# huzaifakhan04/truely-real-time-ai-generated-video-detection-framework-for-social-platforms

Measured on AMD Instinct MI355X. Metric: frames/sec (detect+embed+drift) 720p, higher is better.
Workload: dtype f32; 1 GPU; BASELINE configs[1]: synthetic 720p 1-face frames, batch=256 per GPU, fp32, MTCNN detect + 80x80 crop + InceptionResnetV1 embed + cosine drift score; frames_per_gpu=256, height=720, width=1280, weights=seeded synthetic (no checkpoints offline), prelu_slopes=unit, min_face_size=20, pyramid_levels=11, valid_faces=256, score=6, emb_crc32=3015932725, mode=sharded, ingest=resident, parallelism=single GPU, batches_in_flight=1, driver=single, embed_group=8

## Files before the change

include/truely_hip.h:

```cpp
#ifndef TRUELY_HIP_H
#define TRUELY_HIP_H
#include <stddef.h>
#include <stdint.h>

#ifdef __cplusplus
extern "C" {
#endif

#define TRL_ABI_VERSION 7

typedef enum {
    TRL_OK = 0,
    TRL_ERR_INVALID = -1,
    TRL_ERR_HIP = -2,
    TRL_ERR_WEIGHTS = -3,
    TRL_ERR_CAPACITY = -4,
    TRL_ERR_STATE = -5
} trl_status;

typedef struct trl_ctx trl_ctx;

typedef struct {
    int    device;
    int    min_face_size;
    float  thr0, thr1, thr2;
    double factor;
    int    cap_level;
    int    cap_frame;
    int    max_faces;
    int    pnet_mode;
    int    embed_mode;
    int    embed_precision;
} trl_config;

int  trl_abi_version(void);
const char* trl_last_error(void);
int  trl_default_config(trl_config* cfg);

int  trl_create(const trl_config* cfg, trl_ctx** out);
int  trl_destroy(trl_ctx* ctx);
int  trl_load_weights(trl_ctx* ctx, const void* host_blob, size_t nbytes);

int  trl_mtcnn_detect(trl_ctx* ctx, const uint8_t* d_frames, int n, int H, int W,
                      float* d_boxes, float* d_probs, int32_t* d_counts, void* stream);

int  trl_mtcnn_detect_landmarks(trl_ctx* ctx, const uint8_t* d_frames, int n, int H, int W,
                                float* d_boxes, float* d_probs, float* d_points, int32_t* d_counts, void* stream);

int  trl_mtcnn_detect_ordered(trl_ctx* ctx, const uint8_t* d_frames, int n, int H, int W, int order,
                              float* d_boxes, float* d_probs, float* d_points, int32_t* d_counts, void* stream);

int  trl_select_faces(trl_ctx* ctx, int n, const float* d_boxes, const float* d_probs, const int32_t* d_counts, int H, int W,
                      int method, float threshold, double center_weight, int32_t* d_pick, void* stream);

int  trl_extract_faces(trl_ctx* ctx, const uint8_t* d_frames, int n, int H, int W, const int32_t* d_frame_of, const float* d_boxes,
                       int m, int S, int margin, int resample, int post_process, float* d_out, int32_t* d_status, void* stream);

int  trl_facenet_embed(trl_ctx* ctx, const float* d_faces, int n, int h, int w, float* d_emb, void* stream);

int  trl_facenet_num_classes(trl_ctx* ctx, int* C);
int  trl_facenet_features(trl_ctx* ctx, const float* d_faces, const uint8_t* d_valid, int n, int h, int w, float* d_feat, void* stream);
int  trl_facenet_logits(trl_ctx* ctx, const float* d_feat, int n, float* d_logits, long long ld, void* stream);

int  trl_detect_embed(trl_ctx* ctx, const uint8_t* d_frames, int n, int H, int W,
                      float* d_box, float* d_prob, int32_t* d_rect, uint8_t* d_valid, float* d_emb,
                      void* stream);

int  trl_detect_crop(trl_ctx* ctx, const uint8_t* d_frames, int n, int H, int W,
                     float* d_box, float* d_prob, int32_t* d_rect, uint8_t* d_valid, float* d_faces, void* stream);
int  trl_facenet_embed_masked(trl_ctx* ctx, const float* d_faces, const uint8_t* d_valid, int n, int h, int w, float* d_emb, void* stream);

int  trl_detect_embed_begin(trl_ctx* ctx, const uint8_t* d_frames, int n, int H, int W,
                            float* d_box, float* d_prob, int32_t* d_rect, uint8_t* d_valid, float* d_emb, void* stream);
int  trl_detect_crop_begin(trl_ctx* ctx, const uint8_t* d_frames, int n, int H, int W,
                           float* d_box, float* d_prob, int32_t* d_rect, uint8_t* d_valid, float* d_faces, void* stream);
int  trl_detect_embed_end(trl_ctx* ctx);

int  trl_drift_score(trl_ctx* ctx, const float* d_emb, const uint8_t* d_valid, int n,
                     long long frame_count, int fps, float* d_sims, uint8_t* d_flags,
                     int32_t* d_result, void* stream);

#define TRL_DRIFT_STATE_BYTES 2064
int  trl_drift_update(trl_ctx* ctx, void* d_state, const float* d_emb, const uint8_t* d_valid, int n,
                      long long frame_count, int fps, float* d_sims, uint8_t* d_flags, int32_t* d_result, void* stream);

int  trl_ingest_nv12(trl_ctx* ctx, const uint8_t* d_nv12, int n_in, int H, int W, int step,
                     uint8_t* d_bgr, int* n_out, void* stream);
int  trl_ingest_i420(trl_ctx* ctx, const uint8_t* d_i420, int n_in, int H, int W, int step,
                     uint8_t* d_bgr, int* n_out, void* stream);

int  trl_debug_stage_boxes(trl_ctx* ctx, int stage, int frame, float* h_boxes, int max_rows, int* n_out);
int  trl_debug_level_counts(trl_ctx* ctx, int frame, int32_t* h_cand, int32_t* h_keep, int* n_levels);
int  trl_debug_level_cands(trl_ctx* ctx, int frame, int level, void* h_rows, int max_rows, int* n_out);
int  trl_debug_level_keep(trl_ctx* ctx, int frame, int level, int32_t* h_idx, int max_rows, int* n_out);
int  trl_debug_nms_tiers(trl_ctx* ctx, int small_tier, int full_tier);
int  trl_debug_list_stats(trl_ctx* ctx, long long* h_out8);
int  trl_debug_option(trl_ctx* ctx, const char* key, int value);
int  trl_debug_pnet_screen_bound(trl_ctx* ctx, float* A, float* B, int* on);
int  trl_debug_pnet_screen_weights(trl_ctx* ctx, float* h_g16);
int  trl_debug_batch_capacity(trl_ctx* ctx, float t2_per_frame, float t3_per_frame, int* last_attempts);
int  trl_debug_pyramid_level(trl_ctx* ctx, const uint8_t* d_frame, int H, int W, int level, float* d_out, int* h, int* w, void* stream);
int  trl_debug_pyramid_batch(trl_ctx* ctx, const uint8_t* d_frames, int n, int H, int W, float* d_out, long long* pyr_stride,
                             int32_t* h_levels, int max_levels, int* n_levels, void* stream);
#define TRL_PYR_PLAN_COLS 6
enum { TRL_PYR_FINE = 1, TRL_PYR_S4 = 2, TRL_PYR_S8 = 3, TRL_PYR_SW4 = 4, TRL_PYR_SW8 = 5,
       TRL_PYR_L0_3 = 6, TRL_PYR_L0_4 = 7, TRL_PYR_L0_5 = 8, TRL_PYR_L1 = 9, TRL_PYR_L2 = 10 };
int  trl_debug_pyramid_plan(trl_ctx* ctx, int32_t* h_rows, int max_levels, int* n_levels);
enum { TRL_FNK_FN_CONV = 1, TRL_FNK_FN_SPLIT4 = 2, TRL_FNK_CONV_TAP = 3, TRL_FNK_IGEMM_VEC = 4, TRL_FNK_IGEMM_SCALAR = 5,
       TRL_FNK_SPLITK4 = 6, TRL_FNK_SPLITK4_TAP = 7, TRL_FNK_TAP48 = 8, TRL_FNK_BF16 = 9 };
typedef struct {
    int32_t conv, family, bm, bn, bk, pad, nz, m, cout, k, precision, has_res;
    char layer[48];
} trl_fn_plan_row;
int  trl_debug_facenet_plan(trl_ctx* ctx, trl_fn_plan_row* h_rows, int max_rows, int* n_rows);
int  trl_debug_facenet_capture(trl_ctx* ctx, int conv_index);
int  trl_debug_facenet_capture_read(trl_ctx* ctx, int view, void* h_dst, size_t max_bytes, int32_t* dims5);
int  trl_debug_poison(trl_ctx* ctx, int byte);
int  trl_debug_pnet_level(trl_ctx* ctx, const uint8_t* d_frame, int H, int W, int level,
                          float* d_prob, float* d_reg, int* oh, int* ow, void* stream);
int  trl_debug_rnet(trl_ctx* ctx, const float* d_crops, int n, float* d_out, void* stream);
int  trl_debug_onet(trl_ctx* ctx, const float* d_crops, int n, float* d_out, void* stream);
int  trl_debug_front_net(trl_ctx* ctx, const uint8_t* d_frame, int H, int W, const float* h_boxes, int nb, int net,
                         float* d_out, void* stream);
int  trl_debug_stage_net(trl_ctx* ctx, const uint8_t* d_frames, int nf, int H, int W, const float* h_recs, int nb, int net,
                         int capacity, float* d_out, void* stream);
int  trl_debug_front(trl_ctx* ctx, const uint8_t* d_frames, int nf, int H, int W, const int32_t* h_win, int nb, int net,
                     int capacity, float* d_pool, void* stream);
int  trl_debug_lists(trl_ctx* ctx, int kind, int n, int H, int W, const int32_t* h_caps, int n_levels, const int32_t* h_counts,
                     const void* h_rows, const float* h_logits, float* h_pts, float* d_boxes, float* d_probs, float* d_points,
                     int32_t* d_counts, float* d_box0, float* d_prob0, int32_t* d_rect, uint8_t* d_valid, void* stream);
int  trl_debug_mtcnn_plan(trl_ctx* ctx, trl_fn_plan_row* h_rows, int max_rows, int* n_rows);
int  trl_debug_crop_resize(trl_ctx* ctx, const uint8_t* d_frames, int n, int H, int W,
                           const int32_t* d_rect, const uint8_t* d_valid, float* d_faces, void* stream);
int  trl_debug_crop_aligned(trl_ctx* ctx, const uint8_t* d_frames, int n, int H, int W, const float* d_pts,
                            const uint8_t* d_valid, int S, int rgb, float* d_faces, void* stream);
int  trl_debug_crop_area(trl_ctx* ctx, const uint8_t* d_frames, int n, int H, int W, const int32_t* d_rect,
                         const uint8_t* d_valid, int S, int rgb, float* d_faces, void* stream);
int  trl_debug_timings(trl_ctx* ctx, float* out4);
int  trl_debug_workspace(trl_ctx* ctx, int what, int n, int h, int w, long long* h_out6);
enum { TRL_RZ_MAX_GUARD = 1 << 20, TRL_RZ_MAX_HITS = 256, TRL_RZ_CLEAR = 1, TRL_RZ_SWEEP = 2 };
typedef struct {
    int32_t arena, block;
    char site[24];
    long long block_bytes, gap_off, gap_bytes, first, last, count;
} trl_rz_hit;
int  trl_debug_redzone(trl_ctx* ctx, long long guard, int byte);
int  trl_debug_redzone_report(trl_ctx* ctx, int flags, long long* h_out4, trl_rz_hit* h_hits, int max_hits);
int  trl_debug_redzone_poke(trl_ctx* ctx, int arena, int block, long long offset, int value);
int  trl_debug_stage_totals(trl_ctx* ctx, int32_t* h_out2);
int  trl_debug_pnet_run(trl_ctx* ctx, int run);
int  trl_debug_pnet_kernel_ms(trl_ctx* ctx, float* ms);
int  trl_debug_pnet_span(trl_ctx* ctx, int reset, double* ms_sum, int32_t* launches);

typedef struct trl_jpeg trl_jpeg;
int  trl_jpeg_create(int device, int H, int W, int quality, int max_frames, trl_jpeg** out);
int  trl_jpeg_destroy(trl_jpeg* enc);
int  trl_jpeg_encode(trl_jpeg* enc, const uint8_t* d_bgr, int n, long long frame_stride, uint8_t* d_out, long long capacity,
                     long long* h_sizes, void* stream);
int  trl_jpeg_header(int H, int W, int quality, uint8_t* buf, size_t cap, int* len);
typedef struct trl_jpeg_options {
    int quality, subsampling, restart_rows, restart_blocks, optimize;
} trl_jpeg_options;
int  trl_jpeg_create_ex(int device, int H, int W, const trl_jpeg_options* opt, int max_frames, trl_jpeg** out);
int  trl_jpeg_header_ex(int H, int W, const trl_jpeg_options* opt, uint8_t* buf, size_t cap, int* len);
int  trl_jpeg_optimal_table(const uint32_t* hist, uint8_t* bits, uint8_t* vals, int* nvals, int* maxlen);

typedef struct trl_jpegd trl_jpegd;
typedef struct {
    int32_t width, height;
    int32_t h_samp, v_samp;
    int32_t restart_interval;
    int32_t scan_offset;
    int32_t supported;
    int32_t reason;
} trl_jpegd_info;
int  trl_jpegd_parse(const uint8_t* file, size_t len, trl_jpegd_info* info);
int  trl_jpegd_create(int device, int H, int W, int max_frames, long long max_bytes, trl_jpegd** out);
int  trl_jpegd_destroy(trl_jpegd* dec);
int  trl_jpegd_debug_poison(trl_jpegd* dec, int byte);
int  trl_jpegd_decode(trl_jpegd* dec, const uint8_t* h_files, const uint8_t* d_files, const long long* offsets, const long long* sizes,
                      int n, uint8_t* d_bgr, long long frame_stride, int32_t* h_status, void* stream);

typedef struct {
    int32_t frame;
    int32_t x0, y0, x1, y1;
    int32_t thickness;
    int32_t seg_begin, seg_end;
    uint8_t rect_bgr[3];
    uint8_t text_bgr[3];
    uint8_t reserved[2];
} trl_draw_frame;
typedef struct { float x0, y0, dx, dy, L2, reach; } trl_draw_seg;
size_t trl_draw_workspace(int n_frames, int n_segs);
int  trl_draw(uint8_t* d_bgr, int n, long long frame_stride, int H, int W, const trl_draw_frame* frames, int n_frames,
              const trl_draw_seg* segs, int n_segs, void* d_work, size_t work_bytes, void* stream);

int    trl_gallery_pack(const float* d_rows, long long m, float* d_mat, long long ld, float* d_n2, long long c0, void* stream);
int    trl_gallery_scores(const float* d_q, int n, const float* d_mat, long long ld, const float* d_n2, long long m, int metric,
                          float* d_out, long long ldo, void* stream);
size_t trl_gallery_search_workspace(int n, long long m, int k, int max_strip_cols);
int    trl_gallery_search(const float* d_q, const uint8_t* d_valid, int n, const float* d_mat, long long ld, const float* d_n2,
                          long long m, int metric, int k, float* d_score, int32_t* d_index, void* d_ws, size_t ws_bytes,
                          int max_strip_cols, void* stream);

int    trl_cluster_links(const float* d_q, const uint8_t* d_valid, int n, const float* d_mat, long long ld, const float* d_n2,
                         int metric, float threshold, uint32_t* d_adj, long long pitch_words, int32_t* d_degree,
                         int max_strip_cols, void* stream);
size_t trl_cluster_workspace(int n);
int    trl_cluster_labels(const uint32_t* d_adj, long long pitch_words, const int32_t* d_degree, int n, int min_samples,
                          int32_t* d_labels, uint8_t* d_core, int32_t* d_count, void* d_ws, size_t ws_bytes, int* rounds_out,
                          void* stream);
size_t trl_cluster_lists_workspace(int n);
int    trl_cluster_labels_lists(const long long* d_offsets, const int32_t* d_index, const uint8_t* d_valid, int n, int min_samples,
                                int lanes_per_row, int32_t* d_degree, int32_t* d_labels, uint8_t* d_core, int32_t* d_count,
                                void* d_ws, size_t ws_bytes, int* rounds_out, void* stream);

size_t trl_gallery_hist_workspace(int n, long long m, int nedges, int max_strip_cols);
int    trl_gallery_hist(const float* d_q, const uint8_t* d_qvalid, const int32_t* d_qid, int n, const float* d_mat, long long ld,
                        const float* d_n2, const uint8_t* d_gvalid, const int32_t* d_gid, long long m, int metric, int pairs,
                        const float* d_edges, int nedges, long long* d_counts, void* d_ws, size_t ws_bytes, int max_strip_cols,
                        void* stream);

size_t trl_gallery_range_workspace(int n, long long m, int max_strip_cols);
int    trl_gallery_range_count(const float* d_q, const uint8_t* d_qvalid, int n, const float* d_mat, long long ld, const float* d_n2,
                               const uint8_t* d_gvalid, long long m, int metric, float threshold, int self, long long* d_offsets,
                               void* d_ws, size_t ws_bytes, int max_strip_cols, void* stream);
int    trl_gallery_range_fill(const float* d_q, const uint8_t* d_qvalid, int n, const float* d_mat, long long ld, const float* d_n2,
                              const uint8_t* d_gvalid, long long m, int metric, float threshold, int self, const long long* d_offsets,
                              const void* d_ws, size_t ws_bytes, long long capacity, int32_t* d_index, float* d_score,
                              int max_strip_cols, void* stream);

size_t trl_gallery_search_groups_workspace(int n, long long m, int k, int max_strip_cols);
int    trl_gallery_search_groups(const float* d_q, const uint8_t* d_valid, int n, const float* d_mat, long long ld, const float* d_n2,
                                 const int32_t* d_gid, long long m, int metric, int k, float* d_score, int32_t* d_index,
                                 int32_t* d_group, void* d_ws, size_t ws_bytes, int max_strip_cols, void* stream);

#define TRL_TRACK_SLOTS 64
#define TRL_TRACK_STATE_BYTES 135200
int    trl_track_update(void* d_state, const float* d_boxes, const int32_t* d_counts, int n, int m, const float* d_emb, float iou_min,
                        float sim_min, int max_age, int32_t* d_track, float* d_sim, uint8_t* d_flag, int32_t* d_table, int table_cap,
                        void* stream);
int    trl_track_scores(const void* d_state, const int32_t* d_table, int table_cap, long long frame_count, int fps, int32_t* d_score,
                        int32_t* d_summary, void* stream);

#ifdef __cplusplus
}
#endif
#endif
```

truely-real-time-ai-generated-video-detection-framework-for-social-platforms_amd/_lib.py:

```python
from __future__ import annotations

import ctypes as C
import os

_HERE = os.path.dirname(os.path.abspath(__file__))
LIB_PATH = os.path.join(_HERE, "libtruely_hip.so")


class TrlConfig(C.Structure):
    _fields_ = [("device", C.c_int), ("min_face_size", C.c_int), ("thr0", C.c_float), ("thr1", C.c_float),
                ("thr2", C.c_float), ("factor", C.c_double), ("cap_level", C.c_int), ("cap_frame", C.c_int),
                ("max_faces", C.c_int), ("pnet_mode", C.c_int), ("embed_mode", C.c_int), ("embed_precision", C.c_int)]


class TrlJpegdInfo(C.Structure):
    _fields_ = [(n, C.c_int32) for n in ("width", "height", "h_samp", "v_samp", "restart_interval", "scan_offset", "supported", "reason")]


class TrlJpegOptions(C.Structure):
    _fields_ = [(n, C.c_int) for n in ("quality", "subsampling", "restart_rows", "restart_blocks", "optimize")]


class TrlRzHit(C.Structure):
    _fields_ = [("arena", C.c_int32), ("block", C.c_int32), ("site", C.c_char * 24)] + \
               [(n, C.c_longlong) for n in ("block_bytes", "gap_off", "gap_bytes", "first", "last", "count")]


class TrlError(RuntimeError):
    def __init__(self, status: int, msg: str):
        super().__init__(f"libtruely_hip status {status}: {msg}")
        self.status = status


_lib = None
_vp, _i, _f = C.c_void_p, C.c_int, C.c_float

_SIGNATURES = {
    "trl_abi_version": (C.c_int, []),
    "trl_last_error": (C.c_char_p, []),
    "trl_default_config": (C.c_int, [C.POINTER(TrlConfig)]),
    "trl_create": (C.c_int, [C.POINTER(TrlConfig), C.POINTER(_vp)]),
    "trl_destroy": (C.c_int, [_vp]),
    "trl_load_weights": (C.c_int, [_vp, C.c_char_p, C.c_size_t]),
    "trl_mtcnn_detect": (C.c_int, [_vp, _vp, _i, _i, _i, _vp, _vp, _vp, _vp]),
    "trl_mtcnn_detect_landmarks": (C.c_int, [_vp, _vp, _i, _i, _i, _vp, _vp, _vp, _vp, _vp]),
    "trl_mtcnn_detect_ordered": (C.c_int, [_vp, _vp, _i, _i, _i, _i, _vp, _vp, _vp, _vp, _vp]),
    "trl_select_faces": (C.c_int, [_vp, _i, _vp, _vp, _vp, _i, _i, _i, _f, C.c_double, _vp, _vp]),
    "trl_extract_faces": (C.c_int, [_vp, _vp, _i, _i, _i, _vp, _vp, _i, _i, _i, _i, _i, _vp, _vp, _vp]),
    "trl_facenet_embed": (C.c_int, [_vp, _vp, _i, _i, _i, _vp, _vp]),
    "trl_facenet_num_classes": (C.c_int, [_vp, C.POINTER(_i)]),
    "trl_facenet_features": (C.c_int, [_vp, _vp, _vp, _i, _i, _i, _vp, _vp]),
    "trl_facenet_logits": (C.c_int, [_vp, _vp, _i, _vp, C.c_longlong, _vp]),
    "trl_detect_embed": (C.c_int, [_vp, _vp, _i, _i, _i, _vp, _vp, _vp, _vp, _vp, _vp]),
    "trl_detect_crop": (C.c_int, [_vp, _vp, _i, _i, _i, _vp, _vp, _vp, _vp, _vp, _vp]),
    "trl_detect_embed_begin": (C.c_int, [_vp, _vp, _i, _i, _i, _vp, _vp, _vp, _vp, _vp, _vp]),
    "trl_detect_crop_begin": (C.c_int, [_vp, _vp, _i, _i, _i, _vp, _vp, _vp, _vp, _vp, _vp]),
    "trl_detect_embed_end": (C.c_int, [_vp]),
    "trl_facenet_embed_masked": (C.c_int, [_vp, _vp, _vp, _i, _i, _i, _vp, _vp]),
    "trl_drift_score": (C.c_int, [_vp, _vp, _vp, _i, C.c_longlong, _i, _vp, _vp, _vp, _vp]),
    "trl_ingest_nv12": (C.c_int, [_vp, _vp, _i, _i, _i, _i, _vp, C.POINTER(_i), _vp]),
    "trl_ingest_i420": (C.c_int, [_vp, _vp, _i, _i, _i, _i, _vp, C.POINTER(_i), _vp]),
    "trl_drift_update": (C.c_int, [_vp, _vp, _vp, _vp, _i, C.c_longlong, _i, _vp, _vp, _vp, _vp]),
    "trl_debug_stage_boxes": (C.c_int, [_vp, _i, _i, _vp, _i, C.POINTER(_i)]),
    "trl_debug_level_counts": (C.c_int, [_vp, _i, _vp, _vp, C.POINTER(_i)]),
    "trl_debug_level_cands": (C.c_int, [_vp, _i, _i, _vp, _i, C.POINTER(_i)]),
    "trl_debug_level_keep": (C.c_int, [_vp, _i, _i, _vp, _i, C.POINTER(_i)]),
    "trl_debug_batch_capacity": (C.c_int, [_vp, _f, _f, C.POINTER(_i)]),
    "trl_debug_nms_tiers": (C.c_int, [_vp, _i, _i]),
    "trl_debug_option": (C.c_int, [_vp, C.c_char_p, _i]),
    "trl_debug_list_stats": (C.c_int, [_vp, C.POINTER(C.c_longlong)]),
    "trl_debug_poison": (C.c_int, [_vp, _i]),
    "trl_debug_pyramid_level": (C.c_int, [_vp, _vp, _i, _i, _i, _vp, C.POINTER(_i), C.POINTER(_i), _vp]),
    "trl_debug_pyramid_batch": (C.c_int, [_vp, _vp, _i, _i, _i, _vp, C.POINTER(C.c_longlong), _vp, _i, C.POINTER(_i), _vp]),
    "trl_debug_pyramid_plan": (C.c_int, [_vp, _vp, _i, C.POINTER(_i)]),
    "trl_debug_facenet_plan": (C.c_int, [_vp, _vp, _i, C.POINTER(_i)]),
    "trl_debug_facenet_capture": (C.c_int, [_vp, _i]),
    "trl_debug_facenet_capture_read": (C.c_int, [_vp, _i, _vp, C.c_size_t, _vp]),
    "trl_debug_pnet_level": (C.c_int, [_vp, _vp, _i, _i, _i, _vp, _vp, C.POINTER(_i), C.POINTER(_i), _vp]),
    "trl_debug_rnet": (C.c_int, [_vp, _vp, _i, _vp, _vp]),
    "trl_debug_onet": (C.c_int, [_vp, _vp, _i, _vp, _vp]),
    "trl_debug_front_net": (C.c_int, [_vp, _vp, _i, _i, _vp, _i, _i, _vp, _vp]),
    "trl_debug_stage_net": (C.c_int, [_vp, _vp, _i, _i, _i, _vp, _i, _i, _i, _vp, _vp]),
    "trl_debug_front": (C.c_int, [_vp, _vp, _i, _i, _i, _vp, _i, _i, _i, _vp, _vp]),
    "trl_debug_mtcnn_plan": (C.c_int, [_vp, _vp, _i, C.POINTER(_i)]),
    "trl_debug_lists": (C.c_int, [_vp, _i, _i, _i, _i, _vp, _i, _vp, _vp, _vp, _vp, _vp, _vp, _vp, _vp, _vp, _vp, _vp, _vp, _vp]),
    "trl_debug_crop_resize": (C.c_int, [_vp, _vp, _i, _i, _i, _vp, _vp, _vp, _vp]),
    "trl_debug_crop_aligned": (C.c_int, [_vp, _vp, _i, _i, _i, _vp, _vp, _i, _i, _vp, _vp]),
    "trl_debug_crop_area": (C.c_int, [_vp, _vp, _i, _i, _i, _vp, _vp, _i, _i, _vp, _vp]),
    "trl_debug_timings": (C.c_int, [_vp, C.POINTER(_f)]),
    "trl_debug_workspace": (C.c_int, [_vp, _i, _i, _i, _i, C.POINTER(C.c_longlong)]),
    "trl_debug_redzone": (C.c_int, [_vp, C.c_longlong, _i]),
    "trl_debug_redzone_report": (C.c_int, [_vp, _i, C.POINTER(C.c_longlong), C.POINTER(TrlRzHit), _i]),
    "trl_debug_redzone_poke": (C.c_int, [_vp, _i, _i, C.c_longlong, _i]),
    "trl_debug_stage_totals": (C.c_int, [_vp, C.POINTER(C.c_int32)]),
    "trl_debug_pnet_run": (C.c_int, [_vp, _i]),
    "trl_debug_pnet_kernel_ms": (C.c_int, [_vp, C.POINTER(C.c_float)]),
    "trl_debug_pnet_span": (C.c_int, [_vp, C.c_int, C.POINTER(C.c_double), C.POINTER(C.c_int32)]),
    "trl_debug_pnet_screen_bound": (C.c_int, [_vp, C.POINTER(_f), C.POINTER(_f), C.POINTER(_i)]),
    "trl_debug_pnet_screen_weights": (C.c_int, [_vp, C.POINTER(_f)]),
    "trl_jpeg_create": (C.c_int, [_i, _i, _i, _i, _i, C.POINTER(_vp)]),
    "trl_jpeg_destroy": (C.c_int, [_vp]),
    "trl_jpeg_encode": (C.c_int, [_vp, _vp, _i, C.c_longlong, _vp, C.c_longlong, _vp, _vp]),
    "trl_jpeg_header": (C.c_int, [_i, _i, _i, _vp, C.c_size_t, C.POINTER(_i)]),
    "trl_jpeg_create_ex": (C.c_int, [_i, _i, _i, C.POINTER(TrlJpegOptions), _i, C.POINTER(_vp)]),
    "trl_jpeg_header_ex": (C.c_int, [_i, _i, C.POINTER(TrlJpegOptions), _vp, C.c_size_t, C.POINTER(_i)]),
    "trl_jpeg_optimal_table": (C.c_int, [_vp, _vp, _vp, C.POINTER(_i), C.POINTER(_i)]),
    "trl_jpegd_parse": (C.c_int, [_vp, C.c_size_t, _vp]),
    "trl_jpegd_create": (C.c_int, [_i, _i, _i, _i, C.c_longlong, C.POINTER(_vp)]),
    "trl_jpegd_destroy": (C.c_int, [_vp]),
    "trl_jpegd_debug_poison": (C.c_int, [_vp, _i]),
    "trl_jpegd_decode": (C.c_int, [_vp, _vp, _vp, _vp, _vp, _i, _vp, C.c_longlong, _vp, _vp]),
    "trl_draw_workspace": (C.c_size_t, [_i, _i]),
    "trl_draw": (C.c_int, [_vp, _i, C.c_longlong, _i, _i, _vp, _i, _vp, _i, _vp, C.c_size_t, _vp]),
    "trl_gallery_pack": (C.c_int, [_vp, C.c_longlong, _vp, C.c_longlong, _vp, C.c_longlong, _vp]),
    "trl_gallery_scores": (C.c_int, [_vp, _i, _vp, C.c_longlong, _vp, C.c_longlong, _i, _vp, C.c_longlong, _vp]),
    "trl_gallery_search_workspace": (C.c_size_t, [_i, C.c_longlong, _i, _i]),
    "trl_gallery_search": (C.c_int, [_vp, _vp, _i, _vp, C.c_longlong, _vp, C.c_longlong, _i, _i, _vp, _vp, _vp, C.c_size_t, _i, _vp]),
    "trl_cluster_links": (C.c_int, [_vp, _vp, _i, _vp, C.c_longlong, _vp, _i, _f, _vp, C.c_longlong, _vp, _i, _vp]),
    "trl_cluster_workspace": (C.c_size_t, [_i]),
    "trl_cluster_labels": (C.c_int, [_vp, C.c_longlong, _vp, _i, _i, _vp, _vp, _vp, _vp, C.c_size_t, C.POINTER(_i), _vp]),
    "trl_cluster_lists_workspace": (C.c_size_t, [_i]),
    "trl_cluster_labels_lists": (C.c_int, [_vp, _vp, _vp, _i, _i, _i, _vp, _vp, _vp, _vp, _vp, C.c_size_t, C.POINTER(_i), _vp]),
    "trl_gallery_hist_workspace": (C.c_size_t, [_i, C.c_longlong, _i, _i]),
    "trl_gallery_hist": (C.c_int, [_vp, _vp, _vp, _i, _vp, C.c_longlong, _vp, _vp, _vp, C.c_longlong, _i, _i, _vp, _i, _vp, _vp, C.c_size_t, _i, _vp]),
    "trl_gallery_range_workspace": (C.c_size_t, [_i, C.c_longlong, _i]),
    "trl_gallery_range_count": (C.c_int, [_vp, _vp, _i, _vp, C.c_longlong, _vp, _vp, C.c_longlong, _i, _f, _i, _vp, _vp, C.c_size_t, _i, _vp]),
    "trl_gallery_range_fill": (C.c_int, [_vp, _vp, _i, _vp, C.c_longlong, _vp, _vp, C.c_longlong, _i, _f, _i, _vp, _vp, C.c_size_t, C.c_longlong,
                                         _vp, _vp, _i, _vp]),
    "trl_gallery_search_groups_workspace": (C.c_size_t, [_i, C.c_longlong, _i, _i]),
    "trl_gallery_search_groups": (C.c_int, [_vp, _vp, _i, _vp, C.c_longlong, _vp, _vp, C.c_longlong, _i, _i, _vp, _vp, _vp, _vp, C.c_size_t,
                                            _i, _vp]),
    "trl_track_update": (C.c_int, [_vp, _vp, _vp, _i, _i, _vp, _f, _f, _i, _vp, _vp, _vp, _vp, _i, _vp]),
    "trl_track_scores": (C.c_int, [_vp, _vp, _i, C.c_longlong, _i, _vp, _vp, _vp]),
}
EXPORTS = tuple(_SIGNATURES)


def load(path: str | None = None):
    global _lib
    if _lib is not None:
        return _lib
    path = path or os.environ.get("TRUELY_HIP_LIB") or LIB_PATH
    if not os.path.exists(path):
        raise ImportError(f"{path} not found: build it with `make -C {_HERE}/csrc` "
                          "(or __graft_entry__.build()); there is no CPU fallback")
    try:
        import torch
    except Exception:
        pass
    lib = C.CDLL(path, mode=C.RTLD_GLOBAL)
    for name, (res, args) in _SIGNATURES.items():
        fn = getattr(lib, name, None)
        if fn is None and path != LIB_PATH and name.startswith("trl_debug_"):
            continue
        if fn is None:
            raise ImportError(f"{path} lacks {name}")
        fn.restype = res
        fn.argtypes = args
    if lib.trl_abi_version() != 7:
        raise ImportError("libtruely_hip ABI mismatch")
    _lib = lib
    return lib


def check(status: int):
    if status != 0:
        raise TrlError(status, load().trl_last_error().decode(errors="replace"))
```

truely-real-time-ai-generated-video-detection-framework-for-social-platforms_amd/csrc/trl_api.hip:

```cpp
#include <limits.h>
#include <stdarg.h>
#include <stdio.h>
#include <string.h>
#include <stdlib.h>
#include <algorithm>

#include "trl_ctx.h"

static thread_local char g_err[512] = "";
int g_trl_no_fnconv = 0;
int g_trl_pnet_gate = 0;

#include <mutex>
namespace {
std::mutex g_gate_mu;
hipEvent_t g_gate_ev[64] = {};
bool g_gate_set[64] = {};
}
int trl_gate_wait(trl_ctx* c, hipStream_t s) {
    const int d = c->cfg.device;
    if (!g_trl_pnet_gate || d < 0 || d >= 64) return TRL_OK;
    std::lock_guard<std::mutex> lk(g_gate_mu);
    if (g_gate_set[d]) TRL_HIP(hipStreamWaitEvent(s, g_gate_ev[d], 0));
    return TRL_OK;
}
int trl_gate_record(trl_ctx* c, hipStream_t s) {
    const int d = c->cfg.device;
    if (!g_trl_pnet_gate || d < 0 || d >= 64) return TRL_OK;
    std::lock_guard<std::mutex> lk(g_gate_mu);
    if (!g_gate_ev[d]) TRL_HIP(hipEventCreateWithFlags(&g_gate_ev[d], hipEventDisableTiming));
    TRL_HIP(hipEventRecord(g_gate_ev[d], s));
    g_gate_set[d] = true;
    return TRL_OK;
}
void trl_set_error(const char* fmt, ...) {
    va_list ap;
    va_start(ap, fmt);
    vsnprintf(g_err, sizeof g_err, fmt, ap);
    va_end(ap);
}

extern "C" {

int trl_abi_version(void) { return TRL_ABI_VERSION; }
const char* trl_last_error(void) { return g_err; }

int trl_default_config(trl_config* cfg) {
    if (!cfg) return TRL_ERR_INVALID;
    cfg->device = 0;
    cfg->min_face_size = 20;
    cfg->thr0 = 0.6f; cfg->thr1 = 0.7f; cfg->thr2 = 0.7f;
    cfg->factor = 0.709;
    cfg->cap_level = 2048;
    cfg->cap_frame = 2048;
    cfg->max_faces = 64;
    cfg->pnet_mode = 0;
    cfg->embed_mode = 0;
    cfg->embed_precision = 0;
    return TRL_OK;
}

int trl_create(const trl_config* cfg, trl_ctx** out) {
    if (!cfg || !out) { trl_set_error("null argument"); return TRL_ERR_INVALID; }
    if (cfg->cap_level < 64 || cfg->cap_level > (1 << 24) || cfg->cap_frame < 64 || cfg->cap_frame > (1 << 24) || (cfg->cap_level & 3) ||
        (cfg->cap_frame & 3) || cfg->min_face_size < 12 || cfg->max_faces < 1 || !(cfg->factor > 0.1 && cfg->factor < 0.99) || cfg->embed_mode < 0 || cfg->embed_mode > 3 ||
        cfg->embed_precision < 0 || cfg->embed_precision > 2) {
        trl_set_error("bad trl_config (list start capacities must be multiples of 4 in [64, 2^24], min_face_size >= 12)");
        return TRL_ERR_INVALID;
    }
    TRL_HIP(hipSetDevice(cfg->device));
    trl_ctx* c = new trl_ctx();
    c->cfg = *cfg;
    c->pnet_prof = trl_tune_set("TRL_PNET_CLOCK");
    if (hipMalloc((void**)&c->pnet_clk, 8 * 41) != hipSuccess || hipMemset(c->pnet_clk, 0, 8 * 41) != hipSuccess || hipMemset(c->pnet_clk, 0xFF, 8) != hipSuccess ||
        hipMalloc((void**)&c->pnet_cursor, 64) != hipSuccess || hipHostMalloc((void**)&c->h_pinned, 1024) != hipSuccess ||
        hipEventCreate(&c->ev_call0) != hipSuccess || hipEventCreate(&c->ev_call1) != hipSuccess) {
        trl_set_error("context allocation failed: %s", hipGetErrorString(hipGetLastError()));
        trl_destroy(c);
        return TRL_ERR_HIP;
    }
    memset(c->h_pinned, 0, 1024);
    *out = c;
    return TRL_OK;
}

int trl_destroy(trl_ctx* c) {
    if (!c) return TRL_OK;
    (void)hipSetDevice(c->cfg.device);
    (void)hipDeviceSynchronize();
    c->pend.active = false;
    trl_free_weights(c);
    if (c->arena.base) (void)hipFree(c->arena.base);
    if (c->scratch.base) (void)hipFree(c->scratch.base);
    if (c->sims_tmp.base) (void)hipFree(c->sims_tmp.base);
    if (c->pyr_tab) (void)hipFree(c->pyr_tab);
    if (c->rz.dev) (void)hipFree(c->rz.dev);
    for (auto& b : c->fn_cap) if (b.p) (void)hipFree(b.p);
    if (c->pnet_clk) {
        unsigned long long t[41];
        if (c->pnet_prof && hipMemcpy(t, c->pnet_clk, sizeof t, hipMemcpyDeviceToHost) == hipSuccess && t[2 + 32] > 0) {
            static const char* nm[8] = {"phase0", "barrier0", "phase1", "barrier1", "phase2", "barrier2", "phase3", "barrier3"};
            const double tiles = (double)t[2 + 32];
            fprintf(stderr, "[TRL_PNET_CLOCK] shader clocks per tile (wave 0..3), %.0f workgroup-tiles\n", tiles);
            for (int k = 0; k < 8; k++)
                fprintf(stderr, "[TRL_PNET_CLOCK] %-9s %8.0f %8.0f %8.0f %8.0f\n", nm[k], t[2 + k] / tiles, t[2 + 8 + k] / tiles, t[2 + 16 + k] / tiles, t[2 + 24 + k] / tiles);
            fprintf(stderr, "[TRL_PNET_CLOCK] fp16 screen: %llu M-tiles screened, %llu confirmed (%.2f %%)\n", t[39], t[40],
                    t[39] ? 100.0 * (double)t[40] / (double)t[39] : 0.0);
        }
        (void)hipFree(c->pnet_clk);
    }
    if (c->pnet_cursor) (void)hipFree(c->pnet_cursor);
    if (c->h_pinned) (void)hipHostFree(c->h_pinned);
    if (c->ev_call0) (void)hipEventDestroy(c->ev_call0);
    if (c->ev_call1) (void)hipEventDestroy(c->ev_call1);
    for (auto& e : c->pnet_ev) { (void)hipEventDestroy(e.first); (void)hipEventDestroy(e.second); }
    delete c;
    return TRL_OK;
}

}

__global__ void k_rz_scan(const unsigned char* __restrict__ base, const unsigned long long* __restrict__ gaps, unsigned long long* __restrict__ res,
                          int g0, unsigned byte) {
    const int g = g0 + blockIdx.y;
    const unsigned long long len = gaps[2 * g + 1];
    const unsigned char* p = base + gaps[2 * g];
    unsigned long long head = (16 - ((uintptr_t)p & 15)) & 15;
    if (head > len) head = len;
    const unsigned long long nw = (len - head) / 16, tail0 = head + nw * 16;
    const unsigned long long w = 0x0101010101010101ull * (byte & 0xFF);
    const unsigned long long tid = (unsigned long long)blockIdx.x * blockDim.x + threadIdx.x, nt = (unsigned long long)gridDim.x * blockDim.x;
    unsigned long long cnt = 0, first = ~0ull, last = 0;
    auto look = [&](unsigned long long i) {
        if (p[i] == (unsigned char)byte) return;
        cnt++;
        if (i < first) first = i;
        if (i > last) last = i;
    };
    if (tid == 0) {
        for (unsigned long long i = 0; i < head; i++) look(i);
        for (unsigned long long i = tail0; i < len; i++) look(i);
    }
    const ulonglong2* q = reinterpret_cast<const ulonglong2*>(p + head);
    for (unsigned long long k = tid; k < nw; k += nt) {
        const ulonglong2 v = q[k];
        if (v.x == w && v.y == w) continue;
        for (int b = 0; b < 16; b++) look(head + k * 16 + b);
    }
    if (cnt) {
        atomicAdd(&res[3 * g], cnt);
        atomicMin(&res[3 * g + 1], first);
        atomicMax(&res[3 * g + 2], last);
    }
}

namespace {
struct RzGap { size_t off, len; int block; size_t block_bytes; };
void rz_gaps(const Arena& a, std::vector<RzGap>& out) {
    const size_t nb = a.blocks.size();
    for (size_t i = 0; i < nb; i++) {
        const size_t end = a.blocks[i].off + a.blocks[i].bytes, next = i + 1 < nb ? a.blocks[i + 1].off : a.off;
        if (next > end) out.push_back({end, next - end, (int)i, a.blocks[i].bytes});
    }
    if (a.cap > a.off) out.push_back({a.off, a.cap - a.off, (int)nb, 0});
}
int rz_sweep(trl_ctx* c, Arena& a, const char* site, long long refill_from) {
    trl_ctx::RedZone& z = c->rz;
    TRL_HIP(hipDeviceSynchronize());
    if (!a.base) return TRL_OK;
    std::vector<RzGap> gaps;
    rz_gaps(a, gaps);
    const size_t ng = gaps.size();
    if (ng) {
        if (z.dev_gaps < ng) {
            if (z.dev) TRL_HIP(hipFree(z.dev));
            z.dev = nullptr; z.dev_gaps = 0;
            TRL_HIP(hipMalloc((void**)&z.dev, (ng + 256) * 5 * 8));
            z.dev_gaps = ng + 256;
        }
        std::vector<unsigned long long> tab(5 * ng, 0);
        for (size_t g = 0; g < ng; g++) { tab[2 * g] = gaps[g].off; tab[2 * g + 1] = gaps[g].len; tab[2 * ng + 3 * g + 1] = ~0ull; }
        TRL_HIP(hipMemcpy(z.dev, tab.data(), tab.size() * 8, hipMemcpyHostToDevice));
        const bool has_tail = gaps.back().block == (int)a.blocks.size();
        const size_t nshort = has_tail ? ng - 1 : ng;
        for (size_t g0 = 0; g0 < nshort; g0 += 32768) {
            const unsigned ny = (unsigned)std::min<size_t>(32768, nshort - g0);
            k_rz_scan<<<dim3(4, ny), 256>>>((const unsigned char*)a.base, z.dev, z.dev + 2 * ng, (int)g0, (unsigned)z.byte);
            TRL_LAUNCH_CHECK();
        }
        if (has_tail) {
            k_rz_scan<<<dim3(4096, 1), 256>>>((const unsigned char*)a.base, z.dev, z.dev + 2 * ng, (int)(ng - 1), (unsigned)z.byte);
            TRL_LAUNCH_CHECK();
        }
        TRL_HIP(hipMemcpy(tab.data() + 2 * ng, z.dev + 2 * ng, 3 * ng * 8, hipMemcpyDeviceToHost));
        for (size_t g = 0; g < ng; g++) {
            z.bytes += (long long)gaps[g].len;
            const unsigned long long* r = &tab[2 * ng + 3 * g];
            if (!r[0]) continue;
            z.nhits++;
            if (z.hits.size() < TRL_RZ_MAX_HITS) {
                trl_rz_hit h;
                memset(&h, 0, sizeof h);
                h.arena = &a == &c->arena ? 0 : 1; h.block = gaps[g].block;
                strncpy(h.site, site, sizeof(h.site) - 1);
                h.block_bytes = (long long)gaps[g].block_bytes; h.gap_off = (long long)gaps[g].off; h.gap_bytes = (long long)gaps[g].len;
                h.first = (long long)r[1]; h.last = (long long)r[2]; h.count = (long long)r[0];
                z.hits.push_back(h);
            }
            TRL_HIP(hipMemset(a.base + gaps[g].off, z.byte, gaps[g].len));
        }
    }
    z.sweeps++;
    if (refill_from >= 0 && (size_t)refill_from < a.cap) TRL_HIP(hipMemset(a.base + refill_from, z.byte, a.cap - (size_t)refill_from));
    TRL_HIP(hipDeviceSynchronize());
    return TRL_OK;
}
void rz_on_rewind(Arena& a, size_t mark, const char* site, void* owner) { (void)rz_sweep((trl_ctx*)owner, a, site, (long long)mark); }
}

int trl_rz_sweep_all(trl_ctx* c, const char* site) {
    TRL_CHECK(rz_sweep(c, c->arena, site, -1));
    return rz_sweep(c, c->scratch, site, -1);
}

int trl_ensure(trl_ctx* c, Arena& a, size_t bytes) {
    if (bytes <= a.cap) return TRL_OK;
    const size_t ncap = bytes + (bytes >> 3) + (32u << 20);
    TRL_HIP(hipDeviceSynchronize());
    if (a.guard && a.base) TRL_CHECK(rz_sweep(c, a, "ensure", -1));
    if (a.base) { TRL_HIP(hipFree(a.base)); a.base = nullptr; a.cap = 0; }
    TRL_HIP(hipMalloc((void**)&a.base, ncap));
    a.cap = ncap;
    a.off = 0;
    a.blocks.clear();
    if (c->dbg_poison >= 0) TRL_HIP(hipMemset(a.base, c->dbg_poison, ncap));
    return TRL_OK;
}

int trl_check_idle(trl_ctx* c) {
    if (!c) { trl_set_error("null context"); return TRL_ERR_INVALID; }
    if (c->pend.active) { trl_set_error("the context has a call in flight: trl_detect_embed_end() first"); return TRL_ERR_STATE; }
    return TRL_OK;
}

static int check_call(trl_ctx* c, const void* frames, int n, int H, int W) {
    TRL_CHECK(trl_check_idle(c));
    if (!c->have_weights) { trl_set_error("trl_load_weights has not been called"); return TRL_ERR_STATE; }
    if (!frames || n <= 0 || n > 65535 || H < 12 || W < 12 || H > 16383 || W > 16383) {
        trl_set_error("bad frame batch n=%d H=%d W=%d (1..65535 frames of 12..16383 px per side)", n, H, W);
        return TRL_ERR_INVALID;
    }
    if (((uintptr_t)frames & 3) != 0) { trl_set_error("frame buffer must be 4-byte aligned"); return TRL_ERR_INVALID; }
    return TRL_OK;
}

static void collect_timings(trl_ctx* c) {
    float call_ms = 0.f, pnet_ms = 0.f, pyr_ms = 0.f;
    (void)hipEventElapsedTime(&call_ms, c->ev_call0, c->ev_call1);
    int launches = 0;
    if (c->cfg.pnet_mode == 0 && c->pnet_ev_used >= 2) {
// ... 522 lines not shown
        const int cap = kind == 1 ? h_caps[i % n_levels] : h_caps[n_levels];
        if (h_counts[i] < 0 || h_counts[i] > cap) { trl_set_error("list %d: count %d, capacity %d", i, h_counts[i], cap); return TRL_ERR_INVALID; }
        total += h_counts[i];
    }
    if (total > 0 && (!h_rows || (kind > 1 && !h_logits))) { trl_set_error("null rows"); return TRL_ERR_INVALID; }
    TRL_HIP(hipSetDevice(c->cfg.device));
    const int st = trl_cascade_lists(c, kind, n, H, W, h_caps, n_levels, h_counts, h_rows, h_logits, h_pts, d_boxes, d_probs, d_points, d_counts,
                                     d_box0, d_prob0, d_rect, d_valid, (hipStream_t)stream);
    TRL_CHECK(trl_rz_end(c, "lists_hook"));
    return st;
}

int trl_debug_workspace(trl_ctx* c, int what, int n, int h, int w, long long* h_out6) {
    TRL_CHECK(trl_check_idle(c));
    if (!h_out6 || (what != 0 && what != 1 && what != 24 && what != 48) || (what && n <= 0) || (what == 1 && (h < 75 || w < 75))) { trl_set_error("bad argument"); return TRL_ERR_INVALID; }
    if (what && !c->have_weights) { trl_set_error("context without weights"); return TRL_ERR_STATE; }
    Arena X = Arena::counter(c->scratch.guard);
    if (what == 1) TRL_CHECK(embed_need(c, false, n, h, w));
    else if (what) { const NetDesc& d = trl_net_of(what); TRL_CHECK(trl_run_net(c, X, d, 0, Act::dense(nullptr, n, d.side, d.side, 3), nullptr, nullptr)); }
    const size_t v[6] = {c->scratch.cap, c->scratch.high, c->arena.cap, c->arena.off, c->arena_need, what == 1 ? c->fn_need_bytes : X.high};
    for (int k = 0; k < 6; k++) h_out6[k] = (long long)v[k];
    return TRL_OK;
}

int trl_debug_redzone(trl_ctx* c, long long guard, int byte) {
    TRL_CHECK(trl_check_idle(c));
    if (guard < 0 || guard > TRL_RZ_MAX_GUARD || (guard & 255) || byte < 0 || byte > 255) {
        trl_set_error("bad red zone: guard %lld (0, or a multiple of 256 up to %d), fill byte %d", guard, (int)TRL_RZ_MAX_GUARD, byte);
        return TRL_ERR_INVALID;
    }
    trl_ctx::RedZone& z = c->rz;
    if (!guard && !z.guard) return TRL_OK;
    TRL_HIP(hipSetDevice(c->cfg.device));
    TRL_HIP(hipDeviceSynchronize());
    if (!z.guard) z.saved_poison = c->dbg_poison;
    for (Arena* a : {&c->arena, &c->scratch}) {
        if (a->base) TRL_HIP(hipFree(a->base));
        a->base = nullptr; a->cap = a->off = a->high = 0;
        a->blocks.clear();
        a->guard = (size_t)guard; a->on_rewind = guard ? rz_on_rewind : nullptr; a->owner = c;
    }
    c->cb = CascadeBufs();
    c->arena_need = 0;
    c->fn_need_key[0] = 0;
    z.guard = (size_t)guard; z.byte = byte;
    z.sweeps = z.bytes = z.nhits = 0;
    z.hits.clear();
    c->dbg_poison = guard ? byte : z.saved_poison;
    return TRL_OK;
}

int trl_debug_redzone_report(trl_ctx* c, int flags, long long* h_out4, trl_rz_hit* h_hits, int max_hits) {
    TRL_CHECK(trl_check_idle(c));
    if (!h_out4 || (max_hits > 0 && !h_hits)) { trl_set_error("null argument"); return TRL_ERR_INVALID; }
    trl_ctx::RedZone& z = c->rz;
    if ((flags & TRL_RZ_SWEEP) && z.guard) {
        TRL_HIP(hipSetDevice(c->cfg.device));
        TRL_CHECK(trl_rz_sweep_all(c, "report"));
    }
    int m = 0;
    for (; m < (int)z.hits.size() && m < max_hits; m++) h_hits[m] = z.hits[m];
    h_out4[0] = z.sweeps; h_out4[1] = z.bytes; h_out4[2] = z.nhits; h_out4[3] = m;
    if (flags & TRL_RZ_CLEAR) { z.sweeps = z.bytes = z.nhits = 0; z.hits.clear(); }
    return TRL_OK;
}

int trl_debug_redzone_poke(trl_ctx* c, int arena, int block, long long offset, int value) {
    TRL_CHECK(trl_check_idle(c));
    trl_ctx::RedZone& z = c->rz;
    if (!z.guard) { trl_set_error("red zones are off"); return TRL_ERR_STATE; }
    if ((arena != 0 && arena != 1) || value < 0 || value > 255 || value == z.byte) { trl_set_error("bad argument"); return TRL_ERR_INVALID; }
    Arena& a = arena ? c->scratch : c->arena;
    if (!a.base) { trl_set_error("the workspace has not been allocated"); return TRL_ERR_STATE; }
    std::vector<RzGap> gaps;
    rz_gaps(a, gaps);
    if (block < 0) block = (int)a.blocks.size();
    for (const RzGap& g : gaps) {
        if (g.block != block) continue;
        if (offset < 0 || (size_t)offset >= g.len) break;
        TRL_HIP(hipSetDevice(c->cfg.device));
        TRL_HIP(hipDeviceSynchronize());
        TRL_HIP(hipMemset(a.base + g.off + (size_t)offset, value, 1));
        TRL_HIP(hipDeviceSynchronize());
        return TRL_OK;
    }
    trl_set_error("no byte %lld in the gap behind block %d (%zu live blocks)", offset, block, a.blocks.size());
    return TRL_ERR_INVALID;
}

int trl_debug_mtcnn_plan(trl_ctx* c, trl_fn_plan_row* h_rows, int max_rows, int* n_rows) {
    TRL_CHECK(trl_check_idle(c));
    if (!n_rows || (max_rows > 0 && !h_rows)) { trl_set_error("null argument"); return TRL_ERR_INVALID; }
    *n_rows = (int)c->mt_plan.size();
    for (int i = 0; i < *n_rows && i < max_rows; i++) h_rows[i] = c->mt_plan[i];
    return TRL_OK;
}

static int check_crop_hook(trl_ctx* c, const void* d_frames, int n, int n_max, int H, int W, const void* d_rows, const void* d_valid,
                           int S, const void* d_faces) {
    if (!c || !d_frames || !d_rows || !d_valid || !d_faces || n <= 0 || n > n_max || H < 1 || W < 1 || S < 1 || S > 4096) {
        trl_set_error("bad argument (n=%d H=%d W=%d S=%d)", n, H, W, S);
        return TRL_ERR_INVALID;
    }
    return TRL_OK;
}
int trl_debug_crop_resize(trl_ctx* c, const uint8_t* d_frames, int n, int H, int W, const int32_t* d_rect, const uint8_t* d_valid,
                          float* d_faces, void* stream) {
    TRL_CHECK(check_crop_hook(c, d_frames, n, INT_MAX, H, W, d_rect, d_valid, 80, d_faces));
    TRL_CHECK(trl_launch_crop_resize80(d_frames, n, H, W, d_rect, d_valid, d_faces, (hipStream_t)stream));
    return trl_rz_end(c, "crop_resize");
}
int trl_debug_crop_aligned(trl_ctx* c, const uint8_t* d_frames, int n, int H, int W, const float* d_pts, const uint8_t* d_valid, int S,
                           int rgb, float* d_faces, void* stream) {
    TRL_CHECK(check_crop_hook(c, d_frames, n, 65535, H, W, d_pts, d_valid, S, d_faces));
    TRL_CHECK(trl_launch_crop_aligned(d_frames, n, H, W, d_pts, d_valid, S, rgb != 0, d_faces, (hipStream_t)stream));
    return trl_rz_end(c, "crop_aligned");
}
int trl_debug_crop_area(trl_ctx* c, const uint8_t* d_frames, int n, int H, int W, const int32_t* d_rect, const uint8_t* d_valid, int S,
                        int rgb, float* d_faces, void* stream) {
    TRL_CHECK(check_crop_hook(c, d_frames, n, 65535, H, W, d_rect, d_valid, S, d_faces));
    TRL_CHECK(trl_launch_crop_area_std(d_frames, n, H, W, d_rect, d_valid, S, rgb != 0, d_faces, (hipStream_t)stream));
    return trl_rz_end(c, "crop_area");
}
int trl_debug_nms_tiers(trl_ctx* c, int small_tier, int full_tier) {
    TRL_CHECK(trl_check_idle(c));
    if ((small_tier && (small_tier < 16 || small_tier > 3072 || (small_tier & 3))) || (full_tier && (full_tier < 16 || full_tier > 3072 || (full_tier & 3)))) {
        trl_set_error("tiers must be multiples of 4 in [16, 3072]");
        return TRL_ERR_INVALID;
    }
    if (small_tier) c->nms_small = small_tier;
    if (full_tier) c->nms_full = full_tier;
    return TRL_OK;
}
int trl_debug_list_stats(trl_ctx* c, long long* h_out8) {
    if (!c || !h_out8) { trl_set_error("null argument"); return TRL_ERR_INVALID; }
    const int32_t* f = c->h_pinned + 4;
    unsigned long long used = 0;
    memcpy(&used, f + FLG_SPILL_CUR, 8);
    int mx = 0;
    for (int l = 0; l < 32; l++) if (f[FLG_LEVEL_MAX + l] > mx) mx = f[FLG_LEVEL_MAX + l];
    h_out8[0] = c->caps.last_attempts; h_out8[1] = f[FLG_SPILL_LISTS]; h_out8[2] = (long long)used; h_out8[3] = (long long)c->cb.spill_cap;
    h_out8[4] = c->cb.capF; h_out8[5] = c->cb.lay.S; h_out8[6] = mx; h_out8[7] = f[FLG_FRAME_MAX];
    return TRL_OK;
}

int trl_debug_option(trl_ctx* c, const char* key, int value) {
    if (!key) { trl_set_error("null key"); return TRL_ERR_INVALID; }
    if (!strcmp(key, "no_fnconv")) { g_trl_no_fnconv = value ? 1 : 0; return TRL_OK; }
    if (!strcmp(key, "pnet_gate")) { g_trl_pnet_gate = value ? 1 : 0; return TRL_OK; }
    TRL_CHECK(trl_check_idle(c));
    if (!strcmp(key, "rnet_chunk") && value >= 16) { c->rnet_chunk = value; return TRL_OK; }
    if (!strcmp(key, "onet_chunk") && value >= 16) { c->onet_chunk = value; return TRL_OK; }
    if (!strcmp(key, "pnet_screen") && (value == 0 || value == 1)) { c->pnet_screen = value; return TRL_OK; }
    if (!strcmp(key, "pyr_row_bands") && value >= 0) { c->pyr_row_bands = value; return TRL_OK; }
    if (!strcmp(key, "tail_pool") && (value == 0 || value == 1)) { c->tail_pool = value; return TRL_OK; }
    trl_set_error("unknown option '%s' (or value %d out of range)", key, value);
    return TRL_ERR_INVALID;
}

int trl_debug_pnet_screen_bound(trl_ctx* c, float* A, float* B, int* on) {
    if (!c || !A || !B || !on) { trl_set_error("null argument"); return TRL_ERR_INVALID; }
    *A = c->pnet_scrA; *B = c->pnet_scrB; *on = c->pnet_screen_ok && c->pnet_screen;
    return TRL_OK;
}

int trl_debug_pnet_screen_weights(trl_ctx* c, float* h_g16) {
    if (!c || !h_g16) { trl_set_error("null argument"); return TRL_ERR_INVALID; }
    for (int i = 0; i < 16; i++) h_g16[i] = c->pnet_scrG[i];
    return TRL_OK;
}

int trl_debug_batch_capacity(trl_ctx* c, float t2_per_frame, float t3_per_frame, int* last_attempts) {
    if (!c) { trl_set_error("null context"); return TRL_ERR_INVALID; }
    if (t2_per_frame > 0.f) c->caps.t_per_frame[0] = t2_per_frame;
    if (t3_per_frame > 0.f) c->caps.t_per_frame[1] = t3_per_frame;
    if (last_attempts) *last_attempts = c->caps.last_attempts;
    return TRL_OK;
}

int trl_debug_stage_totals(trl_ctx* c, int32_t* h_out2) {
    if (!c || !h_out2) { trl_set_error("null argument"); return TRL_ERR_INVALID; }
    h_out2[0] = c->h_pinned[4 + FLG_T2N]; h_out2[1] = c->h_pinned[4 + FLG_T3N];
    return TRL_OK;
}

int trl_debug_pnet_run(trl_ctx* c, int run) {
    if (!c || run < 0 || run > 64) { trl_set_error("bad argument"); return TRL_ERR_INVALID; }
    c->pnet_run = run;
    return TRL_OK;
}

int trl_debug_pnet_span(trl_ctx* c, int reset, double* ms_sum, int32_t* launches) {
    if (!c || !ms_sum || !launches) { trl_set_error("null argument"); return TRL_ERR_INVALID; }
    *ms_sum = 0.0; *launches = 0;
    if (!c->pnet_clk) return TRL_OK;
    TRL_CHECK(trl_check_idle(c));
    TRL_HIP(hipSetDevice(c->cfg.device));
    TRL_HIP(hipDeviceSynchronize());
    unsigned long long t[2] = {0, 0};
    int khz = 0;
    TRL_HIP(hipMemcpy(t, c->pnet_clk + 36, sizeof t, hipMemcpyDeviceToHost));
    TRL_HIP(hipDeviceGetAttribute(&khz, hipDeviceAttributeWallClockRate, c->cfg.device));
    if (khz > 0) *ms_sum = (double)t[0] / (double)khz;
    *launches = (int32_t)t[1];
    if (reset) TRL_HIP(hipMemset(c->pnet_clk + 36, 0, 16));
    return TRL_OK;
}

int trl_debug_pnet_kernel_ms(trl_ctx* c, float* ms) {
    if (!c || !ms) { trl_set_error("null argument"); return TRL_ERR_INVALID; }
    *ms = c->pnet_kernel_ms;
    return TRL_OK;
}

int trl_debug_timings(trl_ctx* c, float* out4) {
    if (!c || !out4) return TRL_ERR_INVALID;
    out4[0] = c->last_ms[0]; out4[1] = c->last_ms[1]; out4[2] = c->last_ms[2]; out4[3] = c->last_ms[3];
    return TRL_OK;
}

}
```

truely-real-time-ai-generated-video-detection-framework-for-social-platforms_amd/csrc/trl_capacity.h:

```cpp
#pragma once
#include <cstddef>
#include <cstdint>
#include <cstring>

enum { TRL_NFLAGS = 64 };
enum { FLG_LEVEL = 0, FLG_FRAME = 1, FLG_T2 = 2, FLG_T3 = 3, FLG_T2N = 4, FLG_T3N = 5, FLG_FRAME_MAX = 6, FLG_SPILL = 7,
       FLG_SPILL_CUR = 8 , FLG_SPILL_LISTS = 10, FLG_LEVEL_MAX = 16  };

struct LvLayout {
    int L = 0, S = 0;
    int capl[32] = {0}, rec0[32] = {0};
};

struct CapRule { float mul, add, decay, floor; };
inline float trl_cap_follow(const CapRule& r, float cur, float measured, float per, bool overflow) {
    const float want = r.mul * measured / per + r.add;
    if (overflow) return want;
    const float d = r.decay * cur;
    return want > d ? want : (d > r.floor ? d : (cur < r.floor ? cur : r.floor));
}

struct CascadeCaps {
    static constexpr float T_START[2] = {160.f, 48.f};
    static constexpr CapRule T_RULE[2] = {{1.25f, 1.f, 0.97f, T_START[0]}, {1.25f, 1.f, 0.97f, T_START[1]}};
    static constexpr CapRule LIST_RULE = {1.25f, 4.f, 0.97f, 0.f};

    float t_per_frame[2] = {T_START[0], T_START[1]};
    float lvl_hint[32] = {0}, frame_hint = 0.f;
    size_t spill_hint = 0;
    int cap_t[2] = {0, 0};
    int resume_stage = 0;
    int last_attempts = 0;
};

struct CascadePlan { LvLayout lay; int capF = 0; int cap_t[2] = {0, 0}; };
inline int trl_cap_list(long long start, float hint, long long cells) {
    long long want = start;
    if ((long long)hint > want) want = (long long)hint;
    if (want > cells) want = cells;
    if (want < 4) want = 4;
    return (int)((want + 3) & ~3ll);
}
inline CascadePlan trl_caps_plan(const CascadeCaps& k, int cap_level, int cap_frame, const long long* cells, int L, int n) {
    CascadePlan p;
    LvLayout& G = p.lay;
    G.L = L;
    long long cells_total = 0;
    for (int l = 0; l < L; l++) {
        G.capl[l] = trl_cap_list(cap_level, k.lvl_hint[l], cells[l]);
        G.rec0[l] = G.S;
        G.S += G.capl[l];
        cells_total += cells[l];
    }
    p.capF = trl_cap_list(cap_frame, k.frame_hint, cells_total);
    const long long lim = (long long)n * p.capF;
    for (int s = 0; s < 2; s++) {
        const long long want = (long long)(k.t_per_frame[s] * n) + 64;
        p.cap_t[s] = (int)(want < lim ? want : lim);
    }
    return p;
}

struct CapsVerdict { int retry, resume_stage; };
inline CapsVerdict trl_caps_check(CascadeCaps& k, const int32_t* f, int n, const LvLayout& lay) {
    const int L = lay.L;
    k.resume_stage = 0;
    unsigned long long spill_used = 0;
    memcpy(&spill_used, f + FLG_SPILL_CUR, 8);
    if (f[FLG_LEVEL]) {
        long long sum = 0;
        for (int l = 0; l < L; l++) {
            const float want = trl_cap_follow(CascadeCaps::LIST_RULE, k.lvl_hint[l], (float)f[FLG_LEVEL_MAX + l], 1.f, true);
            if (f[FLG_LEVEL_MAX + l] > lay.capl[l] && want > k.lvl_hint[l]) k.lvl_hint[l] = want;
            sum += f[FLG_LEVEL_MAX + l];
        }
        if ((float)sum > k.frame_hint && (double)sum * 132.0 * (double)n < 8e9) k.frame_hint = (float)sum;
        return {1, 0};
    }
    const float frame_max = (float)f[FLG_FRAME_MAX];
    if (f[FLG_SPILL]) {
        k.spill_hint = (size_t)spill_used * 2 + (16u << 20);
        if (f[FLG_FRAME]) k.frame_hint = trl_cap_follow(CascadeCaps::LIST_RULE, k.frame_hint, frame_max, 1.f, true);
        return {1, 0};
    }
    if (f[FLG_FRAME]) { k.frame_hint = trl_cap_follow(CascadeCaps::LIST_RULE, k.frame_hint, frame_max, 1.f, true); return {1, 0}; }
    for (int s = 0; s < 2; s++)
        if (f[FLG_T2 + s]) {
            k.t_per_frame[s] = trl_cap_follow(CascadeCaps::T_RULE[s], k.t_per_frame[s], (float)f[FLG_T2N + s], (float)n, true);
            return {1, k.resume_stage = 2 + s};
        }
    for (int s = 0; s < 2; s++)
        k.t_per_frame[s] = trl_cap_follow(CascadeCaps::T_RULE[s], k.t_per_frame[s], (float)f[FLG_T2N + s], (float)n, false);
    for (int l = 0; l < L; l++)
        k.lvl_hint[l] = trl_cap_follow(CascadeCaps::LIST_RULE, k.lvl_hint[l], (float)f[FLG_LEVEL_MAX + l], 1.f, false);
    k.frame_hint = trl_cap_follow(CascadeCaps::LIST_RULE, k.frame_hint, frame_max, 1.f, false);
    {
        const size_t want = (size_t)spill_used + (spill_used >> 2), d = k.spill_hint - (k.spill_hint >> 5);
        k.spill_hint = spill_used ? (want > d ? want : d) : (d > (1u << 20) ? d : 0);
    }
    return {0, 0};
}
```

truely-real-time-ai-generated-video-detection-framework-for-social-platforms_amd/csrc/trl_cascade.hip:

```cpp
#include "trl_ctx.h"
#include <algorithm>
#include <stdlib.h>
#include <string.h>


namespace {

__device__ __forceinline__ uint32_t f2ord(float f) {
    uint32_t u = __float_as_uint(f);
    return (u & 0x80000000u) ? ~u : (u | 0x80000000u);
}

__device__ __forceinline__ uint64_t sort_key(float score, uint32_t tie) { return ((uint64_t)~f2ord(score) << 32) | tie; }
constexpr uint64_t NO_KEY = ~0ull;

__device__ void lds_bitonic_steps(uint64_t* key, uint32_t* id, int C, int base, int k, int j0) {
    for (int j = j0; j > 0; j >>= 1) {
        for (int t = threadIdx.x; t < C; t += blockDim.x) {
            const int u = t ^ j;
            if (u > t) {
                const bool up = (((base + t) & k) == 0);
                const uint64_t a = key[t], b = key[u];
                if ((a > b) == up) {
                    key[t] = b; key[u] = a;
// ... 543 lines not shown
                                                     const float* __restrict__ s1_box, const int32_t* __restrict__ off2,
                                                     const float* __restrict__ out6, int32_t* __restrict__ n2,
                                                     float* __restrict__ s2_box, Spill sp) {
    extern __shared__ __attribute__((aligned(16))) unsigned char smem_raw[];
    Smem S(smem_raw, lds_cap, blockDim.x);
    const int f = blockIdx.x;
    const int cnt = n1[f];
    if (cnt == 0 || off2[gridDim.x] > cap_total) { if (threadIdx.x == 0) n2[f] = 0; return; }
    const float* logits = out6 + (size_t)off2[f] * 6;
    const float* fb = s1_box + (size_t)f * capF * 5;
    auto prob = [&](int i) { return trl_softmax2_p1(logits[6 * i], logits[6 * i + 1]); };
    auto s1 = [&](uint32_t i) { const float* b = fb + 5 * i; return make_float4(b[0], b[1], b[2], b[3]); };
    const Kept K = sort_and_suppress<false, true>(S, lds_cap, cnt, 0.7f, sp, nullptr, W, H,
        [&](int i, uint32_t&) { const float p = prob(i); return p > thr ? sort_key(p, (uint32_t)i) : NO_KEY; },
        s1);
    const int out = write_rows(S, lds_cap, K.n, s2_box + (size_t)f * capF * 5, [&](int r, float4& b, float& score) {
        const int i = (int)K.id(r);
        score = prob(i);
        return stage2_row(s1(i), logits + 6 * i + 2, W, H, b);
    });
    if (threadIdx.x == 0) n2[f] = out;
}

__device__ __forceinline__ float4 stage3_box(const float* b, const float* g) {
    const float w = b[2] - b[0] + 1.f, h = b[3] - b[1] + 1.f;
    return make_float4(b[0] + g[0] * w, b[1] + g[1] * h, b[2] + g[2] * w, b[3] + g[3] * h);
}
__device__ __forceinline__ void stage3_points(const float* b, const float* pt, float* po) {
    const float w_i = b[2] - b[0] + 1.f, h_i = b[3] - b[1] + 1.f;
    for (int j = 0; j < 5; j++) {
        po[j] = w_i * pt[j] + b[0] - 1.f;
        po[5 + j] = h_i * pt[5 + j] + b[1] - 1.f;
    }
}
__global__ __launch_bounds__(1024) void k_stage3_post(int lds_cap, int capF, int cap_total, float thr, const int32_t* __restrict__ n2, const float* __restrict__ s2_box,
                                                     const int32_t* __restrict__ off3, const float* __restrict__ out16,
                                                     int32_t* __restrict__ n3, float* __restrict__ s3_box, float* __restrict__ s3_pts, Spill sp) {
    extern __shared__ __attribute__((aligned(16))) unsigned char smem_raw[];
    Smem S(smem_raw, lds_cap, blockDim.x);
    const int f = blockIdx.x;
    const int cnt = n2[f];
    if (cnt == 0 || off3[gridDim.x] > cap_total) { if (threadIdx.x == 0) n3[f] = 0; return; }
    const float* logits = out16 + (size_t)off3[f] * 16;
    const float* fb = s2_box + (size_t)f * capF * 5;
    auto prob = [&](int i) { return trl_softmax2_p1(logits[16 * i], logits[16 * i + 1]); };
    const Kept K = sort_and_suppress<true, true>(S, lds_cap, cnt, 0.7f, sp, nullptr, 0, 0,
        [&](int i, uint32_t&) { const float p = prob(i); return p > thr ? sort_key(p, ~(uint32_t)i) : NO_KEY; },
        [&](uint32_t i) { return stage3_box(fb + 5 * i, logits + 16 * i + 2); });
    for (int r = threadIdx.x; r < K.n; r += blockDim.x) {
        const int i = (int)K.id(r);
        const float4 bb = K.box(r);
        float* o = s3_box + ((size_t)f * capF + r) * 5;
        o[0] = bb.x; o[1] = bb.y; o[2] = bb.z; o[3] = bb.w; o[4] = prob(i);
        stage3_points(fb + 5 * i, logits + 16 * i + 6, s3_pts + ((size_t)f * capF + r) * 10);
    }
    if (threadIdx.x == 0) n3[f] = K.n;
}

__global__ __launch_bounds__(64) void k_select(int capF, int max_faces, int W, int H, int order, const int32_t* __restrict__ n3,
                                               const float* __restrict__ s3_box, const float* __restrict__ s3_pts,
                                               float* __restrict__ boxes, float* __restrict__ probs, float* __restrict__ points,
                                               int32_t* __restrict__ counts, float* __restrict__ box0, float* __restrict__ prob0,
                                               int32_t* __restrict__ rect, uint8_t* __restrict__ valid, float* __restrict__ pts0) {
    const int f = blockIdx.x;
    const int n = n3[f];
    const float* b = s3_box + (size_t)f * capF * 5;
    for (int r = threadIdx.x; r < n; r += blockDim.x) {
        int rank = r;
        if (order == 0) {
            const float ar = (b[5 * r + 2] - b[5 * r]) * (b[5 * r + 3] - b[5 * r + 1]);
            rank = 0;
            for (int q = 0; q < n; q++) {
                const float aq = (b[5 * q + 2] - b[5 * q]) * (b[5 * q + 3] - b[5 * q + 1]);
                rank += (aq > ar) || (aq == ar && q > r);
            }
        }
        if (boxes && rank < max_faces) {
            float* o = boxes + ((size_t)f * max_faces + rank) * 4;
            o[0] = b[5 * r]; o[1] = b[5 * r + 1]; o[2] = b[5 * r + 2]; o[3] = b[5 * r + 3];
            probs[(size_t)f * max_faces + rank] = b[5 * r + 4];
            if (points) {
                const float* ps = s3_pts + ((size_t)f * capF + r) * 10;
                float* po = points + ((size_t)f * max_faces + rank) * 10;
                for (int q = 0; q < 10; q++) po[q] = ps[q];
            }
        }
        if (rank == 0 && box0) {
            box0[4 * f] = b[5 * r]; box0[4 * f + 1] = b[5 * r + 1]; box0[4 * f + 2] = b[5 * r + 2]; box0[4 * f + 3] = b[5 * r + 3];
            prob0[f] = b[5 * r + 4];
            long long x0 = (long long)b[5 * r], y0 = (long long)b[5 * r + 1], x1 = (long long)b[5 * r + 2], y1 = (long long)b[5 * r + 3];
            if (x0 < 0) x0 = 0;
            if (y0 < 0) y0 = 0;
            if (x1 > W) x1 = W;
            if (y1 > H) y1 = H;
            rect[4 * f] = (int)x0; rect[4 * f + 1] = (int)y0; rect[4 * f + 2] = (int)x1; rect[4 * f + 3] = (int)y1;
            valid[f] = (x1 > x0 && y1 > y0) ? 1 : 0;
            if (pts0) {
                const float* ps = s3_pts + ((size_t)f * capF + r) * 10;
                for (int q = 0; q < 10; q++) pts0[10 * f + q] = ps[q];
            }
        }
    }
    if (threadIdx.x == 0) {
        if (counts) counts[f] = n < max_faces ? n : max_faces;
        if (n == 0 && box0) {
            for (int q = 0; q < 4; q++) { box0[4 * f + q] = 0.f; rect[4 * f + q] = 0; }
            prob0[f] = 0.f; valid[f] = 0;
            if (pts0) for (int q = 0; q < 10; q++) pts0[10 * f + q] = 0.f;
        }
    }
}

template <typename K>
int set_dyn_smem(K kernel, size_t bytes) {
    TRL_HIP(hipFuncSetAttribute((const void*)kernel, hipFuncAttributeMaxDynamicSharedMemorySize, (int)bytes));
    return TRL_OK;
}

}

int trl_compute_levels(trl_ctx* c, int H, int W) {
    const double m = 12.0 / c->cfg.min_face_size;
    double minl = (H < W ? H : W) * m;
    double scale_i = m;
    int L = 0;
    while (minl >= 12 && L < 32) {
        LevelGeom& g = c->lv[L];
        g.scale = scale_i;
        g.h = (int)(H * scale_i + 1);
        g.w = (int)(W * scale_i + 1);
        const int ph = (g.h - 2 + 1) / 2, pw = (g.w - 2 + 1) / 2;
        g.oh = ph - 4; g.ow = pw - 4;
        L++;
        scale_i = scale_i * c->cfg.factor;
        minl = minl * c->cfg.factor;
    }
    return L;
}

int trl_launch_area_level(const uint8_t* d_frames, int nf, int H, int W, int h, int w, float* d_level, hipStream_t s) {
    const size_t total = (size_t)nf * h * w;
    size_t blocks = (total + 255) / 256;
    if (blocks > 32768) blocks = 32768;
    k_area_level<<<(unsigned)blocks, 256, 0, s>>>(d_frames, nf, H, W, h, w, d_level);
    TRL_LAUNCH_CHECK();
    return TRL_OK;
}
int trl_launch_heads_to_maps(const float* d_heads, int cells, float* d_prob, float* d_reg, hipStream_t s) {
    k_heads_to_maps<<<(cells + 255) / 256, 256, 0, s>>>(d_heads, cells, d_prob, d_reg);
    TRL_LAUNCH_CHECK();
    return TRL_OK;
}

static void plan_caps(trl_ctx* c, int L, int n) {
    long long cells[32];
    for (int l = 0; l < L; l++) cells[l] = (long long)c->lv[l].oh * c->lv[l].ow;
    const CascadePlan p = trl_caps_plan(c->caps, c->cfg.cap_level, c->cfg.cap_frame, cells, L, n);
    c->cb.lay = p.lay;
    c->cb.capF = p.capF;
    c->caps.cap_t[0] = p.cap_t[0]; c->caps.cap_t[1] = p.cap_t[1];
}
static size_t spill_need(long long cnt, int W, int H) {
    long long P = 2;
    while (P < cnt) P <<= 1;
    return SpillWs::bytes((size_t)P, (size_t)cnt, true, true, W, H) + 256;
}

static size_t spill_pool(const trl_ctx* c, int n, int H, int W) {
    const LvLayout& G = c->cb.lay;
    const int lds_full = c->nms_full;
    size_t spill = c->caps.spill_hint;
    size_t per_frame = 0;
    for (int l = 0; l < G.L; l++) if (G.capl[l] > lds_full) per_frame += spill_need(G.capl[l], W, H);
    if (c->cb.capF > lds_full) per_frame += 3 * spill_need(c->cb.capF, W, H);
    size_t up_front = per_frame * (size_t)n;
    if (up_front > (8ull << 30)) up_front = 8ull << 30;
    if (up_front > spill) spill = up_front;
    return spill;
}

struct ListLaunch {
    int small_cap, full_l, full_f, max_capl, th_l, th_f;
    size_t sm_s, sm_l, sm_f;
};
static int list_launch(trl_ctx* c, ListLaunch& ll) {
    const LvLayout& G = c->cb.lay;
    const int capF = c->cb.capF;
    const int lds_full = c->nms_full, lds_small = c->nms_small < c->nms_full ? c->nms_small : c->nms_full;
    int max_capl = 4;
    for (int l = 0; l < G.L; l++) if (G.capl[l] > max_capl) max_capl = G.capl[l];
    ll.max_capl = max_capl;
    ll.full_l = max_capl < lds_full ? max_capl : lds_full;
    ll.full_f = capF < lds_full ? capF : lds_full;
    ll.th_l = max_capl > lds_full ? 1024 : 256;
    ll.th_f = capF > lds_full ? 1024 : 256;
    ll.sm_l = Smem::bytes(ll.full_l, ll.th_l);
    ll.sm_f = Smem::bytes(ll.full_f, ll.th_f);
    ll.small_cap = ll.full_l < lds_small ? ll.full_l : lds_small;
    ll.sm_s = Smem::bytes(ll.small_cap);
    TRL_CHECK(set_dyn_smem(k_nms_level, ll.sm_l));
    TRL_CHECK(set_dyn_smem(k_nms_frame, ll.sm_f));
    TRL_CHECK(set_dyn_smem(k_stage2_post, ll.sm_f));
    TRL_CHECK(set_dyn_smem(k_stage3_post, ll.sm_f));
    return TRL_OK;
}
static int launch_stage1_lists(trl_ctx* c, const ListLaunch& ll, int n, int H, int W, const Spill& sp, hipStream_t s) {
    CascadeBufs& B = c->cb;
    const LvLayout& G = B.lay;
    const int L = G.L;
    k_nms_level<<<n * L, 256, ll.sm_s, s>>>(G, ll.small_cap, 0, ll.small_cap == ll.max_capl ? 1 : 0, W, H, B.lvl_cnt, B.lvl_rec, B.lvl_keep_cnt, B.lvl_keep_idx, B.flags, sp);
    TRL_LAUNCH_CHECK();
    if (ll.small_cap < ll.max_capl) {
        k_nms_level<<<n * L, ll.th_l, ll.sm_l, s>>>(G, ll.full_l, ll.small_cap + 1, 1, W, H, B.lvl_cnt, B.lvl_rec, B.lvl_keep_cnt, B.lvl_keep_idx, B.flags, sp);
        TRL_LAUNCH_CHECK();
    }
    k_nms_frame<<<n, ll.th_f, ll.sm_f, s>>>(G, ll.full_f, B.capF, W, H, B.lvl_rec, B.lvl_keep_cnt, B.lvl_keep_idx, B.cnt[0], B.box[0], B.flags, sp);
    TRL_LAUNCH_CHECK();
    return TRL_OK;
}
struct StageDesc {
    int net;
    float trl_config::*thr;
    void (*post)(const CascadeBufs& B, const ListLaunch& ll, int cap, float thr, const float* out, const Spill& sp, hipStream_t s);
};
static const StageDesc trl_stages[2] = {
    {24, &trl_config::thr1, [](const CascadeBufs& B, const ListLaunch& ll, int cap, float thr, const float* out, const Spill& sp, hipStream_t s) {
         k_stage2_post<<<B.n, ll.th_f, ll.sm_f, s>>>(ll.full_f, B.capF, cap, B.W, B.H, thr, B.cnt[0], B.box[0], B.off[0], out, B.cnt[1], B.box[1], sp);
     }},
    {48, &trl_config::thr2, [](const CascadeBufs& B, const ListLaunch& ll, int cap, float thr, const float* out, const Spill& sp, hipStream_t s) {
         k_stage3_post<<<B.n, ll.th_f, ll.sm_f, s>>>(ll.full_f, B.capF, cap, thr, B.cnt[1], B.box[1], B.off[1], out, B.cnt[2], B.box[2], B.pts3, sp);
     }},
};
static int launch_stage_scan(const CascadeBufs& B, int st, int cap, hipStream_t s) {
    k_scan_counts<<<1, 256, 0, s>>>(B.cnt[st], B.n, B.off[st], cap, B.flags, st);
    TRL_LAUNCH_CHECK();
    return TRL_OK;
}
static int launch_stage_post(trl_ctx* c, const ListLaunch& ll, int st, int cap, const float* out, const Spill& sp, hipStream_t s) {
    trl_stages[st].post(c->cb, ll, cap, c->cfg.*trl_stages[st].thr, out, sp, s);
    TRL_LAUNCH_CHECK();
    return TRL_OK;
}

static void layout_lists(CascadeBufs& B, Arena& A, size_t spill) {
    const LvLayout& G = B.lay;
    const int n = B.n, L = B.L, capF = B.capF;
    A.reset("lists");
    B.lvl_cnt = (int32_t*)A.alloc((size_t)n * L * 4);
    B.lvl_keep_cnt = (int32_t*)A.alloc((size_t)n * L * 4);
    B.lvl_rec = (Cand*)A.alloc((size_t)n * G.S * sizeof(Cand));
    B.lvl_keep_idx = (int32_t*)A.alloc((size_t)n * G.S * 4);
    for (int k = 0; k < 3; k++) B.cnt[k] = (int32_t*)A.alloc((size_t)n * 4);
    for (int k = 0; k < 3; k++) B.box[k] = (float*)A.alloc((size_t)n * capF * 20);
    B.pts3 = (float*)A.alloc((size_t)n * capF * 40);
    for (int k = 0; k < 2; k++) B.off[k] = (int32_t*)A.alloc((size_t)(n + 1) * 4);
    B.cbox = (int32_t*)A.alloc((size_t)n * capF * 32);
    B.flags = (int32_t*)A.alloc(TRL_NFLAGS * 4);
    B.spill = spill ? (char*)A.alloc(spill) : nullptr;
    B.spill_cap = B.spill ? spill : 0;
    B.box0 = (float*)A.alloc((size_t)n * 16); B.prob0 = (float*)A.alloc((size_t)n * 4);
    B.rect = (int32_t*)A.alloc((size_t)n * 16); B.valid = (uint8_t*)A.alloc((size_t)n);
    B.pts0 = (float*)A.alloc((size_t)n * 40);
}
static int carve_lists(trl_ctx* c, size_t spill, hipStream_t s) {
    CascadeBufs& B = c->cb;
    Arena count = Arena::counter(c->arena.guard);
    layout_lists(B, count, spill);
    TRL_CHECK(trl_ensure(c, c->arena, c->arena_need = count.off));
    layout_lists(B, c->arena, spill);
    if (c->arena.off != c->arena_need) { trl_set_error("cascade workspace allocation failed"); return TRL_ERR_STATE; }
    TRL_HIP(hipMemsetAsync(B.flags, 0, TRL_NFLAGS * 4, s));
    return TRL_OK;
}

int trl_pnet_generic_level(trl_ctx* c, Arena& X, const uint8_t* d_frames, int nf, int H, int W, const LevelGeom& g, float** d_heads, hipStream_t s) {
    X.reset("pnet_level");
    float* lvl = (float*)X.alloc((size_t)nf * g.h * g.w * 12);
    float* heads = (float*)X.alloc((size_t)nf * g.oh * g.ow * 24);
    if (!lvl || !heads) { trl_set_error("pnet generic workspace"); return TRL_ERR_STATE; }
    if (!X.counting) TRL_CHECK(trl_launch_area_level(d_frames, nf, H, W, g.h, g.w, lvl, s));
    TRL_CHECK(trl_run_net(c, X, trl_nets[TRL_PNET], 0, Act::dense(lvl, nf, g.h, g.w, 3), heads, s));
    *d_heads = heads;
    return TRL_OK;
}

static int next_pnet_events(trl_ctx* c, std::pair<hipEvent_t, hipEvent_t>*& out) {
    if ((int)c->pnet_ev.size() <= c->pnet_ev_used) {
        hipEvent_t e0, e1;
        TRL_HIP(hipEventCreate(&e0)); TRL_HIP(hipEventCreate(&e1));
        c->pnet_ev.push_back({e0, e1});
    }
    out = &c->pnet_ev[c->pnet_ev_used++];
    return TRL_OK;
}

static int stage_carve(trl_ctx* c, Arena& X, int net, const uint8_t* d_frames, int H, int W, const int32_t* d_total, int cap, float** d_out, hipStream_t s) {
    const NetDesc& d = trl_net_of(net);
    X.reset("stage_carve");
    *d_out = (float*)X.alloc((size_t)cap * d.nout * 4);
    if (!*d_out) { trl_set_error("%s workspace", d.name); return TRL_ERR_STATE; }
    return trl_stage_net(c, X, net, d_frames, H, W, d_total, cap, *d_out, s);
}

static int size_scratch(trl_ctx* c, int n, int H, int W, bool fused) {
    Arena X = Arena::counter(c->scratch.guard);
    X.high = std::max(c->scratch_after_cascade, fused ? trl_pnet_fused_bytes(c, n, H, W) + (1u << 20) : 0);
    float* o;
    for (int l = 0; l < c->cb.L && !fused; l++) {
        LevelGeom& g = c->lv[l];
        if (g.oh < 1 || g.ow < 1) continue;
        TRL_CHECK(trl_pnet_generic_level(c, X, nullptr, 1, 0, 0, g, &o, nullptr));
        g.chunk = (int)std::min<size_t>(n, std::max<size_t>(1, (size_t)(2048ull << 20) / X.off));
        TRL_CHECK(trl_pnet_generic_level(c, X, nullptr, g.chunk, 0, 0, g, &o, nullptr));
    }
    for (int st = 0; st < 2; st++) TRL_CHECK(stage_carve(c, X, trl_stages[st].net, nullptr, 0, 0, nullptr, c->caps.cap_t[st], &o, nullptr));
    return trl_scratch_begin(c, X.high);
}

static int stage1_fused(trl_ctx* c, const uint8_t* d_frames, hipStream_t s) {
    const CascadeBufs& B = c->cb;
    std::pair<hipEvent_t, hipEvent_t>*pa, *pb;
    c->pnet_ev.reserve(64);
    TRL_CHECK(next_pnet_events(c, pa)); TRL_CHECK(next_pnet_events(c, pb));
    hipEvent_t ev[4] = {pa->first, pa->second, pb->first, pb->second};
    return trl_pnet_fused_all(c, d_frames, B.n, B.H, B.W, ev, s);
}

static int stage1_generic(trl_ctx* c, const uint8_t* d_frames, hipStream_t s) {
    const CascadeBufs& B = c->cb;
    const LvLayout& G = B.lay;
    const int n = B.n, H = B.H, W = B.W, L = B.L;
    for (int l = 0; l < L; l++) {
        const LevelGeom& g = c->lv[l];
        if (g.oh < 1 || g.ow < 1) continue;
        std::pair<hipEvent_t, hipEvent_t>* pe;
        TRL_CHECK(next_pnet_events(c, pe));
        TRL_HIP(hipEventRecord(pe->first, s));
        const int chunk = g.chunk;
        for (int f0 = 0; f0 < n; f0 += chunk) {
            const int nf = (n - f0 < chunk) ? n - f0 : chunk;
            float* heads;
            TRL_CHECK(trl_pnet_generic_level(c, c->scratch, d_frames + (size_t)f0 * H * W * 3, nf, H, W, g, &heads, s));
            const size_t total = (size_t)nf * g.oh * g.ow;
            size_t blocks = (total + 255) / 256;
            if (blocks > 16384) blocks = 16384;
            k_pnet_collect<<<(unsigned)blocks, 256, 0, s>>>(heads, nf, f0, g.oh, g.ow, (float)g.scale, c->cfg.thr0, L, l, G.capl[l],
                                                             G.rec0[l], G.S, B.lvl_cnt, B.lvl_rec, B.flags);
            TRL_LAUNCH_CHECK();
        }
        TRL_HIP(hipEventRecord(pe->second, s));
    }
    return TRL_OK;
}

static int stage_net_and_post(trl_ctx* c, int st, const ListLaunch& ll, const uint8_t* d_frames, const Spill& sp, hipStream_t s) {
    const CascadeBufs& B = c->cb;
    const int n = B.n, H = B.H, W = B.W, cap = c->caps.cap_t[st];
    TRL_CHECK(launch_stage_scan(B, st, cap, s));
    k_build_map<<<n, 64, 0, s>>>(B.cnt[st], B.off[st], B.box[st], B.capF, W, H, B.cbox);
    TRL_LAUNCH_CHECK();
    float* out;
    TRL_CHECK(stage_carve(c, c->scratch, trl_stages[st].net, d_frames, H, W, B.off[st] + n, cap, &out, s));
    return launch_stage_post(c, ll, st, cap, out, sp, s);
}

int trl_cascade_detect(trl_ctx* c, const uint8_t* d_frames, int n, int H, int W, hipStream_t s, int resume) {
    const int L = trl_compute_levels(c, H, W);
    CascadeBufs& B = c->cb;
    if (resume >= 2 && !(B.flags && B.n == n && B.L == L && B.H == H && B.W == W && L > 0)) resume = 0;
    B.n = n; B.L = L; B.H = H; B.W = W;
    plan_caps(c, L, n);
    const size_t spill = spill_pool(c, n, H, W);
    if (resume) {
        for (int st = resume - 2; st < 2; st++) {
            TRL_HIP(hipMemsetAsync(B.flags + FLG_T2 + st, 0, 4, s));
            TRL_HIP(hipMemsetAsync(B.flags + FLG_T2N + st, 0, 4, s));
        }
    } else {
        TRL_CHECK(carve_lists(c, spill, s));
    }
    const Spill sp{B.spill, (unsigned long long)B.spill_cap, B.flags};
    if (L == 0) {
        for (int k = 0; k < 3; k++) TRL_HIP(hipMemsetAsync(B.cnt[k], 0, (size_t)n * 4, s));
        for (int k = 0; k < 2; k++) TRL_HIP(hipMemsetAsync(B.off[k], 0, (size_t)(n + 1) * 4, s));
        TRL_CHECK(trl_scratch_begin(c, c->scratch_after_cascade));
        return TRL_OK;
    }
    if (!resume) {
        TRL_HIP(hipMemsetAsync(B.lvl_cnt, 0, (size_t)n * L * 4, s));
        c->pnet_ev_used = 0;
    }
    const bool fused = c->cfg.pnet_mode == 0 && L <= 16;
    TRL_CHECK(size_scratch(c, n, H, W, fused));
    if (!resume) TRL_CHECK(fused ? stage1_fused(c, d_frames, s) : stage1_generic(c, d_frames, s));
    ListLaunch ll;
    TRL_CHECK(list_launch(c, ll));
    if (!resume) TRL_CHECK(launch_stage1_lists(c, ll, n, H, W, sp, s));
    for (int st = resume ? resume - 2 : 0; st < 2; st++) TRL_CHECK(stage_net_and_post(c, st, ll, d_frames, sp, s));
    return TRL_OK;
}

int trl_stage_net(trl_ctx* c, Arena& X, int net, const uint8_t* d_frames, int H, int W, const int32_t* d_total, int cap, float* d_out, hipStream_t s) {
    const NetDesc& d = trl_net_of(net);
    const int CH = c->*d.chunk;
    const size_t mk = X.off;
    for (int t0 = 0; t0 < cap; t0 += CH) {
        const int nc = (cap - t0 < CH) ? cap - t0 : CH;
        X.rewind(mk, "chunk");
        float* pool1 = (float*)X.alloc((size_t)nc * d.P * d.P * d.C1 * 4);
        if (!pool1) { trl_set_error("%s workspace", d.name); return TRL_ERR_STATE; }
        if (!X.counting) TRL_CHECK(trl_launch_front(c, d, d_frames, H, W, d_total, t0, nc, pool1, s));
        TRL_CHECK(trl_run_net(c, X, d, d.tail, Act::dense(pool1, nc, d.P, d.P, d.C1), d_out + (size_t)t0 * d.nout, s, d_total, t0));
        if (X.counting) break;
    }
    return TRL_OK;
}

int trl_cascade_finish(trl_ctx* c, const uint8_t* d_frames, int n, int H, int W, float* d_boxes, float* d_probs, float* d_points,
                       int32_t* d_counts, float* d_box0, float* d_prob0, int32_t* d_rect, uint8_t* d_valid, float* d_pts0, hipStream_t s,
                       int order) {
    (void)d_frames;
    CascadeBufs& B = c->cb;
    k_select<<<n, 64, 0, s>>>(B.capF, c->cfg.max_faces, W, H, order, B.cnt[2], B.box[2], B.pts3, d_boxes, d_probs, d_points, d_counts, d_box0, d_prob0,
                              d_rect, d_valid, d_pts0);
    TRL_LAUNCH_CHECK();
    TRL_HIP(hipMemcpyAsync(c->h_pinned + 4, B.flags, TRL_NFLAGS * 4, hipMemcpyDeviceToHost, s));
    return TRL_OK;
}

int trl_cascade_check(trl_ctx* c, int n, int* retry) {
    *retry = trl_caps_check(c->caps, c->h_pinned + 4, n, c->cb.lay).retry;
    return TRL_OK;
}

int trl_cascade_lists(trl_ctx* c, int kind, int n, int H, int W, const int32_t* h_caps, int L, const int32_t* h_counts, const void* h_rows,
                      const float* h_logits, float* h_pts, float* d_boxes, float* d_probs, float* d_points, int32_t* d_counts, float* d_box0,
                      float* d_prob0, int32_t* d_rect, uint8_t* d_valid, hipStream_t s) {
    CascadeBufs& B = c->cb;
    B = CascadeBufs();
    LvLayout& G = B.lay;
    G.L = L;
    for (int l = 0; l < L; l++) { G.capl[l] = h_caps[l]; G.rec0[l] = G.S; G.S += h_caps[l]; }
    B.capF = h_caps[L];
    B.n = n; B.L = L; B.H = H; B.W = W;
    const int capF = B.capF, nc = kind == 1 ? n * L : n;
    long long total = 0;
    for (int i = 0; i < nc; i++) total += h_counts[i];
    const int carved = carve_lists(c, spill_pool(c, n, H, W), s);
    if (carved != TRL_OK) { B = CascadeBufs(); return carved; }
    const int poison = c->dbg_poison >= 0 ? c->dbg_poison : 0xA5;
    TRL_HIP(hipMemsetAsync(c->arena.base, poison, (size_t)((char*)B.flags - c->arena.base), s));
    std::vector<int32_t> cnt(h_counts, h_counts + nc);
    std::vector<float> logits;
    const int st = kind - 2;
    const int NO = kind == 1 ? 0 : trl_net_of(trl_stages[st].net).nout;
    if (kind == 1) {
        const Cand* src = (const Cand*)h_rows;
        TRL_HIP(hipMemcpyAsync(B.lvl_cnt, cnt.data(), (size_t)nc * 4, hipMemcpyHostToDevice, s));
        for (int f = 0; f < n; f++)
            for (int l = 0; l < L; l++) {
                const int k = cnt[f * L + l];
                if (k) TRL_HIP(hipMemcpyAsync(B.lvl_rec + (size_t)f * G.S + G.rec0[l], src, (size_t)k * sizeof(Cand), hipMemcpyHostToDevice, s));
                src += k;
            }
    } else {
        const float* src = (const float*)h_rows;
        float* rows = B.box[st];
        TRL_HIP(hipMemcpyAsync(B.cnt[st], cnt.data(), (size_t)n * 4, hipMemcpyHostToDevice, s));
        for (int f = 0; f < n; f++) {
            if (cnt[f]) TRL_HIP(hipMemcpyAsync(rows + (size_t)f * capF * 5, src, (size_t)cnt[f] * 20, hipMemcpyHostToDevice, s));
            src += 5 * (size_t)cnt[f];
        }
        logits.assign(h_logits, h_logits + (size_t)total * NO);
    }
    TRL_HIP(hipStreamSynchronize(s));
    const Spill sp{B.spill, (unsigned long long)B.spill_cap, B.flags};
    ListLaunch ll;
    TRL_CHECK(list_launch(c, ll));
    if (kind == 1) {
        TRL_CHECK(launch_stage1_lists(c, ll, n, H, W, sp, s));
    } else {
        const int cap = (int)total + 64;
        Arena& X = c->scratch;
        TRL_CHECK(trl_scratch_begin(c, (size_t)cap * NO * 4 + (1u << 20)));
        float* out = (float*)X.alloc((size_t)cap * NO * 4);
        if (!out) { trl_set_error("list hook net outputs"); return TRL_ERR_STATE; }
        TRL_HIP(hipMemsetAsync(out, poison, (size_t)cap * NO * 4, s));
        if (total) TRL_HIP(hipMemcpyAsync(out, logits.data(), logits.size() * 4, hipMemcpyHostToDevice, s));
        TRL_CHECK(launch_stage_scan(B, st, cap, s));
        TRL_CHECK(launch_stage_post(c, ll, st, cap, out, sp, s));
        if (kind == 3) {
            TRL_CHECK(trl_cascade_finish(c, nullptr, n, H, W, d_boxes, d_probs, d_points, d_counts, d_box0, d_prob0, d_rect, d_valid, nullptr, s));
        }
        TRL_HIP(hipStreamSynchronize(s));
    }
    if (kind != 3) TRL_HIP(hipMemcpyAsync(c->h_pinned + 4, B.flags, TRL_NFLAGS * 4, hipMemcpyDeviceToHost, s));
    if (kind == 3 && h_pts) TRL_HIP(hipMemcpyAsync(h_pts, B.pts3, (size_t)n * capF * 40, hipMemcpyDeviceToHost, s));
    TRL_HIP(hipStreamSynchronize(s));
    c->caps.last_attempts = 1;
    const int32_t* fl = c->h_pinned + 4;
    if (fl[FLG_LEVEL] || fl[FLG_FRAME] || fl[FLG_SPILL]) {
        trl_set_error("list hook: a capacity was too small (level %d, frame %d, spill %d)", fl[FLG_LEVEL], fl[FLG_FRAME], fl[FLG_SPILL]);
        return TRL_ERR_CAPACITY;
    }
    return TRL_OK;
}
```

truely-real-time-ai-generated-video-detection-framework-for-social-platforms_amd/csrc/trl_ctx.h:

```cpp
#pragma once
#include "trl_common.h"
#include "trl_capacity.h"
#include "trl_facenet.h"

struct Cand {
    float x1, y1, x2, y2, score;
    float r0, r1, r2, r3;
    int cell;
};

struct LevelGeom {
    double scale;
    int h, w;
    int oh, ow;
    int chunk;
};

struct CascadeBufs {
    int n = 0, L = 0, H = 0, W = 0;
    LvLayout lay;
    int capF = 0;
    int32_t* lvl_cnt = nullptr;
    Cand* lvl_rec = nullptr;
    int32_t* lvl_keep_cnt = nullptr;
    int32_t* lvl_keep_idx = nullptr;
    int32_t* cnt[3] = {nullptr, nullptr, nullptr};
    float* box[3] = {nullptr, nullptr, nullptr};
    float* pts3 = nullptr;
    int32_t* off[2] = {nullptr, nullptr};
    int32_t* cbox = nullptr;
    int32_t* flags = nullptr;
    char* spill = nullptr;
    size_t spill_cap = 0;
    float* box0 = nullptr; float* prob0 = nullptr; int32_t* rect = nullptr; uint8_t* valid = nullptr; float* pts0 = nullptr;
};
struct NetLayer { const char* name; const char* prelu; int k, st, cout; };
struct trl_ctx;
struct NetDesc {
    const char* name;
    int side;
    int nl; NetLayer layer[9];
    int tail;
    int P, C1;
    int nout;
    int trl_ctx::*chunk;
};
enum { TRL_PNET = 0, TRL_RNET = 1, TRL_ONET = 2 };
extern const NetDesc trl_nets[3];
inline const NetDesc& trl_net_of(int net) { return trl_nets[net == 24 ? TRL_RNET : TRL_ONET]; }
struct NetLayerW { const DevW* w = nullptr; const float* b = nullptr; const float* slope = nullptr; };
struct FnW { const DevW* w = nullptr; const float* scale = nullptr; const float* shift = nullptr; const float* bias = nullptr; };

struct trl_ctx {
    trl_config cfg;
    bool have_weights = false;
    char* wdev = nullptr;
    size_t wbytes = 0;
    std::vector<DevW> wmat;
    NetLayerW mt[3][9];
    FnW fn[FN_ROWS];
    int front_mode[3] = {0, 0, 0};
    const DevW* logits_w = nullptr;
    const float* logits_b = nullptr;
    int num_classes = 0;
    Arena arena;
    Arena scratch;
    size_t arena_need = 0;
    int fn_need_key[6] = {0}; size_t fn_need_bytes = 0;
    Arena sims_tmp;
    int32_t* h_pinned = nullptr;
    CascadeBufs cb;
    LevelGeom lv[32];
    hipEvent_t ev_call0 = nullptr, ev_call1 = nullptr;
    std::vector<std::pair<hipEvent_t, hipEvent_t>> pnet_ev;
    int pnet_ev_used = 0;
    float last_ms[4] = {0, 0, 0, 0};
    int pnet_mono1 = 0;
    int pnet_unit = 0;
    float pnet_scrA = 0.f, pnet_scrB = 0.f;
    float pnet_scrG[16] = {};
    int pnet_screen_ok = 0;
    int pnet_screen = 1;
    int pnet_run = 0;
    int32_t* pnet_cursor = nullptr;
    unsigned long long* pnet_clk = nullptr;
    bool pnet_prof = false;
    float pnet_kernel_ms = 0.f;
    int dbg_poison = -1;
    struct RedZone {
        size_t guard = 0; int byte = 0, saved_poison = -1;
        long long sweeps = 0, bytes = 0, nhits = 0;
        std::vector<trl_rz_hit> hits;
        unsigned long long* dev = nullptr; size_t dev_gaps = 0;
    } rz;
    CascadeCaps caps;
    int rnet_chunk = 49152, onet_chunk = 16384;
    int tail_pool = 1;
    int nms_small = 512, nms_full = 2048;
    size_t scratch_after_cascade = 0;
    struct Pending {
        enum Kind { EMBED, CROP, DETECT };
        bool active = false; int attempt = 0; Kind kind = EMBED;
        const uint8_t* frames = nullptr; int n = 0, H = 0, W = 0;
        void* stream = nullptr;
        float* box = nullptr; float* prob = nullptr; int32_t* rect = nullptr; uint8_t* valid = nullptr; float* emb = nullptr;
        float* faces_out = nullptr;
        float* boxes = nullptr; float* probs = nullptr; float* points = nullptr; int32_t* counts = nullptr; int order = 0;
    } pend;
    uint32_t* pyr_tab = nullptr;
    int pyr_tab_H = 0, pyr_tab_W = 0;
    int pyr_row_bands = 0;
    struct { int nlev = 0, own0 = 0, band_cols = 0, strip_rows = 0, n_bands = 0, n_strips = 0; } pyr_fine;
    struct { int L = 0; int32_t row[16][TRL_PYR_PLAN_COLS] = {}; } pyr_plan;
    std::vector<trl_fn_plan_row> fn_plan;
    std::vector<trl_fn_plan_row> mt_plan;
    bool mt_plan_arm = false;
    int fn_cap_arm = -1;
    struct { void* p = nullptr; size_t cap = 0; int32_t dims[5] = {0, 0, 0, 0, 0}; } fn_cap[3];
};

struct TrlConvChoice { int family = 0, bm = 0, bn = 0, bk = 0, pad = 0, nz = 1; };
extern thread_local TrlConvChoice g_trl_conv_choice;

int trl_gate_wait(trl_ctx* c, hipStream_t s);
int trl_gate_record(trl_ctx* c, hipStream_t s);
extern int g_trl_pnet_gate;
int trl_ensure(trl_ctx* c, Arena& a, size_t bytes);
inline int trl_scratch_begin(trl_ctx* c, size_t bytes) { c->scratch.reset("scratch_begin"); c->scratch.high = 0; return trl_ensure(c, c->scratch, bytes); }
int trl_rz_sweep_all(trl_ctx* c, const char* site);
inline int trl_rz_end(trl_ctx* c, const char* site) { return c->rz.guard ? trl_rz_sweep_all(c, site) : TRL_OK; }
template <class F> int trl_carve_scratch(trl_ctx* c, F&& carve) {
    Arena X = Arena::counter(c->scratch.guard);
    TRL_CHECK(carve(X)); TRL_CHECK(trl_scratch_begin(c, X.high));
    return carve(c->scratch);
}
int trl_check_idle(trl_ctx* c);
void trl_free_weights(trl_ctx* c);

int trl_run_facenet(trl_ctx* c, Arena& X, const float* d_faces, int n, int h, int w, const uint8_t* d_valid, float* d_emb, hipStream_t s,
                    bool features = false);
int trl_run_net(trl_ctx* c, Arena& X, const NetDesc& d, int first, const Act& x, float* d_out, hipStream_t s, const int32_t* m_dev = nullptr,
                int m_base = 0);
inline const float* trl_host_of(const trl_ctx* c, const char* himg, const float* dev) { return (const float*)(himg + ((const char*)dev - c->wdev)); }
int trl_front_slope_class(const float* h_slope, int n);
int trl_launch_front(trl_ctx* c, const NetDesc& d, const uint8_t* d_frames, int H, int W, const int32_t* d_total, int t0, int nc, float* d_pool, hipStream_t s);
int trl_stage_net(trl_ctx* c, Arena& X, int net, const uint8_t* d_frames, int H, int W, const int32_t* d_total, int cap, float* d_out, hipStream_t s);

int trl_cascade_detect(trl_ctx* c, const uint8_t* d_frames, int n, int H, int W, hipStream_t s, int resume = 0);
int trl_cascade_finish(trl_ctx* c, const uint8_t* d_frames, int n, int H, int W, float* d_boxes, float* d_probs, float* d_points,
                       int32_t* d_counts, float* d_box0, float* d_prob0, int32_t* d_rect, uint8_t* d_valid, float* d_pts0, hipStream_t s,
                       int order = 0);
int trl_cascade_check(trl_ctx* c, int n, int* retry);
int trl_cascade_lists(trl_ctx* c, int kind, int n, int H, int W, const int32_t* h_caps, int L, const int32_t* h_counts, const void* h_rows,
                      const float* h_logits, float* h_pts, float* d_boxes, float* d_probs, float* d_points, int32_t* d_counts, float* d_box0,
                      float* d_prob0, int32_t* d_rect, uint8_t* d_valid, hipStream_t s);
int trl_launch_area_level(const uint8_t* d_frames, int nf, int H, int W, int h, int w, float* d_level, hipStream_t s);
int trl_launch_heads_to_maps(const float* d_heads, int cells, float* d_prob, float* d_reg, hipStream_t s);
int trl_compute_levels(trl_ctx* c, int H, int W);
int trl_launch_crop_resize80(const uint8_t* d_frames, int n, int H, int W, const int32_t* d_rect, const uint8_t* d_valid,
                             float* d_faces, hipStream_t s);
int trl_launch_crop_aligned(const uint8_t* d_frames, int n, int H, int W, const float* d_pts0, const uint8_t* d_valid, int S, bool rgb,
                            float* d_faces, hipStream_t s);
int trl_launch_crop_area_std(const uint8_t* d_frames, int n, int H, int W, const int32_t* d_rect, const uint8_t* d_valid, int S,
                             bool rgb, float* d_faces, hipStream_t s);
int trl_pnet_generic_level(trl_ctx* c, Arena& X, const uint8_t* d_frames, int nf, int H, int W, const LevelGeom& g, float** d_heads, hipStream_t s);
int trl_pnet_prepare(trl_ctx* c, const char* himg);
size_t trl_pnet_fused_bytes(trl_ctx* c, int n, int H, int W);
int trl_pnet_fused_all(trl_ctx* c, const uint8_t* d_frames, int n, int H, int W, hipEvent_t* ev, hipStream_t s);
int trl_pyramid_export(trl_ctx* c, const uint8_t* d_frame, int H, int W, int level, float* d_out, int* h, int* w, hipStream_t s);
int trl_pyramid_export_batch(trl_ctx* c, const uint8_t* d_frames, int n, int H, int W, float* d_out, long long* pyr_stride,
                             int32_t* h_levels, int max_levels, int* n_levels, hipStream_t s);
```

truely-real-time-ai-generated-video-detection-framework-for-social-platforms_amd/csrc/trl_pnet.hip:

```cpp
#include "trl_pyramid.h"
#include <stdlib.h>
#include <type_traits>

typedef float f32x4 __attribute__((ext_vector_type(4)));
typedef float f32x16 __attribute__((ext_vector_type(16)));
typedef _Float16 f16x8 __attribute__((ext_vector_type(8)));

namespace {

constexpr int TS = 16;
constexpr int IN_T = 2 * TS + 10;
constexpr int P1_T = TS + 4;
constexpr int C2_T = TS + 2;
constexpr int C2_LD = 17;
constexpr int REGION_A = C2_T * C2_T * C2_LD;
constexpr int REGION_B = P1_T * P1_T * 10 + 224;
static_assert(3 * 7 * 256 <= REGION_A, "input tile (+ the 28 overhang pixels of the 7x256 copy) fits region A");
static_assert(P1_T * P1_T * 10 <= REGION_B, "pooled tile fits region B");
constexpr int SCR_XM = 2 * C2_T * C2_T * 4;
constexpr int CARRY_P = P1_T * 4 * 10;
constexpr int CARRY_C = C2_T * 2 * C2_LD;
constexpr int BAND = 3;
constexpr int VCARRY_P = 4 * P1_T * 10;
constexpr int VCARRY_C = 2 * C2_T * C2_LD;
constexpr int DYN_LDS = (144 * 32 + BAND * (CARRY_P + CARRY_C) + VCARRY_P + VCARRY_C) * 4;
static_assert((144 * 32) % 4 == 0 && CARRY_P % 4 == 0 && CARRY_C % 4 == 0 && VCARRY_P % 4 == 0, "strips stay 16-byte aligned");

struct PLevel {
    int h, w, oh, ow;
    int tiles_x, tile0;
    int tiles_y;
    unsigned bmagic;
    int pix0;
    int kept0[9];
    unsigned txmagic;
    int kept1[19];
    float scale;
    int cap, rec0;
};
static_assert(sizeof(PLevel) == 164 && offsetof(PLevel, txmagic) == 72 && offsetof(PLevel, scale) == 152, "k_pnet_fused's argument layout");
struct PnetArgs {
    const PyrPx* pyr; long long pyr_stride;
    int n_frames, L, tiles_per_frame, H, W;
    unsigned tpf_magic;
    long long kept;
    PLevel lv[16];
    const float *w1, *w2, *w3, *wh;
    const float *b1, *b2, *b3, *bh, *s1, *s2, *s3;
    float thr; int rec_stride;
    float dthr;
    float scrB; int screen;
    float scrG[16];
    int dbg_skip;
    int32_t* lvl_cnt; Cand* lvl_rec; int32_t* flags;
    int32_t* xcd_next;
    int run;
    unsigned long long* clk;
    int prof;
};


template <int D, int E>
__device__ __forceinline__ int koff(int s, int kq, int e1, int e2, int e3) {
    const int q0 = (4 * s) / D, r0 = (4 * s) % D, thr = D - r0;
    const int add = thr == 1 ? e1 : (thr == 2 ? e2 : (thr == 3 ? e3 : 0));
    return 4 * s + E * q0 + kq + add;
}

template <bool UNIT>
__device__ __forceinline__ float prelu_t(float v, float sl, float sel) { return UNIT ? vmax_nc(v, sl * v) : trl_prelu_med3(v, sl, sel); }
template <bool UNIT>
__device__ __forceinline__ float prelu_pooled_t(float m, float n, float sl, float sel) {
    return UNIT ? vmax_nc(m, sl * (sl < 0.f ? n : m)) : trl_prelu_pooled(m, n, sl, sel);
}

template <int CB, int AB>
__device__ __forceinline__ f32x4 mfma4(float a, float b, f32x4 c) { return __builtin_amdgcn_mfma_f32_4x4x1f32(a, b, c, CB, AB, 0); }
__device__ __forceinline__ void quad_max4(const f32x4& v, float (&o)[4]) {
    float t0, t1, t2, t3;
    asm("v_max_f32_dpp %4, %8, %8 quad_perm:[1,0,3,2] row_mask:0xf bank_mask:0xf\n\t"
        "v_max_f32_dpp %5, %9, %9 quad_perm:[1,0,3,2] row_mask:0xf bank_mask:0xf\n\t"
        "v_max_f32_dpp %6, %10, %10 quad_perm:[1,0,3,2] row_mask:0xf bank_mask:0xf\n\t"
        "v_max_f32_dpp %7, %11, %11 quad_perm:[1,0,3,2] row_mask:0xf bank_mask:0xf\n\t"
        "v_max_f32_dpp %0, %4, %4 quad_perm:[2,3,0,1] row_mask:0xf bank_mask:0xf\n\t"
        "v_max_f32_dpp %1, %5, %5 quad_perm:[2,3,0,1] row_mask:0xf bank_mask:0xf\n\t"
        "v_max_f32_dpp %2, %6, %6 quad_perm:[2,3,0,1] row_mask:0xf bank_mask:0xf\n\t"
        "v_max_f32_dpp %3, %7, %7 quad_perm:[2,3,0,1] row_mask:0xf bank_mask:0xf"
        : "=&v"(o[0]), "=&v"(o[1]), "=&v"(o[2]), "=&v"(o[3]), "=&v"(t0), "=&v"(t1), "=&v"(t2), "=&v"(t3)
        : "v"(v[0]), "v"(v[1]), "v"(v[2]), "v"(v[3]));
}
__device__ __forceinline__ void quad_min4(const f32x4& v, float (&o)[4]) {
    float t0, t1, t2, t3;
    asm("v_min_f32_dpp %4, %8, %8 quad_perm:[1,0,3,2] row_mask:0xf bank_mask:0xf\n\t"
        "v_min_f32_dpp %5, %9, %9 quad_perm:[1,0,3,2] row_mask:0xf bank_mask:0xf\n\t"
        "v_min_f32_dpp %6, %10, %10 quad_perm:[1,0,3,2] row_mask:0xf bank_mask:0xf\n\t"
        "v_min_f32_dpp %7, %11, %11 quad_perm:[1,0,3,2] row_mask:0xf bank_mask:0xf\n\t"
        "v_min_f32_dpp %0, %4, %4 quad_perm:[2,3,0,1] row_mask:0xf bank_mask:0xf\n\t"
        "v_min_f32_dpp %1, %5, %5 quad_perm:[2,3,0,1] row_mask:0xf bank_mask:0xf\n\t"
        "v_min_f32_dpp %2, %6, %6 quad_perm:[2,3,0,1] row_mask:0xf bank_mask:0xf\n\t"
        "v_min_f32_dpp %3, %7, %7 quad_perm:[2,3,0,1] row_mask:0xf bank_mask:0xf"
        : "=&v"(o[0]), "=&v"(o[1]), "=&v"(o[2]), "=&v"(o[3]), "=&v"(t0), "=&v"(t1), "=&v"(t2), "=&v"(t3)
        : "v"(v[0]), "v"(v[1]), "v"(v[2]), "v"(v[3]));
}
__device__ __forceinline__ float lane_sel(float if0, float if1, unsigned long long mask) {
    float r;
    asm("v_cndmask_b32_e64 %0, %1, %2, %3" : "=v"(r) : "v"(if0), "v"(if1), "s"(mask));
    return r;
}
template <int... I, typename F>
__device__ __forceinline__ void pn_static_for(std::integer_sequence<int, I...>, F&& f) { (f(std::integral_constant<int, I>{}), ...); }

template <bool UNIT, bool NEG1, bool DBG>
__global__ __launch_bounds__(256, 2) void k_pnet_fused(PnetArgs a) {
    __shared__ __attribute__((aligned(16))) float RA[REGION_A];
    __shared__ __attribute__((aligned(16))) float RB[REGION_B];
    __shared__ __attribute__((aligned(16))) float T3all[108];
    extern __shared__ __attribute__((aligned(16))) float DYN[];
    float* const B3S = DYN;
    float* const CP0 = DYN + 144 * 32;
    float* const VP = CP0 + BAND * (CARRY_P + CARRY_C);
    float* const VC = VP + VCARRY_P;

    const int tid = threadIdx.x, lane = tid & 63;
    const int wave = __builtin_amdgcn_readfirstlane(tid >> 6);
    const int dbg_skip = DBG ? a.dbg_skip : 0;
    if (DBG && tid == 0) atomicMin(&a.clk[0], (unsigned long long)wall_clock64());
    const int l15 = lane & 15, kq = lane >> 4;
    const int l31 = lane & 31, hh = lane >> 5;

    for (int i = tid; i < 144 * 32; i += 256) B3S[i] = a.w3[i];
    float B2[23], WH[4];
#pragma unroll
    for (int s = 0; s < 23; s++) B2[s] = a.w2[(4 * s + kq) * 32 + l15];
#pragma unroll
    for (int r = 0; r < 4; r++) WH[r] = a.wh[(((lane >> 2) & 7) + 8 * r) * 32 + 4 * (lane >> 5) + (lane & 3)];
    const float bias2 = a.b2[l15], slope2 = a.s2[l15];
    if (tid < 32) { T3all[tid] = a.b3[tid]; T3all[32 + tid] = a.s3[tid]; if (tid < 8) T3all[64 + tid] = a.bh[tid]; }
    if (tid < 32) { T3all[72 + tid] = a.wh[tid * 32 + 1] - a.wh[tid * 32]; if (tid == 0) T3all[104] = a.bh[1] - a.bh[0]; }
    const float sel2 = trl_prelu_sel(slope2);
    const f32x4 bias2v = {bias2, bias2, bias2, bias2};

    for (int i = tid; i < REGION_A; i += 256) RA[i] = 0.f;
    for (int i = tid; i < REGION_B; i += 256) RB[i] = 0.f;
    __syncthreads();

    const int e2_2 = kq >= 2 ? 170 : 0;
    const int xb = lane >> 2, xj = lane & 3, xdy = xj >> 1, xdx = xj & 1;
    float WC[3][2];
#pragma unroll
    for (int cg = 0; cg < 3; cg++)
#pragma unroll
        for (int h = 0; h < 2; h++) {
            const int k = xb + 16 * h;
            WC[cg][h] = k < 27 ? a.w1[k * 32 + 4 * cg + xj] : (k == 27 ? a.b1[4 * cg + xj] : 0.f);
        }
    float xone = 1.0f;
    asm volatile("" : "+v"(xone));
    const int xcg = xj < 3 ? xj : 2;
    const float sl4[4] = {a.s1[4 * xcg], a.s1[4 * xcg + 1], a.s1[4 * xcg + 2], a.s1[4 * xcg + 3]};
    const int c1x_w = ((2 * wave + xdy) * IN_T + 8 + 2 * xb + xdx) * 3;
    const int c1x_sw = (wave * P1_T + 4 + xb) * 10 + 4 * xj;
    const int c1s_l = ((2 * wave + 8 * xj) * IN_T + 8 + 2 * xb) * 3;
    const int c1s_s = ((wave + 4 * xj) * P1_T + 4 + xb) * 10;

    const int total_tiles = a.tiles_per_frame * a.n_frames;
    const int xcd = blockIdx.x & 7;
    const int chunk = (total_tiles + 7) / 8;
    const int t_begin = xcd * chunk, t_end = (t_begin + chunk < total_tiles) ? t_begin + chunk : total_tiles;

    const int lvl_t0v = lane < a.L ? a.lv[lane < 16 ? lane : 15].tile0 : 0x7fffffff;
    auto sdiv = [](int n, unsigned magic, int d) {
        int q = (int)__umulhi((unsigned)n, magic);
        if (q * d > n) q--;
        if (n - q * d >= d) q++;
        return q;
    };
    struct TileId { int f, l, ty, tx, h, w, oh, ow, tiles_x, pix0, rib, rows; float scale; };
    auto decode = [&](int tile) {
        TileId t;
        const int tpf = __builtin_amdgcn_readfirstlane(a.tiles_per_frame);
        t.f = __builtin_amdgcn_readfirstlane(sdiv(tile, __builtin_amdgcn_readfirstlane(a.tpf_magic), tpf));
        const int tt = tile - t.f * tpf;
        t.l = __popcll(__ballot(tt >= lvl_t0v)) - 1;
        const PLevel& g = a.lv[t.l];
        t.h = g.h; t.w = g.w; t.oh = g.oh; t.ow = g.ow; t.tiles_x = g.tiles_x; t.pix0 = g.pix0; t.scale = g.scale;
        const int tq = tt - g.tile0;
        const int band = sdiv(tq, g.bmagic, BAND * t.tiles_x);
        const int rb = tq - band * (BAND * t.tiles_x);
        t.rows = g.tiles_y - BAND * band < BAND ? g.tiles_y - BAND * band : BAND;
        static_assert(BAND == 2 || BAND == 3, "column of a band position: rb / rows for rows in 1..3");
        t.tx = __builtin_amdgcn_readfirstlane(t.rows == 3 ? (rb * 43691) >> 17 : (t.rows == 2 ? rb >> 1 : rb));
        t.rib = rb - t.tx * t.rows;
        t.ty = BAND * band + t.rib;
        return t;
    };
    const int pin_iy0 = tid / IN_T, pin_ix0 = tid - pin_iy0 * IN_T;
    int ctid = tid;
    float4 pre[7];
    auto issue_input = [&](const TileId& t) {
        const TileId& g = t;
        const int gy0 = t.ty * 2 * TS, gx0 = t.tx * 2 * TS;
        const char* srcb = reinterpret_cast<const char*>(a.pyr + (long long)t.f * a.pyr_stride + g.pix0 + (long long)gy0 * g.w + gx0);
        const int w16 = g.w * 12;
        const int hrem = g.h - gy0, wrem = g.w - gx0;
        int iy0 = pin_iy0, ix0 = pin_ix0;
        asm volatile("" : "+v"(iy0), "+v"(ix0));
        if (hrem >= IN_T && wrem >= IN_T) {
            const unsigned v0 = (unsigned)(iy0 * w16 + ix0 * 12);
#pragma unroll
            for (int i = 0; i < 7; i++) {
                unsigned vo = v0 + (unsigned)(i * (6 * w16 + 48)) + ((ix0 >= IN_T - 4 * i) ? (unsigned)(w16 - IN_T * 12) : 0u);
                if (i == 6) vo = (ctid < IN_T * IN_T - 6 * 256) ? vo : 0u;
                { const f32x3_nt v3 = *reinterpret_cast<const f32x3_nt*>(srcb + vo); pre[i] = make_float4(v3[0], v3[1], v3[2], 0.f); }
            }
        } else {
#pragma unroll
            for (int i = 0; i < 7; i++) {
                const bool wrap = ix0 >= IN_T - 4 * i;
                const int iy = iy0 + 6 * i + (wrap ? 1 : 0), ix = ix0 + 4 * i - (wrap ? IN_T : 0);
                const bool ok = iy < hrem && ix < wrem && (i < 6 || ctid < IN_T * IN_T - 6 * 256);
                pre[i] = make_float4(0.f, 0.f, 0.f, 0.f);
                if (ok) { const f32x3_nt v3 = *reinterpret_cast<const f32x3_nt*>(srcb + (unsigned)(iy * w16 + ix * 12)); pre[i] = make_float4(v3[0], v3[1], v3[2], 0.f); }
            }
        }
    };
    typedef float f32x2c __attribute__((ext_vector_type(2)));
    auto copy_pooled = [&](auto SAVE_T, float* CP) {
        constexpr bool SAVE = decltype(SAVE_T)::value;
        const int q = ctid & 15;
#pragma unroll
        for (int pass = 0; pass < 2; pass++) {
            const int r = (ctid >> 4) + 16 * pass;
            if (q < 10 && (pass == 0 || ctid < 64)) {
                f32x4* t = reinterpret_cast<f32x4*>(RB + r * (P1_T * 10) + (SAVE ? 16 * 10 : 0) + 4 * q);
                f32x4* c = reinterpret_cast<f32x4*>(CP + r * 40 + 4 * q);
                if (SAVE) *c = *t; else *t = *c;
            }
        }
    };
    auto copy_conv2 = [&](auto SAVE_T, float* CC) {
        constexpr bool SAVE = decltype(SAVE_T)::value;
        const int q = ctid & 31;
#pragma unroll
        for (int pass = 0; pass < 3; pass++) {
            const int r = (ctid >> 5) + 8 * pass;
            if (q < 17 && (pass < 2 || ctid < 64)) {
                f32x2c* t = reinterpret_cast<f32x2c*>(RA + r * (C2_T * C2_LD) + (SAVE ? 16 * C2_LD : 0) + 2 * q);
                f32x2c* c = reinterpret_cast<f32x2c*>(CC + r * 34 + 2 * q);
                if (SAVE) *c = *t; else *t = *c;
            }
        }
    };
    auto copy_rows = [&](auto SAVE_T) {
        constexpr bool SAVE = decltype(SAVE_T)::value;
        if (ctid < VCARRY_P / 4) {
            f32x4* t = reinterpret_cast<f32x4*>(RB + (SAVE ? 16 * P1_T * 10 : 0)) + ctid;
            f32x4* c = reinterpret_cast<f32x4*>(VP) + ctid;
            if (SAVE) *c = *t; else *t = *c;
        }
    };
    auto copy_rows2 = [&](auto SAVE_T) {
        constexpr bool SAVE = decltype(SAVE_T)::value;
        static_assert((16 * C2_T * C2_LD) % 4 == 0 && VCARRY_C % 4 == 0, "float4 copies");
        if (ctid < VCARRY_C / 4) {
            f32x4* t = reinterpret_cast<f32x4*>(RA + (SAVE ? 16 * C2_T * C2_LD : 0)) + ctid;
            f32x4* c = reinterpret_cast<f32x4*>(VC) + ctid;
            if (SAVE) *c = *t; else *t = *c;
        }
    };
    __shared__ int next_tile_s;
    int run_len = a.run;
    if (tid == 0) next_tile_s = t_begin + atomicAdd(&a.xcd_next[xcd], run_len);
    __syncthreads();
    int tile = __builtin_amdgcn_readfirstlane(next_tile_s);
    __syncthreads();
    TileId cur = decode(tile < t_end ? tile : 0), nxt = cur;
    if (tile < t_end) issue_input(cur);
    int rot = 0, tile_nxt = tile, run_pos = 0;
    int hs_tile[BAND], vs_tile = -1;
#pragma unroll
    for (int i = 0; i < BAND; i++) hs_tile[i] = -1;
    unsigned long long pt[8] = {0, 0, 0, 0, 0, 0, 0, 0}, pt_last = 0;
    const bool prof = DBG && a.prof != 0;
    auto stamp = [&](int k) {
        if (DBG && prof) { const unsigned long long t = clock64(); pt[k] += t - pt_last; pt_last = t; }
    };
    if (DBG && prof) pt_last = clock64();
    unsigned nscr = 0, ncnf = 0;
// ... 179 lines not shown
                const bool two = pr == 2 && !carry && !vcarry;
                if (fast) { if (two) x_units(std::false_type{}, std::true_type{}, A, B); else x_units(std::false_type{}, std::false_type{}, A, B); }
                else { if (two) x_units(std::true_type{}, std::true_type{}, A, B); else x_units(std::true_type{}, std::false_type{}, A, B); }
            }
        }
        stamp(2);
        __syncthreads();
        stamp(3);

        if (!(dbg_skip & 4)) {
            const int w2 = (wave + rot) & 3;
            const int lim2 = C2_T * (vrows + 3 < C2_T ? vrows + 3 : C2_T);
            if (feeds_next) copy_pooled(std::true_type{}, CP);
            if (feeds_down) copy_rows(std::true_type{});
            if (vcarry) copy_rows2(std::false_type{});
            if (carry) copy_conv2(std::false_type{}, CC);
            const int r0 = vcarry ? 2 : 0;
            float xa[23], xb[23];
            if (carry) {
                const int rows2 = vrows + 3 < C2_T ? vrows + 3 : C2_T;
                const int cbase = (2 + l15) * 10;
                auto read_rows = [&](int j) {
                    int yA = r0 + w2 + 8 * j;
                    yA = yA < C2_T ? yA : C2_T - 1;
                    const int yB = (yA + 4 < C2_T) ? yA + 4 : yA;
#pragma unroll
                    for (int s = 0; s < 23; s++) xa[s] = RB[yA * (P1_T * 10) + cbase + koff<30, 170>(s, kq, 0, e2_2, 0)];
                    if (yA + 4 < C2_T) {
#pragma unroll
                        for (int s = 0; s < 23; s++) xb[s] = RB[yB * (P1_T * 10) + cbase + koff<30, 170>(s, kq, 0, e2_2, 0)];
                    }
                };
                read_rows(0);
#pragma unroll
                for (int j = 0; j < 3; j++) {
                    const int yA = r0 + w2 + 8 * j, yB = yA + 4;
                    const bool hasA = yA < rows2, hasB = yB < rows2;
                    f32x4 accA = bias2v, accB = bias2v;
                    __builtin_amdgcn_sched_barrier(0);
                    if (!hasA) {
                    } else if (hasB) {
                        accA = __builtin_amdgcn_mfma_f32_16x16x4f32(xa[0], B2[0], bias2v, 0, 0, 0);
                        accB = __builtin_amdgcn_mfma_f32_16x16x4f32(xb[0], B2[0], bias2v, 0, 0, 0);
#pragma unroll
                        for (int s = 1; s < 23; s++) {
                            accA = __builtin_amdgcn_mfma_f32_16x16x4f32(xa[s], B2[s], accA, 0, 0, 0);
                            accB = __builtin_amdgcn_mfma_f32_16x16x4f32(xb[s], B2[s], accB, 0, 0, 0);
                        }
                    } else {
                        accA = __builtin_amdgcn_mfma_f32_16x16x4f32(xa[0], B2[0], bias2v, 0, 0, 0);
#pragma unroll
                        for (int s = 1; s < 23; s++) accA = __builtin_amdgcn_mfma_f32_16x16x4f32(xa[s], B2[s], accA, 0, 0, 0);
                    }
                    __builtin_amdgcn_sched_barrier(0);
                    if (j < 2) read_rows(j + 1);
                    __builtin_amdgcn_sched_barrier(0);
#pragma unroll
                    for (int q = 0; q < 4; q++) {
                        if (hasA) RA[(yA * C2_T + 2 + kq * 4 + q) * C2_LD + l15] = prelu_t<UNIT>(accA[q], slope2, sel2);
                        if (hasB) RA[(yB * C2_T + 2 + kq * 4 + q) * C2_LD + l15] = prelu_t<UNIT>(accB[q], slope2, sel2);
                    }
                }
            } else {
            const int c0 = r0 * C2_T, nmt2 = vcarry ? 18 : 21;
            auto read_pair2 = [&](int j) {
                const int mtA = w2 + 8 * j, mtB = (mtA + 4 < 21) ? mtA + 4 : mtA;
                int mA = c0 + mtA * 16 + l15; mA = mA < 324 ? mA : 323;
                int mB = c0 + mtB * 16 + l15; mB = mB < 324 ? mB : 323;
                const int yA = mA / C2_T, xA = mA - yA * C2_T, yB = mB / C2_T, xB = mB - yB * C2_T;
                const int baseA = (yA * P1_T + xA) * 10, baseB = (yB * P1_T + xB) * 10;
#pragma unroll
                for (int s = 0; s < 23; s++) xa[s] = RB[baseA + koff<30, 170>(s, kq, 0, e2_2, 0)];
                if (j < 2 || w2 == 0) {
#pragma unroll
                    for (int s = 0; s < 23; s++) xb[s] = RB[baseB + koff<30, 170>(s, kq, 0, e2_2, 0)];
                }
            };
            read_pair2(0);
#pragma unroll
            for (int j = 0; j < 3; j++) {
                const int mtA = w2 + 8 * j, mtB = mtA + 4;
                const bool hasB = mtB < nmt2 && c0 + 16 * mtB < lim2;
                const bool hasA = mtA < nmt2 && c0 + 16 * mtA < lim2;
                f32x4 accA = bias2v, accB = bias2v;
                __builtin_amdgcn_sched_barrier(0);
                if (!hasA) {
                } else if (hasB) {
                    accA = __builtin_amdgcn_mfma_f32_16x16x4f32(xa[0], B2[0], bias2v, 0, 0, 0);
                    accB = __builtin_amdgcn_mfma_f32_16x16x4f32(xb[0], B2[0], bias2v, 0, 0, 0);
#pragma unroll
                    for (int s = 1; s < 23; s++) {
                        accA = __builtin_amdgcn_mfma_f32_16x16x4f32(xa[s], B2[s], accA, 0, 0, 0);
                        accB = __builtin_amdgcn_mfma_f32_16x16x4f32(xb[s], B2[s], accB, 0, 0, 0);
                    }
                } else {
                    accA = __builtin_amdgcn_mfma_f32_16x16x4f32(xa[0], B2[0], bias2v, 0, 0, 0);
#pragma unroll
                    for (int s = 1; s < 23; s++) accA = __builtin_amdgcn_mfma_f32_16x16x4f32(xa[s], B2[s], accA, 0, 0, 0);
                }
                __builtin_amdgcn_sched_barrier(0);
                if (j < 2) read_pair2(j + 1);
                __builtin_amdgcn_sched_barrier(0);
#pragma unroll
                for (int q = 0; q < 4; q++) {
                    const int ra = c0 + mtA * 16 + kq * 4 + q;
                    if (hasA && ra < 324) RA[ra * C2_LD + l15] = prelu_t<UNIT>(accA[q], slope2, sel2);
                    const int rb = c0 + mtB * 16 + kq * 4 + q;
                    if (hasB && rb < 324) RA[rb * C2_LD + l15] = prelu_t<UNIT>(accB[q], slope2, sel2);
                }
            }
            }
        }
        if (tid == 0) next_tile_s = t_begin + cursor;
        stamp(4);
        __syncthreads();
        stamp(5);

        if (a.screen) {
            static_assert(SCR_XM + 2 * 324 <= P1_T * P1_T * 10, "fp16 conv2 tile + error weights stay inside the pooled tile");
#pragma unroll
            for (int p = 0; p < 3; p++) {
                const int half = p < 2 ? p : wave >> 1;
                int cell = ctid;
                if (p == 2) { cell = ctid & 127; cell = 256 + (cell < 324 - 256 ? cell : 324 - 256 - 1); }
                const int i = 324 * half + cell;
                const float* src = RA + cell * C2_LD + 8 * half;
                const float* gs = a.scrG + 8 * half;
                f16x8 hv;
                float m = 0.f, mx = 0.f;
#pragma unroll
                for (int j = 0; j < 8; j++) {
                    const float v = src[j], av = fabsf(v);
                    mx = fmaxf(mx, av);
                    m = __builtin_fmaf(gs[j], av, m);
                    hv[j] = (_Float16)v;
                }
                *reinterpret_cast<f16x8*>(RB + 4 * i) = hv;
                RB[SCR_XM + i] = mx > 65504.f ? 3.402823466e38f : fminf(m, 3.402823466e38f);
                __builtin_amdgcn_sched_barrier(0);
            }
            __syncthreads();
        }

        tile_nxt = __builtin_amdgcn_readfirstlane(next_tile_s);
        if (tile_nxt < t_end) { nxt = decode(tile_nxt); if (!(dbg_skip & 1)) issue_input(nxt); }
        auto strips_get = [&]() __attribute__((always_inline)) {
            if (feeds_next) copy_conv2(std::true_type{}, CC);
            if (feeds_down) copy_rows2(std::true_type{});
        };

        if (!(dbg_skip & 8)) {
            const float fscale = g.scale;
            const f32x4* T3 = reinterpret_cast<const f32x4*>(T3all);
            auto conv3 = [&](int mt, f32x16& P, auto&& between) __attribute__((always_inline)) {
                const int y = mt * 2 + (l31 >> 4), x = l31 & 15;
                const int base = (y * C2_T + x) * C2_LD + hh;
                f32x16 acc;
#pragma unroll
                for (int qa = 0; qa < 4; qa++) {
                    const f32x4 b4 = T3[2 * qa + hh];
                    acc[4 * qa] = b4[0]; acc[4 * qa + 1] = b4[1]; acc[4 * qa + 2] = b4[2]; acc[4 * qa + 3] = b4[3];
                }
                float xa[2][12], wb[2][12];
                auto read_sixth = [&](int sx, float* xo, float* wo) {
#pragma unroll
                    for (int u = 0; u < 12; u++) {
                        const int s = sx * 12 + u, tap = s >> 3, ky = tap / 3, kx = tap - ky * 3;
                        xo[u] = RA[base + (ky * C2_T + kx) * C2_LD + 2 * (s & 7)];
                        wo[u] = B3S[(2 * s + hh) * 32 + l31];
                    }
                };
                read_sixth(0, xa[0], wb[0]);
                pn_static_for(std::make_integer_sequence<int, 6>{}, [&](auto SX) __attribute__((always_inline)) {
                    constexpr int sx = decltype(SX)::value;
                    if (sx < 5) read_sixth(sx + 1, xa[(sx + 1) & 1], wb[(sx + 1) & 1]);
                    __builtin_amdgcn_sched_barrier(0);
                    pn_static_for(std::make_integer_sequence<int, 12>{}, [&](auto UU) __attribute__((always_inline)) {
                        constexpr int u = decltype(UU)::value;
                        acc = __builtin_amdgcn_mfma_f32_32x32x2f32(wb[sx & 1][u], xa[sx & 1][u], acc, 0, 0, 0);
                        between(SX, UU);
                    });
                    __builtin_amdgcn_sched_barrier(0);
                });
#pragma unroll
                for (int qa = 0; qa < 4; qa++) {
                    const f32x4 s4 = T3[8 + 2 * qa + hh];
#pragma unroll
                    for (int qb = 0; qb < 4; qb++) P[4 * qa + qb] = prelu_t<UNIT>(acc[4 * qa + qb], s4[qb], UNIT ? 0.f : trl_prelu_sel(s4[qb]));
                }
            };
            unsigned hlo[4], hhi[4];
            auto head_step = [&](auto H_T, const f32x16& P, f32x4& hq) __attribute__((always_inline)) {
                constexpr int k = decltype(H_T)::value, ga = k >> 3, gb = k & 7;
                if constexpr (gb == 0) {
#pragma unroll
                    for (int qb = 0; qb < 4; qb++) {
                        const unsigned v = __float_as_uint(P[4 * ga + qb]);
                        const auto r = __builtin_amdgcn_permlane32_swap(v, v, false, false);
                        hlo[qb] = r[0]; hhi[qb] = r[1];
                    }
                }
                const float bk = __uint_as_float(gb < 4 ? hlo[gb & 3] : hhi[gb & 3]);
                hq = __builtin_amdgcn_mfma_f32_4x4x1f32(WH[ga], bk, hq, 3, gb, 0);
            };
            auto heads_all = [&](const f32x16& P, f32x4& hq) __attribute__((always_inline)) {
                pn_static_for(std::make_integer_sequence<int, 32>{}, [&](auto H_T) __attribute__((always_inline)) { head_step(H_T, P, hq); });
            };
            auto emit = [&](int mt, const f32x4& hq) __attribute__((always_inline)) {
                if (__builtin_amdgcn_ballot_w64(lane < 32 && hq[1] - hq[0] >= a.dthr) == 0) return;
                const float p = trl_softmax2_p1(hq[0], hq[1]);
                const auto u2 = __builtin_amdgcn_permlane32_swap(__float_as_uint(hq[0]), __float_as_uint(hq[0]), false, false);
                const auto u3 = __builtin_amdgcn_permlane32_swap(__float_as_uint(hq[1]), __float_as_uint(hq[1]), false, false);
                if (lane < 32) {
                    const int oy = ty * TS + mt * 2 + (lane >> 4), ox = tx * TS + (lane & 15);
                    if (oy < g.oh && ox < g.ow) {
                        if (p >= a.thr && !(dbg_skip & 32)) {
                            const int seg = f * a.L + l;
                            const int sl = atomicAdd(&a.lvl_cnt[seg], 1);
                            if (sl < a.lv[l].cap) {
                                Cand c;
                                c.x1 = floorf((2.f * (float)ox + 1.f) / fscale);
                                c.y1 = floorf((2.f * (float)oy + 1.f) / fscale);
                                c.x2 = floorf((2.f * (float)ox + 12.f) / fscale);
                                c.y2 = floorf((2.f * (float)oy + 12.f) / fscale);
                                c.score = p;
                                c.r0 = hq[2]; c.r1 = hq[3]; c.r2 = __uint_as_float(u2[1]); c.r3 = __uint_as_float(u3[1]);
                                c.cell = oy * g.ow + ox;
                                a.lvl_rec[(size_t)f * a.rec_stride + a.lv[l].rec0 + sl] = c;
                            } else {
                                a.flags[FLG_LEVEL] = 1;
                            }
                        }
                    }
                }
            };
            const int mt0 = wave, mt1 = wave + 4;
            const bool has0 = 2 * mt0 < vrows, has1 = 2 * mt1 < vrows;
            bool cf0 = has0, cf1 = has1;
            if (has0 && a.screen) {
                const int sb0 = 324 * hh + (mt0 * 2 + (l31 >> 4)) * C2_T + (l31 & 15);
                auto screen = [&](int mt, int sb) __attribute__((always_inline)) {
                    f32x16 S;
#pragma unroll
                    for (int qa = 0; qa < 4; qa++) {
                        const f32x4 b4 = T3[2 * qa + hh];
#pragma unroll
                        for (int qb = 0; qb < 4; qb++) S[4 * qa + qb] = b4[qb];
                    }
                    float em = 0.f;
#pragma unroll
                    for (int tap = 0; tap < 9; tap++) {
                        const int to = (tap / 3) * C2_T + tap % 3;
                        f16x8 wv;
#pragma unroll
                        for (int j = 0; j < 8; j++) wv[j] = (_Float16)B3S[(tap * 16 + 8 * hh + j) * 32 + l31];
                        const f16x8 xv = *reinterpret_cast<const f16x8*>(RB + 4 * (sb + to));
                        em += RB[SCR_XM + sb + to];
                        S = __builtin_amdgcn_mfma_f32_32x32x16_f16(wv, xv, S, 0, 0, 0);
                    }
                    float part = 0.f;
#pragma unroll
                    for (int qa = 0; qa < 4; qa++) {
                        const f32x4 s4 = T3[8 + 2 * qa + hh], w4 = T3[18 + 2 * qa + hh];
#pragma unroll
                        for (int qb = 0; qb < 4; qb++)
                            part = __builtin_fmaf(w4[qb], prelu_t<UNIT>(S[4 * qa + qb], s4[qb], UNIT ? 0.f : trl_prelu_sel(s4[qb])), part);
                    }
                    const auto pp = __builtin_amdgcn_permlane32_swap(__float_as_uint(part), __float_as_uint(part), false, false);
                    const auto px = __builtin_amdgcn_permlane32_swap(__float_as_uint(em), __float_as_uint(em), false, false);
                    const float d = (part + __uint_as_float(pp[1])) + T3all[104];
                    const float E = (em + __uint_as_float(px[1])) + a.scrB;
                    const int oy = ty * TS + mt * 2 + (lane >> 4), ox = tx * TS + (lane & 15);
                    const bool hit = !(d + E < a.dthr) || !(fabsf(d) <= 3.402823466e38f) || !(E < 3.402823466e38f);
                    return __builtin_amdgcn_ballot_w64(lane < 32 && oy < g.oh && ox < g.ow && hit) != 0;
                };
                cf0 = screen(mt0, sb0);
                if (has1) cf1 = screen(mt1, sb0 + 8 * C2_T);
                if (DBG) { nscr += has1 ? 2 : 1; ncnf += (cf0 ? 1 : 0) + (cf1 ? 1 : 0); }
            }
            if (cf0 && cf1) {
                f32x16 P0;
                f32x4 hq0 = T3[16 + hh];
                conv3(mt0, P0, [](auto, auto) {});
                {
                    f32x16 P1;
                    f32x4 hq1 = T3[16 + hh];
                    conv3(mt1, P1, [&](auto SX, auto UU) __attribute__((always_inline)) {
                        constexpr int sx = decltype(SX)::value, u = decltype(UU)::value, h = sx * 6 + (u >> 1);
                        if constexpr ((u & 1) == 1 && h < 32) {
                            __builtin_amdgcn_sched_barrier(0);
                            head_step(std::integral_constant<int, h>{}, P0, hq0);
                            __builtin_amdgcn_sched_barrier(0);
                        }
                    });
                    strips_get();
                    heads_all(P1, hq1);
                    emit(mt0, hq0);
                    emit(mt1, hq1);
                }
            } else if (cf0 || cf1) {
                const int mt = cf0 ? mt0 : mt1;
                f32x16 P0;
                f32x4 hq0 = T3[16 + hh];
                conv3(mt, P0, [](auto, auto) {});
                strips_get();
                heads_all(P0, hq0);
                emit(mt, hq0);
            } else {
                strips_get();
            }
        } else {
            strips_get();
        }
        stamp(6);
        __syncthreads();
        stamp(7);
    }
    if (DBG && prof && lane == 0) {
#pragma unroll
        for (int k = 0; k < 8; k++) atomicAdd(&a.clk[2 + 8 * wave + k], pt[k]);
        if (wave == 0) atomicAdd(&a.clk[2 + 32], (unsigned long long)rot);
    }
    if (DBG && lane == 0 && nscr) { atomicAdd(&a.clk[39], (unsigned long long)nscr); atomicAdd(&a.clk[40], (unsigned long long)ncnf); }
    if (DBG && tid == 0) atomicMax(&a.clk[1], (unsigned long long)wall_clock64());
}

}

__global__ void k_pnet_span(unsigned long long* clk) {
    const unsigned long long t0 = clk[0], t1 = clk[1];
    const unsigned long long d = t1 > t0 ? t1 - t0 : 0ull;
    clk[36] += d; clk[37] += 1ull; clk[38] = d;
    clk[0] = ~0ull; clk[1] = 0ull;
}

static void pnet_screen_bound(trl_ctx* c, const float* W, const float* H, const float* b3, const float* s3, const float* bh) {
    c->pnet_screen_ok = 0; c->pnet_scrA = c->pnet_scrB = __builtin_inff();
    for (int i = 0; i < 16; i++) c->pnet_scrG[i] = __builtin_inff();
    for (int i = 0; i < 144 * 32; i++) if (!(fabsf(W[i]) <= 65504.f)) return;
    const double u = ldexp(1.0, -24), uh = ldexp(1.0, -11), tiny = ldexp(1.0, -14);
    auto gamma = [](int n, double uu) { return n * uu / (1.0 - n * uu); };
    const double ge = gamma(145, u), gs = gamma(145, 2 * u), g35 = gamma(35, u), g36 = gamma(36, u);
    double Sa = 0, Sb = fabs((double)bh[0]) + fabs((double)bh[1]);
    double ad = 0, bd = 0, wdP_a = 0, wdP_b = 0;
    double g[144] = {};
    for (int co = 0; co < 32; co++) {
        double W1 = 0, D = 0;
        for (int k = 0; k < 144; k++) {
            const double w = W[k * 32 + co], aw = fabs(w);
            W1 += aw;
            D += aw < tiny ? aw : fabs((double)(float)(_Float16)W[k * 32 + co] - w);
        }
        const double b = fabs((double)b3[co]), L = fmax(1.0, fabs((double)s3[co]));
        const double a3 = D * (1 + uh) + W1 * uh + gs * (W1 + D) * (1 + uh) + ge * W1;
        const double b3e = D * tiny + W1 * tiny + gs * (b + (W1 + D) * tiny) + ge * b;
        const double aM = W1 * (1 + ge), bM = b * (1 + ge);
        const double ap = L * (1 + u) * a3 + 2 * u * L * aM, bp = L * (1 + u) * b3e + 2 * u * L * bM;
        const double aP = L * (1 + u) * aM, bP = L * (1 + u) * bM;
        const double w0 = H[co * 32 + 0], w1 = H[co * 32 + 1], wd = fabs(w1 - w0);
        Sa += (fabs(w0) + fabs(w1)) * aP; Sb += (fabs(w0) + fabs(w1)) * bP;
        ad += wd * ap; bd += wd * bp;
        wdP_a += wd * (aP + ap); wdP_b += wd * (bP + bp);
        for (int k = 0; k < 144; k++) {
            const double w = W[k * 32 + co], aw = fabs(w), Dk = aw < tiny ? aw : fabs((double)(float)(_Float16)W[k * 32 + co] - w);
            const double a3k = Dk * (1 + uh) + aw * uh + gs * (aw + Dk) * (1 + uh) + ge * aw, aMk = aw * (1 + ge);
            const double apk = L * (1 + u) * a3k + 2 * u * L * aMk, aPk = L * (1 + u) * aMk;
            g[k] += g35 * (fabs(w0) + fabs(w1)) * aPk + wd * apk + g36 * (1 + u) * wd * (aPk + apk);
        }
    }
    ad += g36 * (1 + u) * wdP_a;
    bd += g36 * (1 + u) * (fabs((double)bh[1] - (double)bh[0]) + wdP_b);
    const double A = (g35 * Sa + ad) * (1 + ldexp(1.0, -10)), B = (g35 * Sb + bd) * (1 + ldexp(1.0, -10));
    auto up = [](double v) { float f = (float)v; return (double)f < v ? nextafterf(f, __builtin_inff()) : f; };
    c->pnet_scrA = up(A); c->pnet_scrB = up(B); c->pnet_screen_ok = 1;
    for (int ci = 0; ci < 16; ci++) {
        double m = 0;
        for (int tap = 0; tap < 9; tap++) m = fmax(m, g[tap * 16 + ci]);
        c->pnet_scrG[ci] = up(m * (1 + ldexp(1.0, -10)));
    }
}

enum { PN_CONV1 = 0, PN_CONV2 = 2, PN_CONV3 = 3, PN_HEADS = 4 };

int trl_pnet_prepare(trl_ctx* c, const char* himg) {
    const NetLayerW* l = c->mt[TRL_PNET];
    auto host = [&](const float* dev) { return trl_host_of(c, himg, dev); };
    c->pnet_mono1 = c->pnet_unit = 1;
    for (int i : {PN_CONV1, PN_CONV2, PN_CONV3}) {
        const float* sl = host(l[i].slope);
        for (int k = 0; k < l[i].w->Cout; k++) {
            if (i == PN_CONV1 && !(sl[k] >= 0.f)) c->pnet_mono1 = 0;
            if (!(sl[k] <= 1.f)) c->pnet_unit = 0;
        }
    }
    pnet_screen_bound(c, host(l[PN_CONV3].w->p), host(l[PN_HEADS].w->p), host(l[PN_CONV3].b), host(l[PN_CONV3].slope), host(l[PN_HEADS].b));
    return TRL_OK;
}

static unsigned sdiv_magic(int d) { return d <= 1 ? 0xFFFFFFFFu : (unsigned)((0x100000000ull + (unsigned)d - 1) / (unsigned)d); }

static void fill_args(trl_ctx* c, int n, int H, int W, const PyrLayout& lay, const PyrPx* pyr, PnetArgs& a) {
    a.pyr = pyr; a.pyr_stride = lay.pyr_stride;
    a.n_frames = n; a.L = lay.L; a.H = H; a.W = W;
    int tiles = 0;
    for (int l = 0; l < lay.L; l++) {
        const LevelGeom& g = c->lv[l];
        PLevel& p = a.lv[l];
        p.h = g.h; p.w = g.w; p.oh = g.oh; p.ow = g.ow;
        p.tiles_x = (g.ow + TS - 1) / TS;
        p.txmagic = sdiv_magic(p.tiles_x);
        p.tile0 = tiles;
        p.tiles_y = (g.oh + TS - 1) / TS;
        p.bmagic = sdiv_magic(BAND * p.tiles_x);
        tiles += p.tiles_x * p.tiles_y;
        p.pix0 = lay.lv[l].pix0;
        p.scale = (float)g.scale;
        p.cap = c->cb.lay.capl[l]; p.rec0 = c->cb.lay.rec0[l];
    }
    a.tiles_per_frame = tiles;
    a.tpf_magic = sdiv_magic(tiles);
    const NetLayerW* l = c->mt[TRL_PNET];
    a.w1 = l[PN_CONV1].w->p; a.w2 = l[PN_CONV2].w->p; a.w3 = l[PN_CONV3].w->p; a.wh = l[PN_HEADS].w->p;
    a.b1 = l[PN_CONV1].b; a.b2 = l[PN_CONV2].b; a.b3 = l[PN_CONV3].b; a.bh = l[PN_HEADS].b;
    a.s1 = l[PN_CONV1].slope; a.s2 = l[PN_CONV2].slope; a.s3 = l[PN_CONV3].slope;
    a.thr = c->cfg.thr0; a.rec_stride = c->cb.lay.S;
    a.dthr = (a.thr >= 0.01f && a.thr <= 0.99f) ? (float)(log((double)a.thr / (1.0 - (double)a.thr)) - 0.05) : -__builtin_inff();
    a.scrB = c->pnet_scrB; a.screen = c->pnet_screen && c->pnet_screen_ok;
    for (int i = 0; i < 16; i++) a.scrG[i] = c->pnet_scrG[i];
    a.dbg_skip = trl_tune_int("TRL_PNET_SKIP", 0);
    a.lvl_cnt = c->cb.lvl_cnt; a.lvl_rec = c->cb.lvl_rec; a.flags = c->cb.flags;
    a.clk = c->pnet_clk; a.prof = c->pnet_prof ? 1 : 0;
    a.xcd_next = c->pnet_cursor;
}

size_t trl_pnet_fused_bytes(trl_ctx* c, int n, int H, int W) {
    PyrLayout lay;
    if (trl_pyramid_layout(c, H, W, lay) != TRL_OK) return 0;
    return trl_pyramid_bytes(lay, n) + 4096;
}

int trl_pnet_fused_all(trl_ctx* c, const uint8_t* d_frames, int n, int H, int W, hipEvent_t* ev, hipStream_t s) {
    PyrLayout lay;
    PyrPx* pyr = nullptr;
    TRL_CHECK(trl_pyramid_build(c, d_frames, n, H, W, lay, &pyr, ev, s));
    PnetArgs a;
    fill_args(c, n, H, W, lay, pyr, a);
    const int total_tiles = a.tiles_per_frame * n;
    int grid = 256 * 2;
    if (grid > ((total_tiles + 7) / 8) * 8) grid = ((total_tiles + 7) / 8) * 8;
    if (grid < 8) grid = 8;
    TRL_HIP(hipMemsetAsync(c->pnet_cursor, 0, 8 * sizeof(int32_t), s));
    TRL_CHECK(trl_gate_wait(c, s));
    if (ev) TRL_HIP(hipEventRecord(ev[2], s));
#ifdef TRL_TUNING
    const bool dbg = c->pnet_prof || a.dbg_skip || trl_tune_set("TRL_PNET_SPAN");
#else
    const bool dbg = false;
#endif
    const int auto_run = (total_tiles / 8) / 128;
    a.run = c->pnet_run > 0 ? c->pnet_run : (auto_run < 1 ? 1 : (auto_run > 8 * BAND ? 8 * BAND : auto_run));
    auto launch = [&](auto kern) {
        if (hipFuncSetAttribute((const void*)kern, hipFuncAttributeMaxDynamicSharedMemorySize, DYN_LDS) != hipSuccess) return false;
        kern<<<grid, 256, DYN_LDS, s>>>(a);
        return true;
    };
    bool launched = false;
#ifdef TRL_TUNING
#define TRL_PK(U, N) do { launched = dbg ? launch(k_pnet_fused<U, N, true>) : launch(k_pnet_fused<U, N, false>); } while (0)
#else
#define TRL_PK(U, N) do { launched = launch(k_pnet_fused<U, N, false>); } while (0)
#endif
    if (c->pnet_unit) { if (c->pnet_mono1) TRL_PK(true, false); else TRL_PK(true, true); }
    else { if (c->pnet_mono1) TRL_PK(false, false); else TRL_PK(false, true); }
#undef TRL_PK
    if (!launched) { trl_set_error("k_pnet_fused: %d bytes of dynamic LDS refused", DYN_LDS); return TRL_ERR_HIP; }
    TRL_LAUNCH_CHECK();
    if (ev) TRL_HIP(hipEventRecord(ev[3], s));
    if (dbg) {
        k_pnet_span<<<1, 1, 0, s>>>(c->pnet_clk);
        TRL_LAUNCH_CHECK();
    }
    return TRL_OK;
}
```

truely-real-time-ai-generated-video-detection-framework-for-social-platforms_amd/engine.py:

```python
from __future__ import annotations

import ctypes as C
from typing import Optional

import numpy as np
import torch

from . import _lib
from . import weights as _weights


SELECTION_METHODS = {"largest": 0, "probability": 1, "largest_over_threshold": 2, "center_weighted_size": 3}
RESAMPLERS = {"torch": 0, "pil": 1, "cv2": 2}


def _ptr(t: Optional[torch.Tensor]):
    return C.c_void_p(t.data_ptr()) if t is not None else C.c_void_p(0)


class Engine:
    def __init__(self, blob: bytes | None = None, device: int | None = None, pnet_mode: int | None = None,
                 cap_level: int | None = None, cap_frame: int | None = None, min_face_size: int = 20,
                 thresholds=(0.6, 0.7, 0.7), factor: float = 0.709, max_faces: int = 64, embed_mode: int = 0,
                 embed_precision: str | int = 0):
# ... 244 lines not shown
        nv12 = nv12.to(self.device).contiguous()
        if nv12.dtype != torch.uint8 or nv12.dim() != 2 or nv12.shape[1] != H * W * 3 // 2:
            raise ValueError("nv12 must be uint8 (n, H*W*3/2)")
        n_in = int(nv12.shape[0])
        n_out = (n_in + step - 1) // step
        out = torch.empty((n_out, H, W, 3), dtype=torch.uint8, device=self.device)
        k = C.c_int()
        fn = self.lib.trl_ingest_i420 if planar else self.lib.trl_ingest_nv12
        _lib.check(fn(self._h, _ptr(nv12), n_in, H, W, int(step), _ptr(out), C.byref(k), self._stream()))
        assert k.value == n_out
        return out

    def drift_score(self, emb: torch.Tensor, valid: torch.Tensor, frame_count: int, fps: int):
        emb = emb.to(self.device, torch.float32).contiguous()
        valid = valid.to(self.device, torch.uint8).contiguous()
        n = int(valid.shape[0])
        sims = torch.empty((n,), dtype=torch.float32, device=self.device)
        flags = torch.empty((n,), dtype=torch.uint8, device=self.device)
        res = torch.zeros((4,), dtype=torch.int32, device=self.device)
        _lib.check(self.lib.trl_drift_score(self._h, _ptr(emb), _ptr(valid), n, int(frame_count), int(fps), _ptr(sims), _ptr(flags),
                                            _ptr(res), self._stream()))
        r = res.cpu().tolist()
        return {"score": r[0], "run": r[1], "hits": r[2], "total": r[3], "sims": sims, "flags": flags}

    DRIFT_STATE_BYTES = 2064

    def drift_state(self) -> torch.Tensor:
        return torch.zeros((self.DRIFT_STATE_BYTES,), dtype=torch.uint8, device=self.device)

    def drift_update(self, state: torch.Tensor, emb: torch.Tensor | None, valid: torch.Tensor | None, frame_count: int, fps: int,
                     want_flags: bool = True, sync: bool = True):
        n = 0 if emb is None else int(emb.shape[0])
        d = self.device
        if n:
            emb = emb.to(d, torch.float32).contiguous(); valid = valid.to(d, torch.uint8).contiguous()
        sims = torch.empty((n,), dtype=torch.float32, device=d)
        flags = torch.empty((n,), dtype=torch.uint8, device=d) if want_flags else None
        res = torch.empty((4,), dtype=torch.int32, device=d)
        _lib.check(self.lib.trl_drift_update(self._h, _ptr(state), _ptr(emb) if n else C.c_void_p(0), _ptr(valid) if n else C.c_void_p(0), n,
                                             int(frame_count), int(fps), _ptr(sims), _ptr(flags), _ptr(res), self._stream()))
        out = {"sims": sims, "flags": flags, "result": res}
        if sync:
            r = res.cpu().tolist()
            out.update(score=r[0], run=r[1], hits=r[2], total=r[3])
        return out

    def stage_boxes(self, stage: int, frame: int, max_rows: int | None = None) -> np.ndarray:
        k = C.c_int()
        if max_rows is None:
            _lib.check(self.lib.trl_debug_stage_boxes(self._h, stage, frame, None, 0, C.byref(k)))
            max_rows = max(1, k.value)
        buf = np.zeros((max_rows, 5), np.float32)
        _lib.check(self.lib.trl_debug_stage_boxes(self._h, stage, frame, buf.ctypes.data_as(C.c_void_p), max_rows, C.byref(k)))
        return buf[:min(k.value, max_rows)].copy()

    def pyramid_level(self, frame, level: int) -> torch.Tensor:
        fr = self._frames(frame[None] if getattr(frame, "ndim", 4) == 3 else frame)
        _, H, W, _ = fr.shape
        m = 12.0 / self.cfg.min_face_size
        out = torch.empty((int(H * m + 1) * int(W * m + 1) * 3,), dtype=torch.float32, device=self.device)
        h, w = C.c_int(), C.c_int()
        _lib.check(self.lib.trl_debug_pyramid_level(self._h, _ptr(fr), H, W, int(level), _ptr(out), C.byref(h), C.byref(w), self._stream()))
        return out[:h.value * w.value * 3].view(h.value, w.value, 3)

    def pyramid_batch(self, frames):
        fr = self._frames(frames)
        n, H, W, _ = fr.shape
        stride, L = C.c_longlong(), C.c_int()
        lv = np.zeros((16, 4), np.int32)
        _lib.check(self.lib.trl_debug_pyramid_batch(self._h, _ptr(fr), n, H, W, None, C.byref(stride), lv.ctypes.data_as(C.c_void_p), 16,
                                                    C.byref(L), self._stream()))
        out = torch.empty((n, stride.value, 3), dtype=torch.float32, device=self.device)
        _lib.check(self.lib.trl_debug_pyramid_batch(self._h, _ptr(fr), n, H, W, _ptr(out), C.byref(stride), lv.ctypes.data_as(C.c_void_p), 16,
                                                    C.byref(L), self._stream()))
        levels = [dict(zip(("pix0", "h", "w", "pix_pad"), (int(v) for v in lv[l]))) for l in range(L.value)]
        return out, levels

    PYR_KERNELS = {1: "F", 2: "S4", 3: "S8", 4: "SW4", 5: "SW8", 6: "L0-3", 7: "L0-4", 8: "L0-5", 9: "L1", 10: "L2"}

    def pyramid_plan(self):
        rows = np.zeros((16, 6), np.int32)
        L = C.c_int()
        _lib.check(self.lib.trl_debug_pyramid_plan(self._h, rows.ctypes.data_as(C.c_void_p), 16, C.byref(L)))
        keys = ("row_bands", "col_bands", "cols_per_band", "frames_per_launch", "khmax")
        return [dict(kernel=self.PYR_KERNELS[int(r[0])], **dict(zip(keys, (int(v) for v in r[1:])))) for r in rows[:L.value]]

    FN_FAMILIES = {1: "fn_conv", 2: "fn_conv_split4", 3: "conv_tap", 4: "conv_igemm_vec", 5: "conv_igemm_scalar",
                   6: "conv_splitk4", 7: "conv_splitk4_tap", 8: "conv_tap48", 9: "conv_bf16"}
    FN_PLAN_DTYPE = np.dtype([(k, np.int32) for k in ("conv", "family", "bm", "bn", "bk", "pad", "nz", "m", "cout", "k", "precision",
                                                      "has_res")] + [("layer", "S48")])

    def facenet_plan(self):
        return self._plan_rows(self.lib.trl_debug_facenet_plan)

    def mtcnn_plan(self):
        return self._plan_rows(self.lib.trl_debug_mtcnn_plan)

    def _plan_rows(self, fn):
        n = C.c_int()
        _lib.check(fn(self._h, None, 0, C.byref(n)))
        rows = np.zeros(n.value, self.FN_PLAN_DTYPE)
        _lib.check(fn(self._h, rows.ctypes.data_as(C.c_void_p), n.value, C.byref(n)))
        out = []
        for r in rows:
            d = {k: int(r[k]) for k in self.FN_PLAN_DTYPE.names if k != "layer"}
            d["family"] = self.FN_FAMILIES[d["family"]]
            d["layer"] = r["layer"].decode()
            out.append(d)
        return out

    def facenet_capture(self, conv_index: int):
        _lib.check(self.lib.trl_debug_facenet_capture(self._h, int(conv_index)))

    def facenet_captured(self):
        out = []
        for v in range(3):
            dims = np.zeros(5, np.int32)
            _lib.check(self.lib.trl_debug_facenet_capture_read(self._h, v, None, 0, dims.ctypes.data_as(C.c_void_p)))
            if dims[3] == 0:
                out.append(None)
                continue
            a = np.empty(tuple(int(d) for d in dims[:4]), np.float32 if dims[4] == 4 else np.uint16)
            _lib.check(self.lib.trl_debug_facenet_capture_read(self._h, v, a.ctypes.data_as(C.c_void_p), a.nbytes,
                                                               dims.ctypes.data_as(C.c_void_p)))
            out.append(a)
        return tuple(out)

    def batch_capacity(self, t2_per_frame: float = 0.0, t3_per_frame: float = 0.0) -> int:
        k = C.c_int()
        _lib.check(self.lib.trl_debug_batch_capacity(self._h, float(t2_per_frame), float(t3_per_frame), C.byref(k)))
        return k.value

    def option(self, key: str, value: int):
        _lib.check(self.lib.trl_debug_option(self._h, key.encode(), int(value)))

    def nms_tiers(self, small: int = 0, full: int = 0):
        _lib.check(self.lib.trl_debug_nms_tiers(self._h, int(small), int(full)))

    def list_stats(self) -> dict:
        t = (C.c_longlong * 8)()
        _lib.check(self.lib.trl_debug_list_stats(self._h, t))
        keys = ("attempts", "spill_lists", "spill_used", "spill_cap", "cap_frame", "slots_per_frame", "max_level_count", "max_frame_total")
        return dict(zip(keys, (int(v) for v in t)))

    def pnet_screen_bound(self):
        A, B, on = C.c_float(), C.c_float(), C.c_int()
        _lib.check(self.lib.trl_debug_pnet_screen_bound(self._h, C.byref(A), C.byref(B), C.byref(on)))
        return float(A.value), float(B.value), bool(on.value)

    def pnet_screen_weights(self):
        g = (C.c_float * 16)()
        _lib.check(self.lib.trl_debug_pnet_screen_weights(self._h, g))
        return [float(v) for v in g]

    def pnet_run(self, run: int = 0):
        _lib.check(self.lib.trl_debug_pnet_run(self._h, int(run)))

    def stage_totals(self):
        t = (C.c_int32 * 2)()
        _lib.check(self.lib.trl_debug_stage_totals(self._h, t))
        return int(t[0]), int(t[1])

    def workspace(self, what: int = 0, n: int = 0, h: int = 0, w: int = 0) -> dict:
        o = (C.c_longlong * 6)()
        _lib.check(self.lib.trl_debug_workspace(self._h, int(what), int(n), int(h), int(w), o))
        return dict(zip(("scratch_cap", "scratch_high", "arena_cap", "arena_off", "arena_need", "need"), (int(v) for v in o)))

    def poison_workspaces(self, byte: int = 0xFF):
        _lib.check(self.lib.trl_debug_poison(self._h, int(byte)))

    def redzone(self, guard: int, byte: int = 0xA5):
        _lib.check(self.lib.trl_debug_redzone(self._h, int(guard), int(byte)))

    def redzone_report(self, clear: bool = False, sweep: bool = False) -> dict:
        o = (C.c_longlong * 4)()
        hits = (_lib.TrlRzHit * 256)()
        _lib.check(self.lib.trl_debug_redzone_report(self._h, (1 if clear else 0) | (2 if sweep else 0), o, hits, 256))
        rows = [dict(arena=int(h.arena), site=h.site.decode(), block=int(h.block), block_bytes=int(h.block_bytes), gap_off=int(h.gap_off),
                     gap_bytes=int(h.gap_bytes), first=int(h.first), last=int(h.last), count=int(h.count)) for h in hits[:int(o[3])]]
        return dict(sweeps=int(o[0]), bytes=int(o[1]), nhits=int(o[2]), hits=rows)

    def redzone_poke(self, arena: int, block: int, offset: int, value: int = 0x3C):
        _lib.check(self.lib.trl_debug_redzone_poke(self._h, int(arena), int(block), int(offset), int(value)))

    def level_counts(self, frame: int):
        a = np.zeros(32, np.int32); b = np.zeros(32, np.int32)
        L = C.c_int()
        _lib.check(self.lib.trl_debug_level_counts(self._h, frame, a.ctypes.data_as(C.c_void_p), b.ctypes.data_as(C.c_void_p), C.byref(L)))
        return a[:L.value].tolist(), b[:L.value].tolist()

    CAND_DTYPE = np.dtype([("box", np.float32, 4), ("score", np.float32), ("reg", np.float32, 4), ("cell", np.int32)])

    def level_keep(self, frame: int, level: int):
        k = C.c_int()
        _lib.check(self.lib.trl_debug_level_cands(self._h, int(frame), int(level), None, 0, C.byref(k)))
        rec = np.zeros((max(1, k.value),), self.CAND_DTYPE)
        _lib.check(self.lib.trl_debug_level_cands(self._h, int(frame), int(level), rec.ctypes.data_as(C.c_void_p), len(rec), C.byref(k)))
        rec = rec[:k.value]
        _lib.check(self.lib.trl_debug_level_keep(self._h, int(frame), int(level), None, 0, C.byref(k)))
        idx = np.zeros((max(1, k.value),), np.int32)
        _lib.check(self.lib.trl_debug_level_keep(self._h, int(frame), int(level), idx.ctypes.data_as(C.c_void_p), len(idx), C.byref(k)))
        return rec, idx[:k.value]

    def level_cands(self, frame: int, level: int) -> np.ndarray:
        k = C.c_int()
        _lib.check(self.lib.trl_debug_level_cands(self._h, int(frame), int(level), None, 0, C.byref(k)))
        buf = np.zeros((max(1, k.value),), self.CAND_DTYPE)
        _lib.check(self.lib.trl_debug_level_cands(self._h, int(frame), int(level), buf.ctypes.data_as(C.c_void_p), len(buf), C.byref(k)))
        rows = buf[:min(k.value, len(buf))]
        return rows[np.argsort(rows["cell"], kind="stable")].copy()

    def pnet_level(self, frame, level: int):
        fr = self._frames(frame[None] if frame.ndim == 3 else frame)
        _, H, W, _ = fr.shape
        prob = torch.empty((H * W,), dtype=torch.float32, device=self.device)
        reg = torch.empty((H * W * 4,), dtype=torch.float32, device=self.device)
        oh, ow = C.c_int(), C.c_int()
        _lib.check(self.lib.trl_debug_pnet_level(self._h, _ptr(fr), H, W, level, _ptr(prob), _ptr(reg), C.byref(oh), C.byref(ow), self._stream()))
        k = oh.value * ow.value
        return prob[:k].reshape(oh.value, ow.value), reg[:4 * k].reshape(oh.value, ow.value, 4)

    def rnet(self, crops: torch.Tensor) -> torch.Tensor:
        crops = crops.to(self.device, torch.float32).contiguous()
        out = torch.empty((crops.shape[0], 6), dtype=torch.float32, device=self.device)
        _lib.check(self.lib.trl_debug_rnet(self._h, _ptr(crops), crops.shape[0], _ptr(out), self._stream()))
        return out

    def onet(self, crops: torch.Tensor) -> torch.Tensor:
        crops = crops.to(self.device, torch.float32).contiguous()
        out = torch.empty((crops.shape[0], 16), dtype=torch.float32, device=self.device)
        _lib.check(self.lib.trl_debug_onet(self._h, _ptr(crops), crops.shape[0], _ptr(out), self._stream()))
        return out

    def front_net(self, frame, boxes: np.ndarray, net: int) -> torch.Tensor:
        fr = self._frames(frame[None] if getattr(frame, "ndim", 4) == 3 else frame)
        _, H, W, _ = fr.shape
        b = np.ascontiguousarray(boxes, np.float32).reshape(-1, 4)
        out = torch.empty((len(b), 6 if net == 24 else 16), dtype=torch.float32, device=self.device)
        _lib.check(self.lib.trl_debug_front_net(self._h, _ptr(fr), H, W, b.ctypes.data_as(C.c_void_p), len(b), int(net), _ptr(out), self._stream()))
        return out

    def stage_net(self, frames, recs: np.ndarray, net: int, capacity: int, fill: float | None = None) -> torch.Tensor:
        fr = self._frames(frames)
        nf, H, W, _ = fr.shape
        r = np.ascontiguousarray(recs, np.float32).reshape(-1, 5)
        shape = (int(capacity), 6 if net == 24 else 16)
        out = torch.empty(shape, dtype=torch.float32, device=self.device) if fill is None else \
            torch.full(shape, fill, dtype=torch.float32, device=self.device)
        _lib.check(self.lib.trl_debug_stage_net(self._h, _ptr(fr), nf, H, W, r.ctypes.data_as(C.c_void_p), len(r), int(net),
                                                int(capacity), _ptr(out), self._stream()))
        return out

    def front_pool(self, frames, win: np.ndarray, net: int, capacity: int | None = None, out: torch.Tensor | None = None) -> torch.Tensor:
        fr = self._frames(frames)
        nf, H, W, _ = fr.shape
        w = np.ascontiguousarray(win, np.int32).reshape(-1, 5)
        cap = len(w) if capacity is None else int(capacity)
        shape = (cap, 11, 11, 28) if net == 24 else (cap, 23, 23, 32)
        if out is None:
            out = torch.empty(shape, dtype=torch.float32, device=self.device)
        elif tuple(out.shape) != shape or out.dtype != torch.float32 or out.device != self.device or not out.is_contiguous():
            raise ValueError(f"out must be a contiguous float32 {shape} tensor on {self.device}")
        _lib.check(self.lib.trl_debug_front(self._h, _ptr(fr), nf, H, W, w.ctypes.data_as(C.c_void_p), len(w), int(net), cap, _ptr(out),
                                            self._stream()))
        return out

    def lists(self, kind: int, H: int, W: int, caps, counts, rows: np.ndarray, logits: np.ndarray | None = None) -> dict:
        caps = np.ascontiguousarray(caps, np.int32)
        counts = np.ascontiguousarray(counts, np.int32)
        n = counts.shape[0]
        L = counts.shape[1] if kind == 1 else 0
        assert len(caps) == L + 1
        rows = np.ascontiguousarray(rows, self.CAND_DTYPE if kind == 1 else np.float32)
        lg = None if logits is None else np.ascontiguousarray(logits, np.float32)
        capF = int(caps[-1])
        out = {}
        if kind == 3:
            mf = self.cfg.max_faces
            dev = dict(boxes=torch.empty((n, mf, 4), dtype=torch.float32, device=self.device),
                       probs=torch.empty((n, mf), dtype=torch.float32, device=self.device),
                       points=torch.empty((n, mf, 10), dtype=torch.float32, device=self.device),
                       counts=torch.empty((n,), dtype=torch.int32, device=self.device),
                       box0=torch.empty((n, 4), dtype=torch.float32, device=self.device),
                       prob0=torch.empty((n,), dtype=torch.float32, device=self.device),
                       rect=torch.empty((n, 4), dtype=torch.int32, device=self.device),
                       valid=torch.empty((n,), dtype=torch.uint8, device=self.device))
            pts = np.zeros((n, capF, 10), np.float32)
        else:
            dev = dict.fromkeys(("boxes", "probs", "points", "counts", "box0", "prob0", "rect", "valid"))
            pts = None
        _lib.check(self.lib.trl_debug_lists(self._h, int(kind), n, int(H), int(W), caps.ctypes.data_as(C.c_void_p), L,
                                            counts.ctypes.data_as(C.c_void_p), rows.ctypes.data_as(C.c_void_p),
                                            None if lg is None else lg.ctypes.data_as(C.c_void_p),
                                            None if pts is None else pts.ctypes.data_as(C.c_void_p),
                                            *(_ptr(dev[k]) for k in ("boxes", "probs", "points", "counts", "box0", "prob0", "rect", "valid")),
                                            self._stream()))
        torch.cuda.synchronize(self.device)
        if kind == 1:
            out["keep"] = [[self.level_keep(f, l)[1] for l in range(L)] for f in range(n)]
        out[f"rows{kind}"] = [self.stage_boxes(kind, f) for f in range(n)]
        if kind == 3:
            out["pts3"] = [pts[f, :len(out["rows3"][f])].copy() for f in range(n)]
            out.update({k: v.cpu().numpy() for k, v in dev.items()})
        return out

    def _faces_out(self, out: torch.Tensor | None, n: int, S: int) -> torch.Tensor:
# ... 73 lines not shown
```

Measured before the change: 22630 frames/s.

## Defer PNet fp16-screen confirmations to a separate compacted confirm kernel

M-tiles that the fused PNet kernel's fp16 screen flags for exact confirmation are no longer confirmed inline. Their conv2 output rows and a small header are pushed to a global queue, and a new k_pnet_confirm kernel then runs conv3 and the heads on the compacted queue. The goal is to keep divergent confirmation work out of the main fused loop. The queue is sized adaptively with overflow retry and hold-off logic in the capacity planner. This adds an extra launch, queue memory traffic, and a possible retry when the queue overflows.

```diff
diff --git a/include/truely_hip.h b/include/truely_hip.h
--- a/include/truely_hip.h
+++ b/include/truely_hip.h
@@ -98,6 +98,7 @@
 int  trl_debug_option(trl_ctx* ctx, const char* key, int value);
 int  trl_debug_pnet_screen_bound(trl_ctx* ctx, float* A, float* B, int* on);
 int  trl_debug_pnet_screen_weights(trl_ctx* ctx, float* h_g16);
+int  trl_debug_pnet_defer(trl_ctx* ctx, long long* h_out4);
 int  trl_debug_batch_capacity(trl_ctx* ctx, float t2_per_frame, float t3_per_frame, int* last_attempts);
 int  trl_debug_pyramid_level(trl_ctx* ctx, const uint8_t* d_frame, int H, int W, int level, float* d_out, int* h, int* w, void* stream);
 int  trl_debug_pyramid_batch(trl_ctx* ctx, const uint8_t* d_frames, int n, int H, int W, float* d_out, long long* pyr_stride,
diff --git a/truely-real-time-ai-generated-video-detection-framework-for-social-platforms_amd/_lib.py b/truely-real-time-ai-generated-video-detection-framework-for-social-platforms_amd/_lib.py
--- a/truely-real-time-ai-generated-video-detection-framework-for-social-platforms_amd/_lib.py
+++ b/truely-real-time-ai-generated-video-detection-framework-for-social-platforms_amd/_lib.py
@@ -98,6 +98,7 @@
     "trl_debug_pnet_span": (C.c_int, [_vp, C.c_int, C.POINTER(C.c_double), C.POINTER(C.c_int32)]),
     "trl_debug_pnet_screen_bound": (C.c_int, [_vp, C.POINTER(_f), C.POINTER(_f), C.POINTER(_i)]),
     "trl_debug_pnet_screen_weights": (C.c_int, [_vp, C.POINTER(_f)]),
+    "trl_debug_pnet_defer": (C.c_int, [_vp, C.POINTER(C.c_longlong)]),
     "trl_jpeg_create": (C.c_int, [_i, _i, _i, _i, _i, C.POINTER(_vp)]),
     "trl_jpeg_destroy": (C.c_int, [_vp]),
     "trl_jpeg_encode": (C.c_int, [_vp, _vp, _i, C.c_longlong, _vp, C.c_longlong, _vp, _vp]),
diff --git a/truely-real-time-ai-generated-video-detection-framework-for-social-platforms_amd/csrc/trl_api.hip b/truely-real-time-ai-generated-video-detection-framework-for-social-platforms_amd/csrc/trl_api.hip
--- a/truely-real-time-ai-generated-video-detection-framework-for-social-platforms_amd/csrc/trl_api.hip
+++ b/truely-real-time-ai-generated-video-detection-framework-for-social-platforms_amd/csrc/trl_api.hip
@@ -72,7 +72,7 @@
     trl_ctx* c = new trl_ctx();
     c->cfg = *cfg;
     c->pnet_prof = trl_tune_set("TRL_PNET_CLOCK");
-    if (hipMalloc((void**)&c->pnet_clk, 8 * 41) != hipSuccess || hipMemset(c->pnet_clk, 0, 8 * 41) != hipSuccess || hipMemset(c->pnet_clk, 0xFF, 8) != hipSuccess ||
+    if (hipMalloc((void**)&c->pnet_clk, 8 * 44) != hipSuccess || hipMemset(c->pnet_clk, 0, 8 * 44) != hipSuccess || hipMemset(c->pnet_clk, 0xFF, 8) != hipSuccess ||
         hipMalloc((void**)&c->pnet_cursor, 64) != hipSuccess || hipHostMalloc((void**)&c->h_pinned, 1024) != hipSuccess ||
         hipEventCreate(&c->ev_call0) != hipSuccess || hipEventCreate(&c->ev_call1) != hipSuccess) {
         trl_set_error("context allocation failed: %s", hipGetErrorString(hipGetLastError()));
@@ -97,7 +97,7 @@
     if (c->rz.dev) (void)hipFree(c->rz.dev);
     for (auto& b : c->fn_cap) if (b.p) (void)hipFree(b.p);
     if (c->pnet_clk) {
-        unsigned long long t[41];
+        unsigned long long t[42];
         if (c->pnet_prof && hipMemcpy(t, c->pnet_clk, sizeof t, hipMemcpyDeviceToHost) == hipSuccess && t[2 + 32] > 0) {
             static const char* nm[8] = {"phase0", "barrier0", "phase1", "barrier1", "phase2", "barrier2", "phase3", "barrier3"};
             const double tiles = (double)t[2 + 32];
@@ -106,6 +106,7 @@
                 fprintf(stderr, "[TRL_PNET_CLOCK] %-9s %8.0f %8.0f %8.0f %8.0f\n", nm[k], t[2 + k] / tiles, t[2 + 8 + k] / tiles, t[2 + 16 + k] / tiles, t[2 + 24 + k] / tiles);
             fprintf(stderr, "[TRL_PNET_CLOCK] fp16 screen: %llu M-tiles screened, %llu confirmed (%.2f %%)\n", t[39], t[40],
                     t[39] ? 100.0 * (double)t[40] / (double)t[39] : 0.0);
+            fprintf(stderr, "[TRL_PNET_CLOCK] confirm queue: %llu M-tiles queued, %.0f per launch\n", t[41], t[37] ? (double)t[41] / (double)t[37] : 0.0);
         }
         (void)hipFree(c->pnet_clk);
     }
@@ -934,6 +935,8 @@
     if (!strcmp(key, "rnet_chunk") && value >= 16) { c->rnet_chunk = value; return TRL_OK; }
     if (!strcmp(key, "onet_chunk") && value >= 16) { c->onet_chunk = value; return TRL_OK; }
     if (!strcmp(key, "pnet_screen") && (value == 0 || value == 1)) { c->pnet_screen = value; return TRL_OK; }
+    if (!strcmp(key, "pnet_defer") && (value == 0 || value == 1)) { c->pnet_defer = value; c->caps.defer = DeferCaps(); return TRL_OK; }
+    if (!strcmp(key, "pnet_defer_cap") && value >= 0) { c->caps.defer = DeferCaps(); c->caps.defer.forced = value; return TRL_OK; }
     if (!strcmp(key, "pyr_row_bands") && value >= 0) { c->pyr_row_bands = value; return TRL_OK; }
     if (!strcmp(key, "tail_pool") && (value == 0 || value == 1)) { c->tail_pool = value; return TRL_OK; }
     trl_set_error("unknown option '%s' (or value %d out of range)", key, value);
@@ -943,6 +946,13 @@
 int trl_debug_pnet_screen_bound(trl_ctx* c, float* A, float* B, int* on) {
     if (!c || !A || !B || !on) { trl_set_error("null argument"); return TRL_ERR_INVALID; }
     *A = c->pnet_scrA; *B = c->pnet_scrB; *on = c->pnet_screen_ok && c->pnet_screen;
+    return TRL_OK;
+}
+
+int trl_debug_pnet_defer(trl_ctx* c, long long* h_out4) {
+    if (!c || !h_out4) { trl_set_error("null argument"); return TRL_ERR_INVALID; }
+    const DeferCaps& d = c->caps.defer;
+    h_out4[0] = d.cap; h_out4[1] = d.cap > 0 ? c->h_pinned[4 + FLG_DEFER_N] : 0; h_out4[2] = d.mtiles; h_out4[3] = d.hold;
     return TRL_OK;
 }
 
diff --git a/truely-real-time-ai-generated-video-detection-framework-for-social-platforms_amd/csrc/trl_capacity.h b/truely-real-time-ai-generated-video-detection-framework-for-social-platforms_amd/csrc/trl_capacity.h
--- a/truely-real-time-ai-generated-video-detection-framework-for-social-platforms_amd/csrc/trl_capacity.h
+++ b/truely-real-time-ai-generated-video-detection-framework-for-social-platforms_amd/csrc/trl_capacity.h
@@ -6,6 +6,7 @@
 enum { TRL_NFLAGS = 64 };
 enum { FLG_LEVEL = 0, FLG_FRAME = 1, FLG_T2 = 2, FLG_T3 = 3, FLG_T2N = 4, FLG_T3N = 5, FLG_FRAME_MAX = 6, FLG_SPILL = 7,
        FLG_SPILL_CUR = 8 , FLG_SPILL_LISTS = 10, FLG_LEVEL_MAX = 16  };
+enum { FLG_DEFER = 11, FLG_DEFER_N = 12 };
 
 struct LvLayout {
     int L = 0, S = 0;
@@ -20,6 +21,37 @@
     return want > d ? want : (d > r.floor ? d : (cur < r.floor ? cur : r.floor));
 }
 
+enum { TRL_DEFER_HDR = 32, TRL_DEFER_BLOCK = 72 * 17 * 4, TRL_DEFER_SLOT = TRL_DEFER_HDR + TRL_DEFER_BLOCK };
+static_assert(TRL_DEFER_SLOT % 16 == 0, "slots are copied in 16-byte words");
+struct DeferCaps {
+    static constexpr float START = 0.25f, BOUND = 0.5f;
+    static constexpr CapRule RULE = {1.25f, 0.f, 0.97f, 0.f};
+    static constexpr int HOLD = 256;
+    static constexpr long long FULL_SLOTS = (64ll << 20) / TRL_DEFER_SLOT;
+    static constexpr long long MAX_SLOTS = (4ll << 30) / TRL_DEFER_SLOT;
+    float frac = 0.f;
+    int hold = 0;
+    int forced = 0;
+    int cap = 0; long long mtiles = 0;
+};
+inline int trl_defer_plan(const DeferCaps& d, long long mtiles, bool applicable) {
+    if (!applicable || mtiles <= 0 || d.hold > 0) return 0;
+    long long want = d.forced > 0 ? d.forced : (long long)(DeferCaps::START * (float)mtiles) + 64;
+    if (d.forced <= 0 && want < DeferCaps::FULL_SLOTS) want = DeferCaps::FULL_SLOTS;
+    const long long hint = d.frac > 0.f ? (long long)(d.frac * (float)mtiles) + 64 : 0;
+    if (hint > want) want = hint;
+    if (want > mtiles) want = mtiles;
+    if (want > DeferCaps::MAX_SLOTS) want = DeferCaps::MAX_SLOTS;
+    return (int)want;
+}
+template <class ArenaT> inline void* trl_defer_carve(ArenaT& A, int cap) { return cap > 0 ? A.alloc((size_t)cap * TRL_DEFER_SLOT) : nullptr; }
+inline bool trl_defer_check(DeferCaps& d, bool overflow, int need) {
+    const float per = (float)(d.mtiles > 0 ? d.mtiles : 1);
+    if ((float)need > DeferCaps::BOUND * per || (long long)(1.25f * (float)need) + 64 > DeferCaps::MAX_SLOTS) d.hold = DeferCaps::HOLD;
+    else d.frac = trl_cap_follow(DeferCaps::RULE, d.frac, (float)need, per, overflow);
+    return overflow;
+}
+
 struct CascadeCaps {
     static constexpr float T_START[2] = {160.f, 48.f};
     static constexpr CapRule T_RULE[2] = {{1.25f, 1.f, 0.97f, T_START[0]}, {1.25f, 1.f, 0.97f, T_START[1]}};
@@ -29,6 +61,7 @@
     float lvl_hint[32] = {0}, frame_hint = 0.f;
     size_t spill_hint = 0;
     int cap_t[2] = {0, 0};
+    DeferCaps defer;
     int resume_stage = 0;
     int last_attempts = 0;
 };
@@ -67,6 +100,7 @@
     k.resume_stage = 0;
     unsigned long long spill_used = 0;
     memcpy(&spill_used, f + FLG_SPILL_CUR, 8);
+    if (k.defer.cap > 0 && trl_defer_check(k.defer, f[FLG_DEFER] != 0, f[FLG_DEFER_N])) return {1, 0};
     if (f[FLG_LEVEL]) {
         long long sum = 0;
         for (int l = 0; l < L; l++) {
@@ -94,6 +128,7 @@
     for (int l = 0; l < L; l++)
         k.lvl_hint[l] = trl_cap_follow(CascadeCaps::LIST_RULE, k.lvl_hint[l], (float)f[FLG_LEVEL_MAX + l], 1.f, false);
     k.frame_hint = trl_cap_follow(CascadeCaps::LIST_RULE, k.frame_hint, frame_max, 1.f, false);
+    if (k.defer.cap == 0 && k.defer.hold > 0) k.defer.hold--;
     {
         const size_t want = (size_t)spill_used + (spill_used >> 2), d = k.spill_hint - (k.spill_hint >> 5);
         k.spill_hint = spill_used ? (want > d ? want : d) : (d > (1u << 20) ? d : 0);
diff --git a/truely-real-time-ai-generated-video-detection-framework-for-social-platforms_amd/csrc/trl_cascade.hip b/truely-real-time-ai-generated-video-detection-framework-for-social-platforms_amd/csrc/trl_cascade.hip
--- a/truely-real-time-ai-generated-video-detection-framework-for-social-platforms_amd/csrc/trl_cascade.hip
+++ b/truely-real-time-ai-generated-video-detection-framework-for-social-platforms_amd/csrc/trl_cascade.hip
@@ -719,7 +719,11 @@
     return TRL_OK;
 }
 
+static bool pnet_is_fused(const trl_ctx* c, int L) { return c->cfg.pnet_mode == 0 && L <= 16; }
 static void plan_caps(trl_ctx* c, int L, int n) {
+    DeferCaps& d = c->caps.defer;
+    d.mtiles = trl_pnet_mtiles(c, L, n);
+    c->cb.pq_cap = d.cap = trl_defer_plan(d, d.mtiles, pnet_is_fused(c, L) && trl_pnet_can_defer(c));
     long long cells[32];
     for (int l = 0; l < L; l++) cells[l] = (long long)c->lv[l].oh * c->lv[l].ow;
     const CascadePlan p = trl_caps_plan(c->caps, c->cfg.cap_level, c->cfg.cap_frame, cells, L, n);
@@ -823,6 +827,7 @@
     for (int k = 0; k < 2; k++) B.off[k] = (int32_t*)A.alloc((size_t)(n + 1) * 4);
     B.cbox = (int32_t*)A.alloc((size_t)n * capF * 32);
     B.flags = (int32_t*)A.alloc(TRL_NFLAGS * 4);
+    B.pq = (char*)trl_defer_carve(A, B.pq_cap);
     B.spill = spill ? (char*)A.alloc(spill) : nullptr;
     B.spill_cap = B.spill ? spill : 0;
     B.box0 = (float*)A.alloc((size_t)n * 16); B.prob0 = (float*)A.alloc((size_t)n * 4);
@@ -957,7 +962,7 @@
         TRL_HIP(hipMemsetAsync(B.lvl_cnt, 0, (size_t)n * L * 4, s));
         c->pnet_ev_used = 0;
     }
-    const bool fused = c->cfg.pnet_mode == 0 && L <= 16;
+    const bool fused = pnet_is_fused(c, L);
     TRL_CHECK(size_scratch(c, n, H, W, fused));
     if (!resume) TRL_CHECK(fused ? stage1_fused(c, d_frames, s) : stage1_generic(c, d_frames, s));
     ListLaunch ll;
@@ -1005,6 +1010,7 @@
                       float* d_prob0, int32_t* d_rect, uint8_t* d_valid, hipStream_t s) {
     CascadeBufs& B = c->cb;
     B = CascadeBufs();
+    c->caps.defer.cap = 0;
     LvLayout& G = B.lay;
     G.L = L;
     for (int l = 0; l < L; l++) { G.capl[l] = h_caps[l]; G.rec0[l] = G.S; G.S += h_caps[l]; }
diff --git a/truely-real-time-ai-generated-video-detection-framework-for-social-platforms_amd/csrc/trl_ctx.h b/truely-real-time-ai-generated-video-detection-framework-for-social-platforms_amd/csrc/trl_ctx.h
--- a/truely-real-time-ai-generated-video-detection-framework-for-social-platforms_amd/csrc/trl_ctx.h
+++ b/truely-real-time-ai-generated-video-detection-framework-for-social-platforms_amd/csrc/trl_ctx.h
@@ -30,6 +30,8 @@
     int32_t* off[2] = {nullptr, nullptr};
     int32_t* cbox = nullptr;
     int32_t* flags = nullptr;
+    char* pq = nullptr;
+    int pq_cap = 0;
     char* spill = nullptr;
     size_t spill_cap = 0;
     float* box0 = nullptr; float* prob0 = nullptr; int32_t* rect = nullptr; uint8_t* valid = nullptr; float* pts0 = nullptr;
@@ -45,6 +47,7 @@
     int nout;
     int trl_ctx::*chunk;
 };
+enum { TRL_PNET_DEFER_DEFAULT = 1 };
 enum { TRL_PNET = 0, TRL_RNET = 1, TRL_ONET = 2 };
 extern const NetDesc trl_nets[3];
 inline const NetDesc& trl_net_of(int net) { return trl_nets[net == 24 ? TRL_RNET : TRL_ONET]; }
@@ -81,6 +84,7 @@
     float pnet_scrG[16] = {};
     int pnet_screen_ok = 0;
     int pnet_screen = 1;
+    int pnet_defer = TRL_PNET_DEFER_DEFAULT;
     int pnet_run = 0;
     int32_t* pnet_cursor = nullptr;
     unsigned long long* pnet_clk = nullptr;
@@ -165,6 +169,8 @@
                              bool rgb, float* d_faces, hipStream_t s);
 int trl_pnet_generic_level(trl_ctx* c, Arena& X, const uint8_t* d_frames, int nf, int H, int W, const LevelGeom& g, float** d_heads, hipStream_t s);
 int trl_pnet_prepare(trl_ctx* c, const char* himg);
+bool trl_pnet_can_defer(const trl_ctx* c);
+long long trl_pnet_mtiles(const trl_ctx* c, int L, int n);
 size_t trl_pnet_fused_bytes(trl_ctx* c, int n, int H, int W);
 int trl_pnet_fused_all(trl_ctx* c, const uint8_t* d_frames, int n, int H, int W, hipEvent_t* ev, hipStream_t s);
 int trl_pyramid_export(trl_ctx* c, const uint8_t* d_frame, int H, int W, int level, float* d_out, int* h, int* w, hipStream_t s);
diff --git a/truely-real-time-ai-generated-video-detection-framework-for-social-platforms_amd/csrc/trl_pnet.hip b/truely-real-time-ai-generated-video-detection-framework-for-social-platforms_amd/csrc/trl_pnet.hip
--- a/truely-real-time-ai-generated-video-detection-framework-for-social-platforms_amd/csrc/trl_pnet.hip
+++ b/truely-real-time-ai-generated-video-detection-framework-for-social-platforms_amd/csrc/trl_pnet.hip
@@ -5,6 +5,7 @@
 typedef float f32x4 __attribute__((ext_vector_type(4)));
 typedef float f32x16 __attribute__((ext_vector_type(16)));
 typedef _Float16 f16x8 __attribute__((ext_vector_type(8)));
+typedef int i32x4 __attribute__((ext_vector_type(4)));
 
 namespace {
 
@@ -24,6 +25,7 @@
 constexpr int VCARRY_P = 4 * P1_T * 10;
 constexpr int VCARRY_C = 2 * C2_T * C2_LD;
 constexpr int DYN_LDS = (144 * 32 + BAND * (CARRY_P + CARRY_C) + VCARRY_P + VCARRY_C) * 4;
+static_assert((2 * C2_T * C2_LD * 4) % 16 == 0 && 4 * C2_T * C2_LD * 4 == TRL_DEFER_BLOCK, "an M-tile's 4 conv2 rows: 16-byte words of region A, one queue block");
 static_assert((144 * 32) % 4 == 0 && CARRY_P % 4 == 0 && CARRY_C % 4 == 0 && VCARRY_P % 4 == 0, "strips stay 16-byte aligned");
 
 struct PLevel {
@@ -57,6 +59,7 @@
     int run;
     unsigned long long* clk;
     int prof;
+    char* q; int q_cap; int32_t* q_cnt;
 };
 
 
@@ -110,7 +113,100 @@
 template <int... I, typename F>
 __device__ __forceinline__ void pn_static_for(std::integer_sequence<int, I...>, F&& f) { (f(std::integral_constant<int, I>{}), ...); }
 
-template <bool UNIT, bool NEG1, bool DBG>
+template <bool UNIT, typename Between>
+__device__ __forceinline__ void pn_conv3(const float* R, const float* B3S, const f32x4* T3, int mt, int l31, int hh, f32x16& P, Between&& between) {
+    const int y = mt * 2 + (l31 >> 4), x = l31 & 15;
+    const int base = (y * C2_T + x) * C2_LD + hh;
+    f32x16 acc;
+#pragma unroll
+    for (int qa = 0; qa < 4; qa++) {
+        const f32x4 b4 = T3[2 * qa + hh];
+        acc[4 * qa] = b4[0]; acc[4 * qa + 1] = b4[1]; acc[4 * qa + 2] = b4[2]; acc[4 * qa + 3] = b4[3];
+    }
+    float xa[2][12], wb[2][12];
+    auto read_sixth = [&](int sx, float* xo, float* wo) {
+#pragma unroll
+        for (int u = 0; u < 12; u++) {
+            const int s = sx * 12 + u, tap = s >> 3, ky = tap / 3, kx = tap - ky * 3;
+            xo[u] = R[base + (ky * C2_T + kx) * C2_LD + 2 * (s & 7)];
+            wo[u] = B3S[(2 * s + hh) * 32 + l31];
+        }
+    };
+    read_sixth(0, xa[0], wb[0]);
+    pn_static_for(std::make_integer_sequence<int, 6>{}, [&](auto SX) __attribute__((always_inline)) {
+        constexpr int sx = decltype(SX)::value;
+        if (sx < 5) read_sixth(sx + 1, xa[(sx + 1) & 1], wb[(sx + 1) & 1]);
+        __builtin_amdgcn_sched_barrier(0);
+        pn_static_for(std::make_integer_sequence<int, 12>{}, [&](auto UU) __attribute__((always_inline)) {
+            constexpr int u = decltype(UU)::value;
+            acc = __builtin_amdgcn_mfma_f32_32x32x2f32(wb[sx & 1][u], xa[sx & 1][u], acc, 0, 0, 0);
+            between(SX, UU);
+        });
+        __builtin_amdgcn_sched_barrier(0);
+    });
+#pragma unroll
+    for (int qa = 0; qa < 4; qa++) {
+        const f32x4 s4 = T3[8 + 2 * qa + hh];
+#pragma unroll
+        for (int qb = 0; qb < 4; qb++) P[4 * qa + qb] = prelu_t<UNIT>(acc[4 * qa + qb], s4[qb], UNIT ? 0.f : trl_prelu_sel(s4[qb]));
+    }
+}
+struct PnHeads {
+    float WH[4];
+    unsigned hlo[4], hhi[4];
+    __device__ __forceinline__ void load(const float* wh, int lane) {
+#pragma unroll
+        for (int r = 0; r < 4; r++) WH[r] = wh[(((lane >> 2) & 7) + 8 * r) * 32 + 4 * (lane >> 5) + (lane & 3)];
+    }
+    template <int k>
+    __device__ __forceinline__ void step(const f32x16& P, f32x4& hq) {
+        constexpr int ga = k >> 3, gb = k & 7;
+        if constexpr (gb == 0) {
+#pragma unroll
+            for (int qb = 0; qb < 4; qb++) {
+                const unsigned v = __float_as_uint(P[4 * ga + qb]);
+                const auto r = __builtin_amdgcn_permlane32_swap(v, v, false, false);
+                hlo[qb] = r[0]; hhi[qb] = r[1];
+            }
+        }
+        const float bk = __uint_as_float(gb < 4 ? hlo[gb & 3] : hhi[gb & 3]);
+        hq = __builtin_amdgcn_mfma_f32_4x4x1f32(WH[ga], bk, hq, 3, gb, 0);
+    }
+    __device__ __forceinline__ void all(const f32x16& P, f32x4& hq) {
+        pn_static_for(std::make_integer_sequence<int, 32>{}, [&](auto H_T) __attribute__((always_inline)) { step<decltype(H_T)::value>(P, hq); });
+    }
+};
+__device__ __forceinline__ void pn_emit(const PnetArgs& a, int f, int l, int oy0, int ox0, int oh, int ow, float fscale, int dbg_skip, int lane,
+                                        const f32x4& hq) {
+    if (__builtin_amdgcn_ballot_w64(lane < 32 && hq[1] - hq[0] >= a.dthr) == 0) return;
+    const float p = trl_softmax2_p1(hq[0], hq[1]);
+    const auto u2 = __builtin_amdgcn_permlane32_swap(__float_as_uint(hq[0]), __float_as_uint(hq[0]), false, false);
+    const auto u3 = __builtin_amdgcn_permlane32_swap(__float_as_uint(hq[1]), __float_as_uint(hq[1]), false, false);
+    if (lane < 32) {
+        const int oy = oy0 + (lane >> 4), ox = ox0 + (lane & 15);
+        if (oy < oh && ox < ow) {
+            if (p >= a.thr && !(dbg_skip & 32)) {
+                const int seg = f * a.L + l;
+                const int sl = atomicAdd(&a.lvl_cnt[seg], 1);
+                if (sl < a.lv[l].cap) {
+                    Cand c;
+                    c.x1 = floorf((2.f * (float)ox + 1.f) / fscale);
+                    c.y1 = floorf((2.f * (float)oy + 1.f) / fscale);
+                    c.x2 = floorf((2.f * (float)ox + 12.f) / fscale);
+                    c.y2 = floorf((2.f * (float)oy + 12.f) / fscale);
+                    c.score = p;
+                    c.r0 = hq[2]; c.r1 = hq[3]; c.r2 = __uint_as_float(u2[1]); c.r3 = __uint_as_float(u3[1]);
+                    c.cell = oy * ow + ox;
+                    a.lvl_rec[(size_t)f * a.rec_stride + a.lv[l].rec0 + sl] = c;
+                } else {
+                    a.flags[FLG_LEVEL] = 1;
+                }
+            }
+        }
+    }
+}
+
+template <bool UNIT, bool NEG1, bool DBG, bool DEFER>
 __global__ __launch_bounds__(256, 2) void k_pnet_fused(PnetArgs a) {
     __shared__ __attribute__((aligned(16))) float RA[REGION_A];
     __shared__ __attribute__((aligned(16))) float RB[REGION_B];
@@ -129,11 +225,11 @@
     const int l31 = lane & 31, hh = lane >> 5;
 
     for (int i = tid; i < 144 * 32; i += 256) B3S[i] = a.w3[i];
-    float B2[23], WH[4];
+    float B2[23];
 #pragma unroll
     for (int s = 0; s < 23; s++) B2[s] = a.w2[(4 * s + kq) * 32 + l15];
-#pragma unroll
-    for (int r = 0; r < 4; r++) WH[r] = a.wh[(((lane >> 2) & 7) + 8 * r) * 32 + 4 * (lane >> 5) + (lane & 3)];
+    PnHeads hd;
+    if constexpr (!DEFER) hd.load(a.wh, lane);
     const float bias2 = a.b2[l15], slope2 = a.s2[l15];
     if (tid < 32) { T3all[tid] = a.b3[tid]; T3all[32 + tid] = a.s3[tid]; if (tid < 8) T3all[64 + tid] = a.bh[tid]; }
     if (tid < 32) { T3all[72 + tid] = a.wh[tid * 32 + 1] - a.wh[tid * 32]; if (tid == 0) T3all[104] = a.bh[1] - a.bh[0]; }
@@ -619,87 +715,9 @@
         if (!(dbg_skip & 8)) {
             const float fscale = g.scale;
             const f32x4* T3 = reinterpret_cast<const f32x4*>(T3all);
-            auto conv3 = [&](int mt, f32x16& P, auto&& between) __attribute__((always_inline)) {
-                const int y = mt * 2 + (l31 >> 4), x = l31 & 15;
-                const int base = (y * C2_T + x) * C2_LD + hh;
-                f32x16 acc;
-#pragma unroll
-                for (int qa = 0; qa < 4; qa++) {
-                    const f32x4 b4 = T3[2 * qa + hh];
-                    acc[4 * qa] = b4[0]; acc[4 * qa + 1] = b4[1]; acc[4 * qa + 2] = b4[2]; acc[4 * qa + 3] = b4[3];
-                }
-                float xa[2][12], wb[2][12];
-                auto read_sixth = [&](int sx, float* xo, float* wo) {
-#pragma unroll
-                    for (int u = 0; u < 12; u++) {
-                        const int s = sx * 12 + u, tap = s >> 3, ky = tap / 3, kx = tap - ky * 3;
-                        xo[u] = RA[base + (ky * C2_T + kx) * C2_LD + 2 * (s & 7)];
-                        wo[u] = B3S[(2 * s + hh) * 32 + l31];
-                    }
-                };
-                read_sixth(0, xa[0], wb[0]);
-                pn_static_for(std::make_integer_sequence<int, 6>{}, [&](auto SX) __attribute__((always_inline)) {
-                    constexpr int sx = decltype(SX)::value;
-                    if (sx < 5) read_sixth(sx + 1, xa[(sx + 1) & 1], wb[(sx + 1) & 1]);
-                    __builtin_amdgcn_sched_barrier(0);
-                    pn_static_for(std::make_integer_sequence<int, 12>{}, [&](auto UU) __attribute__((always_inline)) {
-                        constexpr int u = decltype(UU)::value;
-                        acc = __builtin_amdgcn_mfma_f32_32x32x2f32(wb[sx & 1][u], xa[sx & 1][u], acc, 0, 0, 0);
-                        between(SX, UU);
-                    });
-                    __builtin_amdgcn_sched_barrier(0);
-                });
-#pragma unroll
-                for (int qa = 0; qa < 4; qa++) {
-                    const f32x4 s4 = T3[8 + 2 * qa + hh];
-#pragma unroll
-                    for (int qb = 0; qb < 4; qb++) P[4 * qa + qb] = prelu_t<UNIT>(acc[4 * qa + qb], s4[qb], UNIT ? 0.f : trl_prelu_sel(s4[qb]));
-                }
-            };
-            unsigned hlo[4], hhi[4];
-            auto head_step = [&](auto H_T, const f32x16& P, f32x4& hq) __attribute__((always_inline)) {
-                constexpr int k = decltype(H_T)::value, ga = k >> 3, gb = k & 7;
-                if constexpr (gb == 0) {
-#pragma unroll
-                    for (int qb = 0; qb < 4; qb++) {
-                        const unsigned v = __float_as_uint(P[4 * ga + qb]);
-                        const auto r = __builtin_amdgcn_permlane32_swap(v, v, false, false);
-                        hlo[qb] = r[0]; hhi[qb] = r[1];
-                    }
-                }
-                const float bk = __uint_as_float(gb < 4 ? hlo[gb & 3] : hhi[gb & 3]);
-                hq = __builtin_amdgcn_mfma_f32_4x4x1f32(WH[ga], bk, hq, 3, gb, 0);
-            };
-            auto heads_all = [&](const f32x16& P, f32x4& hq) __attribute__((always_inline)) {
-                pn_static_for(std::make_integer_sequence<int, 32>{}, [&](auto H_T) __attribute__((always_inline)) { head_step(H_T, P, hq); });
-            };
-            auto emit = [&](int mt, const f32x4& hq) __attribute__((always_inline)) {
-                if (__builtin_amdgcn_ballot_w64(lane < 32 && hq[1] - hq[0] >= a.dthr) == 0) return;
-                const float p = trl_softmax2_p1(hq[0], hq[1]);
-                const auto u2 = __builtin_amdgcn_permlane32_swap(__float_as_uint(hq[0]), __float_as_uint(hq[0]), false, false);
-                const auto u3 = __builtin_amdgcn_permlane32_swap(__float_as_uint(hq[1]), __float_as_uint(hq[1]), false, false);
-                if (lane < 32) {
-                    const int oy = ty * TS + mt * 2 + (lane >> 4), ox = tx * TS + (lane & 15);
-                    if (oy < g.oh && ox < g.ow) {
-                        if (p >= a.thr && !(dbg_skip & 32)) {
-                            const int seg = f * a.L + l;
-                            const int sl = atomicAdd(&a.lvl_cnt[seg], 1);
-                            if (sl < a.lv[l].cap) {
-                                Cand c;
-                                c.x1 = floorf((2.f * (float)ox + 1.f) / fscale);
-                                c.y1 = floorf((2.f * (float)oy + 1.f) / fscale);
-                                c.x2 = floorf((2.f * (float)ox + 12.f) / fscale);
-                                c.y2 = floorf((2.f * (float)oy + 12.f) / fscale);
-                                c.score = p;
-                                c.r0 = hq[2]; c.r1 = hq[3]; c.r2 = __uint_as_float(u2[1]); c.r3 = __uint_as_float(u3[1]);
-                                c.cell = oy * g.ow + ox;
-                                a.lvl_rec[(size_t)f * a.rec_stride + a.lv[l].rec0 + sl] = c;
-                            } else {
-                                a.flags[FLG_LEVEL] = 1;
-                            }
-                        }
-                    }
-                }
+            [[maybe_unused]] auto conv3 = [&](int mt, f32x16& P, auto&& between) __attribute__((always_inline)) { pn_conv3<UNIT>(RA, B3S, T3, mt, l31, hh, P, between); };
+            [[maybe_unused]] auto emit = [&](int mt, const f32x4& hq) __attribute__((always_inline)) {
+                pn_emit(a, f, l, ty * TS + mt * 2, tx * TS, g.oh, g.ow, fscale, dbg_skip, lane, hq);
             };
             const int mt0 = wave, mt1 = wave + 4;
             const bool has0 = 2 * mt0 < vrows, has1 = 2 * mt1 < vrows;
@@ -745,7 +763,33 @@
                 if (has1) cf1 = screen(mt1, sb0 + 8 * C2_T);
                 if (DBG) { nscr += has1 ? 2 : 1; ncnf += (cf0 ? 1 : 0) + (cf1 ? 1 : 0); }
             }
-            if (cf0 && cf1) {
+            if constexpr (DEFER) {
+                auto defer = [&](int mt) __attribute__((always_inline)) {
+                    int slot = 0;
+                    if (lane == 0) slot = atomicAdd(a.q_cnt, 1);
+                    slot = __builtin_amdgcn_readfirstlane(slot);
+                    if (slot < a.q_cap) {
+                        char* const dst = a.q + (size_t)slot * TRL_DEFER_SLOT;
+                        const f32x4* src = reinterpret_cast<const f32x4*>(RA + mt * (2 * C2_T * C2_LD));
+                        f32x4* d4 = reinterpret_cast<f32x4*>(dst + TRL_DEFER_HDR);
+#pragma unroll
+                        for (int i = 0; i < (TRL_DEFER_BLOCK / 16 + 63) / 64; i++) {
+                            const int j = lane + 64 * i;
+                            if (j < TRL_DEFER_BLOCK / 16) d4[j] = src[j];
+                        }
+                        if (lane == 0) {
+                            int* h = reinterpret_cast<int*>(dst);
+                            *reinterpret_cast<i32x4*>(h) = i32x4{f, l, ty, tx};
+                            h[4] = mt;
+                        }
+                    } else if (lane == 0) {
+                        a.flags[FLG_DEFER] = 1;
+                    }
+                };
+                if (cf0) defer(mt0);
+                if (cf1) defer(mt1);
+                strips_get();
+            } else if (cf0 && cf1) {
                 f32x16 P0;
                 f32x4 hq0 = T3[16 + hh];
                 conv3(mt0, P0, [](auto, auto) {});
@@ -756,12 +800,12 @@
                         constexpr int sx = decltype(SX)::value, u = decltype(UU)::value, h = sx * 6 + (u >> 1);
                         if constexpr ((u & 1) == 1 && h < 32) {
                             __builtin_amdgcn_sched_barrier(0);
-                            head_step(std::integral_constant<int, h>{}, P0, hq0);
+                            hd.template step<h>(P0, hq0);
                             __builtin_amdgcn_sched_barrier(0);
                         }
                     });
                     strips_get();
-                    heads_all(P1, hq1);
+                    hd.all(P1, hq1);
                     emit(mt0, hq0);
                     emit(mt1, hq1);
                 }
@@ -771,7 +815,7 @@
                 f32x4 hq0 = T3[16 + hh];
                 conv3(mt, P0, [](auto, auto) {});
                 strips_get();
-                heads_all(P0, hq0);
+                hd.all(P0, hq0);
                 emit(mt, hq0);
             } else {
                 strips_get();
@@ -788,17 +832,62 @@
         for (int k = 0; k < 8; k++) atomicAdd(&a.clk[2 + 8 * wave + k], pt[k]);
         if (wave == 0) atomicAdd(&a.clk[2 + 32], (unsigned long long)rot);
     }
-    if (DBG && lane == 0 && nscr) { atomicAdd(&a.clk[39], (unsigned long long)nscr); atomicAdd(&a.clk[40], (unsigned long long)ncnf); }
+    if (DBG && lane == 0 && nscr) { atomicAdd(&a.clk[DEFER ? 42 : 39], (unsigned long long)nscr); atomicAdd(&a.clk[DEFER ? 43 : 40], (unsigned long long)ncnf); }
     if (DBG && tid == 0) atomicMax(&a.clk[1], (unsigned long long)wall_clock64());
 }
 
-}
-
-__global__ void k_pnet_span(unsigned long long* clk) {
+constexpr int CONFIRM_WAVES = 8;
+template <bool UNIT>
+__global__ __launch_bounds__(64 * CONFIRM_WAVES, 4) void k_pnet_confirm(PnetArgs a) {
+    __shared__ __attribute__((aligned(16))) float B3S[144 * 32];
+    __shared__ __attribute__((aligned(16))) float WA[CONFIRM_WAVES][4 * C2_T * C2_LD];
+    __shared__ __attribute__((aligned(16))) float T3all[72];
+    const int tid = threadIdx.x, lane = tid & 63;
+    const int wave = __builtin_amdgcn_readfirstlane(tid >> 6);
+    const int asked = *a.q_cnt;
+    if (blockIdx.x == 0 && tid == 0) a.flags[FLG_DEFER_N] = asked;
+    const int n = asked < a.q_cap ? asked : a.q_cap;
+    if ((int)blockIdx.x * CONFIRM_WAVES >= n) return;
+    for (int i = tid; i < 144 * 32; i += 64 * CONFIRM_WAVES) B3S[i] = a.w3[i];
+    if (tid < 32) { T3all[tid] = a.b3[tid]; T3all[32 + tid] = a.s3[tid]; if (tid < 8) T3all[64 + tid] = a.bh[tid]; }
+    const int slot = blockIdx.x * CONFIRM_WAVES + wave;
+    const char* const src = a.q + (size_t)(slot < n ? slot : 0) * TRL_DEFER_SLOT;
+    if (slot < n) {
+        const f32x4* s4 = reinterpret_cast<const f32x4*>(src + TRL_DEFER_HDR);
+        f32x4* d4 = reinterpret_cast<f32x4*>(WA[wave]);
+#pragma unroll
+        for (int i = 0; i < (TRL_DEFER_BLOCK / 16 + 63) / 64; i++) {
+            const int j = lane + 64 * i;
+            if (j < TRL_DEFER_BLOCK / 16) d4[j] = s4[j];
+        }
+    }
+    PnHeads hd;
+    hd.load(a.wh, lane);
+    __syncthreads();
+    if (slot >= n) return;
+    const int* h = reinterpret_cast<const int*>(src);
+    const int f = h[0], l = h[1], ty = h[2], tx = h[3], mt = h[4];
+    const PLevel& g = a.lv[l];
+    const int l31 = lane & 31, hh = lane >> 5;
+    const f32x4* T3 = reinterpret_cast<const f32x4*>(T3all);
+    f32x16 P;
+    f32x4 hq = T3[16 + hh];
+    pn_conv3<UNIT>(WA[wave], B3S, T3, 0, l31, hh, P, [](auto, auto) {});
+    hd.all(P, hq);
+    pn_emit(a, f, l, ty * TS + mt * 2, tx * TS, g.oh, g.ow, g.scale, 0, lane, hq);
+}
+
+}
+
+__global__ void k_pnet_span(unsigned long long* clk, const int32_t* q_cnt, int q_cap) {
     const unsigned long long t0 = clk[0], t1 = clk[1];
     const unsigned long long d = t1 > t0 ? t1 - t0 : 0ull;
     clk[36] += d; clk[37] += 1ull; clk[38] = d;
     clk[0] = ~0ull; clk[1] = 0ull;
+    if (q_cnt) {
+        if (*q_cnt <= q_cap) { clk[39] += clk[42]; clk[40] += clk[43]; clk[41] += (unsigned long long)*q_cnt; }
+        clk[42] = clk[43] = 0ull;
+    }
 }
 
 static void pnet_screen_bound(trl_ctx* c, const float* W, const float* H, const float* b3, const float* s3, const float* bh) {
@@ -898,6 +987,17 @@
     a.lvl_cnt = c->cb.lvl_cnt; a.lvl_rec = c->cb.lvl_rec; a.flags = c->cb.flags;
     a.clk = c->pnet_clk; a.prof = c->pnet_prof ? 1 : 0;
     a.xcd_next = c->pnet_cursor;
+    a.q = c->cb.pq; a.q_cap = c->cb.pq ? c->cb.pq_cap : 0; a.q_cnt = c->pnet_cursor + 8;
+}
+
+bool trl_pnet_can_defer(const trl_ctx* c) {
+    return c->pnet_defer && c->pnet_screen && c->pnet_screen_ok && c->pnet_unit && c->cfg.thr0 >= 0.01f && c->cfg.thr0 <= 0.99f &&
+           trl_tune_int("TRL_PNET_SKIP", 0) == 0;
+}
+long long trl_pnet_mtiles(const trl_ctx* c, int L, int n) {
+    long long m = 0;
+    for (int l = 0; l < L; l++) if (c->lv[l].oh > 0 && c->lv[l].ow > 0) m += (long long)((c->lv[l].ow + TS - 1) / TS) * ((c->lv[l].oh + 1) / 2);
+    return m * n;
 }
 
 size_t trl_pnet_fused_bytes(trl_ctx* c, int n, int H, int W) {
@@ -916,7 +1016,7 @@
     int grid = 256 * 2;
     if (grid > ((total_tiles + 7) / 8) * 8) grid = ((total_tiles + 7) / 8) * 8;
     if (grid < 8) grid = 8;
-    TRL_HIP(hipMemsetAsync(c->pnet_cursor, 0, 8 * sizeof(int32_t), s));
+    TRL_HIP(hipMemsetAsync(c->pnet_cursor, 0, 9 * sizeof(int32_t), s));
     TRL_CHECK(trl_gate_wait(c, s));
     if (ev) TRL_HIP(hipEventRecord(ev[2], s));
 #ifdef TRL_TUNING
@@ -933,18 +1033,25 @@
     };
     bool launched = false;
 #ifdef TRL_TUNING
-#define TRL_PK(U, N) do { launched = dbg ? launch(k_pnet_fused<U, N, true>) : launch(k_pnet_fused<U, N, false>); } while (0)
+#define TRL_PK(U, N, D) do { launched = dbg ? launch(k_pnet_fused<U, N, true, D>) : launch(k_pnet_fused<U, N, false, D>); } while (0)
 #else
-#define TRL_PK(U, N) do { launched = launch(k_pnet_fused<U, N, false>); } while (0)
+#define TRL_PK(U, N, D) do { launched = launch(k_pnet_fused<U, N, false, D>); } while (0)
 #endif
-    if (c->pnet_unit) { if (c->pnet_mono1) TRL_PK(true, false); else TRL_PK(true, true); }
-    else { if (c->pnet_mono1) TRL_PK(false, false); else TRL_PK(false, true); }
+    const bool defer = a.q_cap > 0;
+    if (defer && !(c->pnet_unit && a.screen)) { trl_set_error("confirm queue planned for a launch that cannot defer"); return TRL_ERR_STATE; }
+    if (defer) { if (c->pnet_mono1) TRL_PK(true, false, true); else TRL_PK(true, true, true); }
+    else if (c->pnet_unit) { if (c->pnet_mono1) TRL_PK(true, false, false); else TRL_PK(true, true, false); }
+    else { if (c->pnet_mono1) TRL_PK(false, false, false); else TRL_PK(false, true, false); }
 #undef TRL_PK
     if (!launched) { trl_set_error("k_pnet_fused: %d bytes of dynamic LDS refused", DYN_LDS); return TRL_ERR_HIP; }
     TRL_LAUNCH_CHECK();
+    if (defer) {
+        k_pnet_confirm<true><<<(a.q_cap + CONFIRM_WAVES - 1) / CONFIRM_WAVES, 64 * CONFIRM_WAVES, 0, s>>>(a);
+        TRL_LAUNCH_CHECK();
+    }
     if (ev) TRL_HIP(hipEventRecord(ev[3], s));
     if (dbg) {
-        k_pnet_span<<<1, 1, 0, s>>>(c->pnet_clk);
+        k_pnet_span<<<1, 1, 0, s>>>(c->pnet_clk, defer ? a.q_cnt : nullptr, a.q_cap);
         TRL_LAUNCH_CHECK();
     }
     return TRL_OK;
diff --git a/truely-real-time-ai-generated-video-detection-framework-for-social-platforms_amd/engine.py b/truely-real-time-ai-generated-video-detection-framework-for-social-platforms_amd/engine.py
--- a/truely-real-time-ai-generated-video-detection-framework-for-social-platforms_amd/engine.py
+++ b/truely-real-time-ai-generated-video-detection-framework-for-social-platforms_amd/engine.py
@@ -420,6 +420,11 @@
         g = (C.c_float * 16)()
         _lib.check(self.lib.trl_debug_pnet_screen_weights(self._h, g))
         return [float(v) for v in g]
+
+    def pnet_defer(self) -> dict:
+        t = (C.c_longlong * 4)()
+        _lib.check(self.lib.trl_debug_pnet_defer(self._h, t))
+        return dict(zip(("slots", "queued", "mtiles", "hold"), (int(v) for v in t)))
 
     def pnet_run(self, run: int = 0):
         _lib.check(self.lib.trl_debug_pnet_run(self._h, int(run)))
```

After: 23190 frames/s, median of 6. 2.5% higher.
